# lzzcd001/MeshDiffusion

Hardware: AMD Instinct MI355X
Metric: denoise steps/sec on 64^3x4 DMTet grids (sample-steps/s = n_gpus*batch*steps/wall) (higher is better)
Workload: dtype f16f6 in the Winograd convs behind a GroupNorm (fp16 hi*hi MFMA + MX block-scaled e2m3 cross terms in a K-concatenated scaled MFMA at twice the e4m3 rate; operands and weights equalised per input channel by a power of two: md_wino_equaliser, after the load-time calibration from the measured operand

## Files before the change

### include/meshdiffusion_hip.h

```cpp
#ifndef MESHDIFFUSION_HIP_H
#define MESHDIFFUSION_HIP_H

#include <stdint.h>

#ifdef __cplusplus
extern "C" {
#endif

#define MD_OK 0
#define MD_ERR_BAD_ARG (-1)
#define MD_ERR_UNSUPPORTED (-2)
#define MD_ERR_NO_DEVICE (-3)

#define MD_ABI_VERSION 16

enum {
  MD_CFG_C3_128 = 0,
  MD_CFG_C3_128_K16 = 1,
  MD_CFG_C3_32 = 2,
  MD_CFG_C3_LOW = 3,
  MD_CFG_C3_S2 = 4,
  MD_CFG_G1_128 = 5,
  MD_CFG_G1_128_LOW = 6,
  MD_CFG_G1_64_LOW = 7,
  MD_CFG_C3_128_V2 = 8,
  MD_CFG_C3_128_SW = 9,
  MD_CFG_C3_128_PIPE = 10,
  MD_CFG_C3_128_FAST = 14,
  MD_CFG_C5_128_K16 = 15,
  MD_CFG_C5_32_K16 = 16,
  MD_CFG_C3_128_W4 = 17,
  MD_CFG_C3X_32 = 18,
  MD_CFG_C5X_32_K16 = 19,
  MD_CFG_C3X_128_K16 = 20,
  MD_CFG_C5X_128 = 21,
  MD_CFG_G1_128_N128 = 22,
  MD_CFG_COUNT = 23
};

enum { MD_OUT_F32B = 0, MD_OUT_S16B = 1, MD_OUT_NCDHW = 2 };
enum { MD_A_PACKED = 0, MD_A_S16B = 1 };
enum { MD_B_S16B = 0, MD_B_F32B_GN = 1 };
enum { MD_PREC_BF16X3 = 0, MD_PREC_FP16X2 = 1 };

typedef struct MdGemmConvArgs {
  const void* a;
  const void* b;
  void* out;
  const float* bias;
  const float* residual;
  float alpha;
  int32_t cfg;
  int32_t batch;
  int32_t rows;
  int32_t rows_alloc;
  int32_t kdim;
  int32_t D, H, W;
  int32_t ups;
  int32_t a_src;
  int32_t out_mode;
  int32_t a_rows;
  int64_t a_bstride;
  int64_t bias_bstride;
  int64_t res_bstride;
  int64_t b_bstride;
  float* partial;
  int32_t ksplit;
  int32_t prec;
  double* stats;
  int32_t stagger;
  int32_t b_mode;
  const void* b2;
  const float* b_ac;
  int64_t b2_bstride;
  int32_t b_split;
  int32_t b_silu;
} MdGemmConvArgs;

int md_abi_version(void);
int md_device_count(void);

int md_gemm_conv(const MdGemmConvArgs* args, void* stream);
int64_t md_gemm_conv_partial_bytes(const MdGemmConvArgs* args);
int md_gemm_conv_cfg_info(int32_t cfg, int32_t* nt, int32_t* kc, int32_t* cols,
                          int32_t* taps, int32_t* lds_bytes, int32_t* threads);

int md_pack_weights(const float* w, void* wpk, int32_t rows, int32_t kdim, int32_t taps,
                    int64_t s_row, int64_t s_k, int64_t s_tap, int32_t nt, int32_t kc,
                    int32_t prec, void* stream);
int64_t md_packed_weight_bytes(int32_t rows, int32_t kdim, int32_t taps, int32_t nt, int32_t kc);

int md_gn_stats(const float* x, double* sums, int32_t batch, int32_t C, int64_t P,
                int32_t c_total, int32_t c_off, void* stream);
int md_gn_finalize(const double* sums, const float* gamma, const float* beta,
                   float* params, int32_t batch, int32_t c_total, int32_t groups,
                   int64_t P, float eps, float* ac, void* stream);
int md_gn_apply(const float* x, const float* params, void* out, void* out_raw, int32_t batch,
                int32_t C, int64_t P, int32_t c_total, int32_t c_off, int32_t norm,
                int32_t silu, float drop_p, uint64_t drop_seed, void* stream);
int md_dropout_scale(float* out, int32_t batch, int32_t C, int64_t P, int32_t c_total, int32_t c_off,
                     float drop_p, uint64_t drop_seed, void* stream);
int md_zero(void* p, int64_t bytes, void* stream);

int md_timestep_embedding(const float* t, float* emb, int32_t batch, int32_t dim, void* stream);
int md_linear(const float* x, const float* w, const float* bias, float* y, int32_t batch,
              int32_t in_dim, int32_t out_dim, int32_t silu_in, void* stream);

int md_fold_dx(const float* y, const float* bias, float* out, int32_t batch, int32_t co, int32_t kx, int32_t rows_alloc,
               int32_t D, int32_t H, int32_t W, void* stream);
int md_ncdhw_to_s16b_xfold(const float* x, void* out, int32_t batch, int32_t C, int32_t kx, int32_t c_pad, int32_t D, int32_t H,
                           int32_t W, void* stream);
int md_ncdhw_to_s16b(const float* x, void* out, int32_t batch, int32_t C, int32_t c_pad,
                     int64_t P, void* stream);
int md_f32b_to_ncdhw(const float* x, float* out, int32_t batch, int32_t C, int64_t P, void* stream);
int md_ncdhw_to_f32b(const float* x, float* out, int32_t batch, int32_t C, int64_t P, void* stream);
int md_s16b_to_ncdhw(const void* x, float* out, int32_t batch, int32_t C, int64_t P, void* stream);

int md_softmax_keys(const float* s, void* p, int32_t batch, int32_t n_keys, int32_t n_q,
                    void* stream);

int md_nin_f32(const float* x1, const float* x2, int32_t c1, int32_t c2, const void* wpk, const float* bias,
               float* out, int32_t batch, int32_t cout, int64_t P, int32_t n_cu, void* stream);

int64_t md_wino_operand_bytes(int32_t batch, int32_t cin, int32_t D, int32_t H, int32_t W);
int md_wino_prep(const float* x1, const float* x2, int32_t c1, int32_t c2, const float* ac, int32_t silu, int32_t ups,
                 void* t_out, int32_t batch, int32_t D, int32_t H, int32_t W, float drop_p, uint64_t drop_seed, void* stream);
int64_t md_wino_weight_bytes(int32_t cout, int32_t cin);
int md_wino_pack_weights(const float* w, void* wpk, int32_t cout, int32_t cin, int64_t s_row, int64_t s_k, int32_t flip,
                         void* stream);
int md_conv3_wino(const void* t_in, const void* wpk, float* out, const float* bias, int64_t bias_bstride,
                  const float* residual, int64_t res_bstride, double* stats, int32_t batch, int32_t cin, int32_t cout,
                  int32_t D, int32_t H, int32_t W, int32_t variant, void* stream);

int md_wino_equaliser(const float* gamma, const float* beta, const float* w, int32_t cout, int32_t cin, int64_t s_row, int64_t s_k,
                      float* eq, void* stream);
int md_wino_equaliser_measured(const float* gamma, const float* beta, const float* w, const float* a2m, int32_t cout, int32_t cin,
                               int64_t s_row, int64_t s_k, float* eq, void* stream);
int md_wino_operand_ms(const float* x1, const float* x2, int32_t c1, int32_t c2, const float* ac, int32_t silu, int32_t batch, int64_t P,
                       float* ms, void* stream);
int md_wino_prep_f8(const float* x1, const float* x2, int32_t c1, int32_t c2, const float* ac, int32_t silu, int32_t ups,
                    const float* eq, void* t_out, int32_t batch, int32_t D, int32_t H, int32_t W, void* stream);
int64_t md_wino_weight_bytes_f8(int32_t cout, int32_t cin);
int md_wino_pack_weights_f8(const float* w, const float* eq, void* wpk, int32_t cout, int32_t cin, int64_t s_row, int64_t s_k, void* stream);
int md_conv3_wino_f8(const void* t_in, const void* wpk, float* out, const float* bias, int64_t bias_bstride,
                     const float* residual, int64_t res_bstride, double* stats, int32_t batch, int32_t cin, int32_t cout,
                     int32_t D, int32_t H, int32_t W, void* stream);
int md_absmax(const float* x, int64_t n, uint32_t* amax_bits, void* stream);
int md_wino_prep_dual_f6(const float* x, int32_t c, void* t_out, void* u_out, float* sums, float tscale, const uint32_t* amax_bits,
                         int32_t batch, int32_t D, int32_t H, int32_t W, void* stream);
int md_conv3_wino_f6_scaled(const void* t_in, const void* wpk, float* out, const float* bias, int64_t bias_bstride,
                            const float* residual, int64_t res_bstride, double* stats, int32_t batch, int32_t cin, int32_t cout,
                            int32_t D, int32_t H, int32_t W, float out_scale, const uint32_t* amax_bits, void* stream);

int md_wino_prep_f6(const float* x1, const float* x2, int32_t c1, int32_t c2, const float* ac, int32_t silu, int32_t ups,
                    const float* eq, void* t_out, int32_t batch, int32_t D, int32_t H, int32_t W, void* stream);
int md_wino_pack_weights_f6(const float* w, const float* eq, void* wpk, int32_t cout, int32_t cin, int64_t s_row, int64_t s_k, void* stream);
int md_conv3_wino_f6(const void* t_in, const void* wpk, float* out, const float* bias, int64_t bias_bstride,
                     const float* residual, int64_t res_bstride, double* stats, int32_t batch, int32_t cin, int32_t cout,
                     int32_t D, int32_t H, int32_t W, void* stream);

int md_conv3_stem(const void* x16, const void* wpk, float* out, const float* bias, const float* residual, double* stats,
                  int32_t batch, int32_t cout, int32_t D, int32_t H, int32_t W, void* stream);

int md_conv3_head(const float* x, const float* ac, const void* wpk, float* y, int32_t batch, int32_t cin, int32_t rows_alloc,
                  int32_t D, int32_t H, int32_t W, void* stream);

enum { MD_PACK_WPK = 0, MD_PACK_WINO = 1, MD_PACK_WINO_F6 = 2 };
typedef struct MdPackJob {
  const float* w;
  void* out;
  int64_t s_row, s_k, s_tap, n_items, block0;
  int32_t rows, kdim, taps, nt, kc, prec, flip, kind;
} MdPackJob;
int md_pack_batch(const MdPackJob* jobs_dev, int32_t n_jobs, int64_t total_blocks, int32_t tiled, void* stream);

int md_conv3_s2(const float* x, const void* wpk, float* out, const float* bias, int64_t bias_bstride, double* stats,
                int32_t batch, int32_t cin, int32_t rows, int32_t rows_alloc, int32_t D, int32_t H, int32_t W, void* stream);

int md_wino_prep_v2(const float* x1, const float* x2, int32_t c1, int32_t c2, const float* ac, int32_t silu, int32_t ups,
                    void* t_out, int32_t batch, int32_t D, int32_t H, int32_t W, float drop_p, uint64_t drop_seed, void* stream);

int md_wino_prep_dual(const float* x1, const float* x2, int32_t c1, int32_t c2, const float* ac, int32_t silu, int32_t ups,
                      void* t_out, void* u_out, float* sums, int32_t batch, int32_t D, int32_t H, int32_t W, float drop_p,
                      uint64_t drop_seed, void* stream);

int md_attn_fwd(const void* qk, const void* vT, void* out, const float* bias_v, int32_t batch, int32_t C,
                int32_t N, float scale, void* stream);

int md_ancestral_step(const float* x, const float* eps, const float* z, const float* mask,
                      const float* coef, float* x_out, float* x_mean_out, int32_t batch,
                      int32_t C, int64_t P, void* stream);
int md_ddim_step(const double* x, const float* eps, const float* mask, const double* coef, const float* partial,
                 const float* pmask, int32_t ch, double* x_out, double* x0_out, float* x_f32, int32_t batch,
                 int32_t C, int64_t P, void* stream);
#define MD_LANGEVIN_SLABS 64
#define MD_CORRECTOR_LANGEVIN 0
#define MD_CORRECTOR_ALD 1
#define MD_SDE_REVERSE_DIFFUSION 0
#define MD_SDE_EULER_MARUYAMA 1
int md_langevin_norms(const float* eps, const float* z, int32_t batch, int32_t C, int64_t P, double* slabs, void* stream);
int md_langevin_step(const float* x, const float* eps, const float* z, const float* mask, const float* coef,
                     const double* slabs, float snr, int32_t mode, float* x_out, float* x_mean_out, float* step_out,
                     int32_t batch, int32_t C, int64_t P, void* stream);
int md_sde_step(const float* x, const float* eps, const float* z, const float* mask, const float* coef, int32_t kind,
                float* x_out, float* x_mean_out, int32_t batch, int32_t C, int64_t P, void* stream);
int md_inpaint_blend(float* x, const float* src, const float* pmask, const float* gmask,
                     int32_t batch, int32_t C, int32_t ch, int64_t P, int64_t src_bstride,
                     void* stream);

int md_inpaint_renoise(float* x, float* x_mean, const float* z, const float* pmask,
                       const float* gmask, const float* coef, int32_t batch, int32_t C,
                       int32_t ch, int64_t P, void* stream);

int md_ddpm_perturb(const float* x0, const float* noise, const float* mask, const float* coef, float* out,
                    int32_t batch, int32_t C, int64_t P, void* stream);
int md_masked_sq_err(const float* eps_hat, const float* noise, const float* mask, double* sums, float* grad,
                     float gscale, int32_t batch, int32_t C, int64_t P, void* stream);
int md_grad_sqnorm(const float* g, int64_t n, double* out, void* stream);
int md_adam_ema_step(float* p, const float* g, float* m, float* v, float* ema, int64_t n, float lr, float beta1,
                     float beta2, float eps, float weight_decay, int32_t step, float ema_decay,
                     const double* grad_sqnorm, float max_norm, void* stream);

int64_t md_pb16_bytes(int32_t batch, int32_t C, int32_t D, int32_t H, int32_t W, int32_t guard, int32_t pad);
int md_to_pb16(const void* src, void* out, int32_t batch, int32_t C, int32_t c_src, int32_t D, int32_t H, int32_t W,
               int32_t guard, int32_t pad, int32_t mode, int32_t up, int32_t stuff, int32_t zsplit, int32_t zhalo,
               void* stream);
int md_wgrad_finish(const float* g, float* dw, int32_t rows, int32_t cols, int32_t cols_alloc, int32_t ntap,
                    int32_t tap0, int64_t s_row, int64_t s_k, int64_t s_tap, void* stream);
int64_t md_wgrad_workspace_bytes(int32_t rows, int32_t cols, int32_t taps, int32_t ksplit);
int md_wgrad(const void* dy_pb, const void* act_pb, float* dw, void* workspace, int64_t workspace_bytes, int32_t batch,
             int32_t a_ch, int32_t b_ch, int32_t rows, int32_t cols, int32_t D, int32_t H, int32_t W, int32_t guard,
             int32_t taps, int32_t ksplit, int64_t s_row, int64_t s_k, int64_t s_tap, void* stream);

int64_t md_wgrad_wino_workspace_bytes(int32_t co, int32_t ci, int32_t ksplit);
int md_wgrad_wino(const void* u_dy, const void* t_act, float* dw, void* workspace, int64_t workspace_bytes, int32_t batch,
                  int32_t co, int32_t ci, int32_t D, int32_t H, int32_t W, int32_t ksplit, int64_t s_row, int64_t s_k,
                  int64_t s_tap, void* stream);

int64_t md_wgrad_nin_workspace_bytes(int32_t co, int32_t ci, int32_t ksplit);
int md_wgrad_nin(const void* dy_s16, const void* x_s16, float* dw, void* workspace, int64_t workspace_bytes, int32_t batch,
                 int32_t co, int32_t ci, int64_t P, int32_t ksplit, int64_t s_row, int64_t s_k, void* stream);
int md_gn_bwd_stats(const float* x, const float* dy, const float* params, double* sums, int32_t batch, int32_t C,
                    int64_t P, int32_t c_total, int32_t c_off, int32_t dy_ctotal, int32_t silu, float drop_p,
                    uint64_t drop_seed, void* stream);
int md_gn_bwd_finalize(const double* sums, const float* params, const float* gamma, float* coef, float* dgamma,
                       float* dbeta, int32_t batch, int32_t c_total, int32_t groups, int64_t P, void* stream);
int md_gn_bwd_apply(const float* x, const float* dy, const float* params, const float* coef, float* dx, int32_t batch,
                    int32_t C, int64_t P, int32_t c_total, int32_t c_off, int32_t dy_ctotal, int32_t silu,
                    int32_t accumulate, float drop_p, uint64_t drop_seed, const float* residual, float* ch_sums,
                    uint32_t* amax_bits, void* stream);
int md_channel_sums(const float* x, float* out, int32_t batch, int32_t C, int64_t P, void* stream);
int md_s16b_transpose(const void* in, void* out, int32_t batch, int32_t R, int32_t Cn, void* stream);
int md_softmax_keys_bwd(const void* p, const float* dp, void* ds, int32_t batch, int32_t n_keys, int32_t n_q,
                        float alpha, void* stream);
int md_grad_resample(const float* in, float* out, int32_t batch, int32_t C, int32_t Dc, int32_t Hc, int32_t Wc,
                     int32_t mode, int32_t accumulate, void* stream);

int64_t md_marching_tets_workspace_bytes(int32_t n_meshes, int32_t n_edges, int32_t n_tets);
int md_marching_tets(const float* pos, const float* sdf, const int32_t* tets,
                     const int32_t* edges, const int32_t* tet_edges, int32_t n_meshes,
                     int32_t n_verts, int32_t n_edges, int32_t n_tets, float* verts,
                     int64_t* faces, int64_t* face_tet, int32_t* counts, void* workspace,
                     int64_t workspace_bytes, void* stream);
#define MD_SDF_REG_SLABS 64
#define MD_SDF_REG_WORKSPACE_BYTES (MD_SDF_REG_SLABS * 24)
int md_marching_tets_bwd(const float* pos, const float* sdf, const int32_t* edges, const int32_t* vid,
                         const int32_t* counts, const float* grad_verts, const int32_t* inc_ptr, const int32_t* inc,
                         int32_t n_meshes, int32_t n_verts, int32_t n_edges, float* dpos, float* dsdf, void* stream);
int md_sdf_reg_loss(const float* sdf, const int32_t* edges, int32_t n_verts, int32_t n_edges, void* workspace,
                    float* loss, int32_t* count, void* stream);
int md_sdf_reg_loss_bwd(const float* sdf, const int32_t* edges, const int32_t* inc_ptr, const int32_t* inc,
                        const int32_t* count, const float* grad_out, int32_t n_verts, int32_t n_edges, float* dsdf,
                        void* stream);

int md_vertex_normals(const float* verts, const int64_t* faces, int64_t n_verts, int64_t n_faces, float* v_nrm,
                      float* f_nrm, void* stream);

int64_t md_nn_sided_workspace_bytes(int32_t batch, int32_t n, int32_t m);
int md_nn_sided(const float* p, const float* q, int32_t batch, int32_t n, int32_t m, int32_t skip_same_index,
                float* dist, int64_t* idx, void* workspace, int64_t workspace_bytes, void* stream);
int md_chamfer_bwd(const float* p, const float* q, const int64_t* idx_pq, const int64_t* idx_qp,
                   const int32_t* ptr_p, const int32_t* order_p, const int32_t* ptr_q, const int32_t* order_q,
                   int32_t batch, int32_t n, int32_t m, float w1, float w2, const float* grad_out, float* dp,
                   float* dq, void* stream);
int md_face_areas(const float* verts, const int64_t* faces, int32_t batch, int32_t n_verts, int32_t n_faces,
                  float* areas, void* stream);
int md_sample_points(const float* verts, const int64_t* faces, const float* cdf, const float* r_face,
                     const float* r_u, const float* r_v, const int64_t* face_choices_in, int32_t batch,
                     int32_t n_verts, int32_t n_faces, int32_t n_samples, float* points, int64_t* face_choices,
                     float* weights, void* stream);
int md_sample_points_bwd(const float* grad_points, const float* weights, const int32_t* ptr, const int32_t* order,
                         int32_t batch, int32_t n_verts, int32_t n_samples, float* dverts, void* stream);

#ifdef __cplusplus
}
#endif
#endif
```

### meshdiffusion_amd/_lib.py

```python
import ctypes as C
import os

_HERE = os.path.dirname(os.path.abspath(__file__))
LIB_PATH = os.environ.get("MD_LIB") or os.path.join(_HERE, "libmeshdiffusion_hip.so")

(CFG_C3_128, CFG_C3_128_K16, CFG_C3_32, CFG_C3_LOW, CFG_C3_S2, CFG_G1_128, CFG_G1_128_LOW, CFG_G1_64_LOW,
 CFG_C3_128_V2, CFG_C3_128_SW, CFG_C3_128_PIPE) = range(11)
(CFG_C3_128_FAST, CFG_C5_128_K16, CFG_C5_32_K16, CFG_C3_128_W4, CFG_C3X_32, CFG_C5X_32_K16, CFG_C3X_128_K16, CFG_C5X_128,
 CFG_G1_128_N128) = range(14, 23)
OUT_F32B, OUT_S16B, OUT_NCDHW = 0, 1, 2
PREC_BF16X3, PREC_FP16X2 = 0, 1
A_PACKED, A_S16B = 0, 1
B_S16B, B_F32B_GN = 0, 1
CORRECTOR_LANGEVIN, CORRECTOR_ALD = 0, 1
SDE_REVERSE_DIFFUSION, SDE_EULER_MARUYAMA = 0, 1
LANGEVIN_SLABS = 64

CFG_NT_KC = {
    CFG_C3_128: (128, 32), CFG_C3_128_K16: (128, 16), CFG_C3_32: (32, 32), CFG_C3_LOW: (128, 32),
    CFG_C3_S2: (128, 32), CFG_G1_128: (128, 32), CFG_G1_128_LOW: (128, 32), CFG_G1_64_LOW: (64, 32),
    CFG_C3_128_V2: (128, 32), CFG_C3_128_SW: (128, 32), CFG_C3_128_PIPE: (128, 32),
    CFG_C3_128_FAST: (128, 32), CFG_C5_128_K16: (128, 16), CFG_C5_32_K16: (32, 16), CFG_C3_128_W4: (128, 32), CFG_C3X_32: (32, 32), CFG_C5X_32_K16: (32, 16), CFG_C3X_128_K16: (128, 16), CFG_C5X_128: (128, 32), CFG_G1_128_N128: (128, 32),
}
ABLATION_CFG_NT_KC = {c: (128, 32) for c in (101, 102, 103, 104, 105, 111, 113, 114, 116, 117, 118, 122)}


class MdGemmConvArgs(C.Structure):
    _fields_ = [
        ("a", C.c_void_p), ("b", C.c_void_p), ("out", C.c_void_p), ("bias", C.c_void_p),
        ("residual", C.c_void_p), ("alpha", C.c_float), ("cfg", C.c_int32), ("batch", C.c_int32),
        ("rows", C.c_int32), ("rows_alloc", C.c_int32), ("kdim", C.c_int32), ("D", C.c_int32),
        ("H", C.c_int32), ("W", C.c_int32), ("ups", C.c_int32), ("a_src", C.c_int32),
        ("out_mode", C.c_int32), ("a_rows", C.c_int32), ("a_bstride", C.c_int64),
        ("bias_bstride", C.c_int64), ("res_bstride", C.c_int64), ("b_bstride", C.c_int64), ("partial", C.c_void_p), ("ksplit", C.c_int32), ("prec", C.c_int32),
        ("stats", C.c_void_p), ("stagger", C.c_int32), ("b_mode", C.c_int32), ("b2", C.c_void_p), ("b_ac", C.c_void_p),
        ("b2_bstride", C.c_int64), ("b_split", C.c_int32), ("b_silu", C.c_int32),
    ]


class MdPackJob(C.Structure):
    _fields_ = [
        ("w", C.c_void_p), ("out", C.c_void_p), ("s_row", C.c_int64), ("s_k", C.c_int64), ("s_tap", C.c_int64),
        ("n_items", C.c_int64), ("block0", C.c_int64), ("rows", C.c_int32), ("kdim", C.c_int32), ("taps", C.c_int32),
        ("nt", C.c_int32), ("kc", C.c_int32), ("prec", C.c_int32), ("flip", C.c_int32), ("kind", C.c_int32),
    ]


PACK_WPK, PACK_WINO, PACK_WINO_F6 = 0, 1, 2
ABI_VERSION = 16
_P, _I32, _I64, _F, _U64 = C.c_void_p, C.c_int32, C.c_int64, C.c_float, C.c_uint64

SIGNATURES = {
    "md_abi_version": (C.c_int, []),
    "md_device_count": (C.c_int, []),
    "md_gemm_conv": (C.c_int, [C.POINTER(MdGemmConvArgs), _P]),
    "md_gemm_conv_partial_bytes": (_I64, [C.POINTER(MdGemmConvArgs)]),
    "md_gemm_conv_cfg_info": (C.c_int, [_I32] + [C.POINTER(C.c_int32)] * 6),
    "md_pack_weights": (C.c_int, [_P, _P, _I32, _I32, _I32, _I64, _I64, _I64, _I32, _I32, _I32, _P]),
    "md_packed_weight_bytes": (_I64, [_I32, _I32, _I32, _I32, _I32]),
    "md_gn_stats": (C.c_int, [_P, _P, _I32, _I32, _I64, _I32, _I32, _P]),
    "md_gn_finalize": (C.c_int, [_P, _P, _P, _P, _I32, _I32, _I32, _I64, _F, _P, _P]),
    "md_gn_apply": (C.c_int, [_P, _P, _P, _P, _I32, _I32, _I64, _I32, _I32, _I32, _I32, _F, _U64, _P]),
    "md_dropout_scale": (C.c_int, [_P, _I32, _I32, _I64, _I32, _I32, _F, _U64, _P]),
    "md_zero": (C.c_int, [_P, _I64, _P]),
    "md_timestep_embedding": (C.c_int, [_P, _P, _I32, _I32, _P]),
    "md_linear": (C.c_int, [_P, _P, _P, _P, _I32, _I32, _I32, _I32, _P]),
    "md_ncdhw_to_s16b_xfold": (C.c_int, [_P, _P, _I32, _I32, _I32, _I32, _I32, _I32, _I32, _P]),
    "md_fold_dx": (C.c_int, [_P, _P, _P, _I32, _I32, _I32, _I32, _I32, _I32, _I32, _P]),
    "md_ncdhw_to_s16b": (C.c_int, [_P, _P, _I32, _I32, _I32, _I64, _P]),
    "md_f32b_to_ncdhw": (C.c_int, [_P, _P, _I32, _I32, _I64, _P]),
    "md_ncdhw_to_f32b": (C.c_int, [_P, _P, _I32, _I32, _I64, _P]),
    "md_s16b_to_ncdhw": (C.c_int, [_P, _P, _I32, _I32, _I64, _P]),
    "md_nin_f32": (C.c_int, [_P, _P, _I32, _I32, _P, _P, _P, _I32, _I32, _I64, _I32, _P]),
    "md_wino_operand_bytes": (_I64, [_I32, _I32, _I32, _I32, _I32]),
    "md_wino_prep": (C.c_int, [_P, _P, _I32, _I32, _P, _I32, _I32, _P, _I32, _I32, _I32, _I32, _F, _U64, _P]),
    "md_wino_weight_bytes": (_I64, [_I32, _I32]),
    "md_wino_pack_weights": (C.c_int, [_P, _P, _I32, _I32, _I64, _I64, _I32, _P]),
    "md_conv3_wino": (C.c_int, [_P, _P, _P, _P, _I64, _P, _I64, _P, _I32, _I32, _I32, _I32, _I32, _I32, _I32, _P]),
    "md_wino_equaliser": (C.c_int, [_P, _P, _P, _I32, _I32, _I64, _I64, _P, _P]),
    "md_wino_equaliser_measured": (C.c_int, [_P, _P, _P, _P, _I32, _I32, _I64, _I64, _P, _P]),
    "md_wino_operand_ms": (C.c_int, [_P, _P, _I32, _I32, _P, _I32, _I32, _I64, _P, _P]),
    "md_wino_prep_f8": (C.c_int, [_P, _P, _I32, _I32, _P, _I32, _I32, _P, _P, _I32, _I32, _I32, _I32, _P]),
    "md_wino_weight_bytes_f8": (_I64, [_I32, _I32]),
    "md_wino_pack_weights_f8": (C.c_int, [_P, _P, _P, _I32, _I32, _I64, _I64, _P]),
    "md_conv3_wino_f8": (C.c_int, [_P, _P, _P, _P, _I64, _P, _I64, _P, _I32, _I32, _I32, _I32, _I32, _I32, _P]),
    "md_absmax": (C.c_int, [_P, _I64, _P, _P]),
    "md_wino_prep_dual_f6": (C.c_int, [_P, _I32, _P, _P, _P, _F, _P, _I32, _I32, _I32, _I32, _P]),
    "md_conv3_wino_f6_scaled": (C.c_int, [_P, _P, _P, _P, _I64, _P, _I64, _P, _I32, _I32, _I32, _I32, _I32, _I32, _F, _P, _P]),
    "md_wino_prep_f6": (C.c_int, [_P, _P, _I32, _I32, _P, _I32, _I32, _P, _P, _I32, _I32, _I32, _I32, _P]),
    "md_wino_pack_weights_f6": (C.c_int, [_P, _P, _P, _I32, _I32, _I64, _I64, _P]),
    "md_conv3_wino_f6": (C.c_int, [_P, _P, _P, _P, _I64, _P, _I64, _P, _I32, _I32, _I32, _I32, _I32, _I32, _P]),
    "md_conv3_stem": (C.c_int, [_P, _P, _P, _P, _P, _P, _I32, _I32, _I32, _I32, _I32, _P]),
    "md_conv3_head": (C.c_int, [_P, _P, _P, _P, _I32, _I32, _I32, _I32, _I32, _I32, _P]),
    "md_pack_batch": (C.c_int, [_P, _I32, _I64, _I32, _P]),
    "md_conv3_s2": (C.c_int, [_P, _P, _P, _P, _I64, _P, _I32, _I32, _I32, _I32, _I32, _I32, _I32, _P]),
    "md_wino_prep_v2": (C.c_int, [_P, _P, _I32, _I32, _P, _I32, _I32, _P, _I32, _I32, _I32, _I32, _F, _U64, _P]),
    "md_wino_prep_dual": (C.c_int, [_P, _P, _I32, _I32, _P, _I32, _I32, _P, _P, _P, _I32, _I32, _I32, _I32, _F, _U64, _P]),
    "md_wgrad_wino_workspace_bytes": (_I64, [_I32, _I32, _I32]),
    "md_wgrad_wino": (C.c_int, [_P, _P, _P, _P, _I64, _I32, _I32, _I32, _I32, _I32, _I32, _I32, _I64, _I64, _I64, _P]),
    "md_wgrad_nin_workspace_bytes": (_I64, [_I32, _I32, _I32]),
    "md_wgrad_nin": (C.c_int, [_P, _P, _P, _P, _I64, _I32, _I32, _I32, _I64, _I32, _I64, _I64, _P]),
    "md_attn_fwd": (C.c_int, [_P, _P, _P, _P, _I32, _I32, _I32, _F, _P]),
    "md_softmax_keys": (C.c_int, [_P, _P, _I32, _I32, _I32, _P]),
    "md_ancestral_step": (C.c_int, [_P, _P, _P, _P, _P, _P, _P, _I32, _I32, _I64, _P]),
    "md_ddim_step": (C.c_int, [_P, _P, _P, _P, _P, _P, _I32, _P, _P, _P, _I32, _I32, _I64, _P]),
    "md_langevin_norms": (C.c_int, [_P, _P, _I32, _I32, _I64, _P, _P]),
    "md_langevin_step": (C.c_int, [_P, _P, _P, _P, _P, _P, _F, _I32, _P, _P, _P, _I32, _I32, _I64, _P]),
    "md_sde_step": (C.c_int, [_P, _P, _P, _P, _P, _I32, _P, _P, _I32, _I32, _I64, _P]),
    "md_inpaint_blend": (C.c_int, [_P, _P, _P, _P, _I32, _I32, _I32, _I64, _I64, _P]),
    "md_inpaint_renoise": (C.c_int, [_P, _P, _P, _P, _P, _P, _I32, _I32, _I32, _I64, _P]),
    "md_ddpm_perturb": (C.c_int, [_P, _P, _P, _P, _P, _I32, _I32, _I64, _P]),
    "md_masked_sq_err": (C.c_int, [_P, _P, _P, _P, _P, _F, _I32, _I32, _I64, _P]),
    "md_grad_sqnorm": (C.c_int, [_P, _I64, _P, _P]),
    "md_adam_ema_step": (C.c_int, [_P, _P, _P, _P, _P, _I64, _F, _F, _F, _F, _F, _I32, _F, _P, _F, _P]),
    "md_pb16_bytes": (_I64, [_I32, _I32, _I32, _I32, _I32, _I32, _I32]),
    "md_to_pb16": (C.c_int, [_P, _P, _I32, _I32, _I32, _I32, _I32, _I32, _I32, _I32, _I32, _I32, _I32, _I32, _I32, _P]),
    "md_wgrad_finish": (C.c_int, [_P, _P, _I32, _I32, _I32, _I32, _I32, _I64, _I64, _I64, _P]),
    "md_wgrad_workspace_bytes": (_I64, [_I32, _I32, _I32, _I32]),
    "md_wgrad": (C.c_int, [_P, _P, _P, _P, _I64, _I32, _I32, _I32, _I32, _I32, _I32, _I32, _I32, _I32, _I32, _I32, _I64, _I64,
                           _I64, _P]),
    "md_gn_bwd_stats": (C.c_int, [_P, _P, _P, _P, _I32, _I32, _I64, _I32, _I32, _I32, _I32, _F, _U64, _P]),
    "md_gn_bwd_finalize": (C.c_int, [_P, _P, _P, _P, _P, _P, _I32, _I32, _I32, _I64, _P]),
    "md_gn_bwd_apply": (C.c_int, [_P, _P, _P, _P, _P, _I32, _I32, _I64, _I32, _I32, _I32, _I32, _I32, _F, _U64, _P, _P, _P, _P]),
    "md_channel_sums": (C.c_int, [_P, _P, _I32, _I32, _I64, _P]),
    "md_s16b_transpose": (C.c_int, [_P, _P, _I32, _I32, _I32, _P]),
    "md_softmax_keys_bwd": (C.c_int, [_P, _P, _P, _I32, _I32, _I32, _F, _P]),
    "md_grad_resample": (C.c_int, [_P, _P, _I32, _I32, _I32, _I32, _I32, _I32, _I32, _P]),
    "md_marching_tets_workspace_bytes": (_I64, [_I32, _I32, _I32]),
    "md_vertex_normals": (C.c_int, [_P, _P, _I64, _I64, _P, _P, _P]),
    "md_marching_tets": (C.c_int, [_P, _P, _P, _P, _P, _I32, _I32, _I32, _I32, _P, _P, _P, _P, _P, _I64, _P]),
    "md_marching_tets_bwd": (C.c_int, [_P, _P, _P, _P, _P, _P, _P, _P, _I32, _I32, _I32, _P, _P, _P]),
    "md_sdf_reg_loss": (C.c_int, [_P, _P, _I32, _I32, _P, _P, _P, _P]),
    "md_sdf_reg_loss_bwd": (C.c_int, [_P, _P, _P, _P, _P, _P, _I32, _I32, _P, _P]),
    "md_nn_sided_workspace_bytes": (_I64, [_I32, _I32, _I32]),
    "md_nn_sided": (C.c_int, [_P, _P, _I32, _I32, _I32, _I32, _P, _P, _P, _I64, _P]),
    "md_chamfer_bwd": (C.c_int, [_P, _P, _P, _P, _P, _P, _P, _P, _I32, _I32, _I32, _F, _F, _P, _P, _P, _P]),
    "md_face_areas": (C.c_int, [_P, _P, _I32, _I32, _I32, _P, _P]),
    "md_sample_points": (C.c_int, [_P, _P, _P, _P, _P, _P, _P, _I32, _I32, _I32, _I32, _P, _P, _P, _P]),
    "md_sample_points_bwd": (C.c_int, [_P, _P, _P, _P, _I32, _I32, _I32, _P, _P]),
}
SDF_REG_SLABS = 64
SDF_REG_WORKSPACE_BYTES = SDF_REG_SLABS * 24

ABLATION_SIGNATURES = {"md_wgrad_set_debug": (None, [_I32])}

_lib = None


class MeshDiffusionHipError(RuntimeError):
    pass


def load():
    global _lib
    if _lib is not None:
        return _lib
    if not os.path.exists(LIB_PATH):
        raise MeshDiffusionHipError(
            f"{LIB_PATH} not found: run `python -m meshdiffusion_amd.build` (needs hipcc). "
            "There is no CPU fallback for the HIP path.")
    import torch
    lib = C.CDLL(LIB_PATH)
    for name, (res, args) in SIGNATURES.items():
        fn = getattr(lib, name)
        fn.restype = res
        fn.argtypes = args
    for name, (res, args) in ABLATION_SIGNATURES.items():
        fn = getattr(lib, name, None)
        if fn is not None:
            fn.restype = res
            fn.argtypes = args
    if lib.md_abi_version() != ABI_VERSION:
        raise MeshDiffusionHipError(f"ABI version mismatch: library {lib.md_abi_version()}, host code {ABI_VERSION}")
    if hasattr(lib, "md_wgrad_set_debug"):
        CFG_NT_KC.update(ABLATION_CFG_NT_KC)
    for cfg, (nt, kc) in CFG_NT_KC.items():
        v = [C.c_int32() for _ in range(6)]
        lib.md_gemm_conv_cfg_info(cfg, *[C.byref(x) for x in v])
        if (v[0].value, v[1].value) != (nt, kc):
            raise MeshDiffusionHipError(f"cfg {cfg} NT/KC mismatch between _lib.py and the library")
    if torch.cuda.is_available() and lib.md_device_count() != torch.cuda.device_count():
        raise MeshDiffusionHipError("libmeshdiffusion_hip.so is not sharing PyTorch's HIP runtime "
                                    f"({lib.md_device_count()} vs {torch.cuda.device_count()} devices)")
    _lib = lib
    return lib


def check(rc, what):
    if rc != 0:
        raise MeshDiffusionHipError(f"{what} failed with code {rc}")


def cfg_info(cfg):
    lib = load()
    v = [C.c_int32() for _ in range(6)]
    check(lib.md_gemm_conv_cfg_info(cfg, *[C.byref(x) for x in v]), "md_gemm_conv_cfg_info")
    keys = ("nt", "kc", "cols", "taps", "lds_bytes", "threads")
    return dict(zip(keys, (x.value for x in v)))
```

### meshdiffusion_amd/csrc/conv3_wino.hip

```cpp
#include <type_traits>
#include "md_common.h"
#include "md_pack.h"

namespace {
constexpr int WN_THREADS = 256;
constexpr int WN_TZ = 4, WN_TY = 8, WN_TX = 8;
constexpr int WN_TPOS = 6 * 10 * 4;
constexpr int WN_HBUF = 4 * WN_TPOS * 16;
constexpr int WN_NDMA = WN_HBUF / 1024;
constexpr int WN_RED = 4 * 32 * 2;
constexpr int WN_WAVE_LDS = 2 * WN_HBUF;
constexpr int WN_LDS_BYTES = 4 * WN_WAVE_LDS + 4 * WN_NDMA * 64 * 4;

__device__ const uint4 wn_zero16 = {0u, 0u, 0u, 0u};

typedef uint32_t wn_u32x4 __attribute__((ext_vector_type(4)));
__device__ __forceinline__ uint4 wn_gload16(const void* p) {
  return __builtin_bit_cast(uint4, *(__attribute__((address_space(1))) const wn_u32x4*)(uintptr_t)p);
}
}

__global__ __launch_bounds__(256) void md_wino_prep_kernel(const float* __restrict__ x1, const float* __restrict__ x2,
                                                           int c1, int c2, const float* __restrict__ ac, int silu, int ups,
                                                           uint4* __restrict__ T, int batch, int D, int H, int W,
                                                           uint32_t thr16, float drop_scale, uint64_t seed) {
  const int Wp = W >> 1;
  const int64_t Ph = (int64_t)D * H * Wp;
  const int CG = (c1 + c2) >> 3;
  const int64_t n = (int64_t)batch * CG * Ph;
  const int64_t id = (int64_t)blockIdx.x * 256 + threadIdx.x;
  if (id >= n) return;
  const int64_t pos2 = id % Ph;
  const int cg = (int)((id / Ph) % CG);
  const int b = (int)(id / (Ph * CG));
  const int pr = (int)(pos2 % Wp), y = (int)((pos2 / Wp) % H), z = (int)(pos2 / ((int64_t)Wp * H));
  int Di = D, Hi = H, Wi = W, zs = z, ys = y;
  if (ups) { Di >>= 1; Hi >>= 1; Wi >>= 1; zs >>= 1; ys >>= 1; }
  const int64_t Pin = (int64_t)Di * Hi * Wi;
  const float* src = (cg * 8 < c1) ? x1 + ((int64_t)b * (c1 >> 3) + cg) * Pin * 8
                                   : x2 + ((int64_t)b * (c2 >> 3) + (cg - (c1 >> 3))) * Pin * 8;
  float a[8], c[8];
#pragma unroll
  for (int e = 0; e < 8; ++e) { a[e] = 1.f; c[e] = 0.f; }
  if (ac != nullptr) {
    const f32x4* ap = (const f32x4*)(ac + ((int64_t)b * (c1 + c2) + cg * 8) * 2);
#pragma unroll
    for (int q = 0; q < 4; ++q) {
      const f32x4 v = ap[q];
      a[2 * q] = v[0]; c[2 * q] = v[1]; a[2 * q + 1] = v[2]; c[2 * q + 1] = v[3];
    }
  }
  float d[4][8];
#pragma unroll
  for (int q = 0; q < 4; ++q) {
    const int xw = 2 * pr - 1 + q;
    const bool live = xw >= 0 && xw < W;
    f32x4 v0 = {0.f, 0.f, 0.f, 0.f}, v1 = v0;
    const int xs = ups ? (xw >> 1) : xw;
    const int64_t spos = ((int64_t)zs * Hi + ys) * Wi + xs;
    if (live) {
      const f32x4* p = (const f32x4*)(src + spos * 8);
      v0 = p[0]; v1 = p[1];
    }
    uint64_t bits[2] = {0, 0};
    if (thr16) {
      const uint64_t quad0 = (uint64_t)(((int64_t)b * (c1 + c2) + cg * 8) >> 2) * (uint64_t)Pin;
      bits[0] = md_drop_bits(seed, quad0 + (uint64_t)spos);
      bits[1] = md_drop_bits(seed, quad0 + (uint64_t)Pin + (uint64_t)spos);
    }
#pragma unroll
    for (int e = 0; e < 8; ++e) {
      float yv = e < 4 ? v0[e] : v1[e - 4];
      if (ac != nullptr) {
        yv = yv * a[e] + c[e];
        if (silu) yv = yv * __builtin_amdgcn_rcpf(1.0f + __builtin_amdgcn_exp2f(yv * -1.4426950408889634f));
      }
      if (thr16) yv = md_drop_keep(bits[e >> 2], e & 3, thr16) ? yv * drop_scale : 0.f;
      d[q][e] = live ? yv : 0.f;
    }
  }
  uint4* out = T + ((int64_t)b * CG + cg) * 8 * Ph + pos2;
#pragma unroll
  for (int f = 0; f < 4; ++f) {
    float t[8];
#pragma unroll
    for (int e = 0; e < 8; ++e)
      t[e] = f == 0 ? d[0][e] - d[2][e] : f == 1 ? d[1][e] + d[2][e] : f == 2 ? d[2][e] - d[1][e] : d[1][e] - d[3][e];
    uint32_t hw[4], lw[4];
#pragma unroll
    for (int q = 0; q < 4; ++q) md_split2(t[2 * q], t[2 * q + 1], hw[q], lw[q]);
    out[(int64_t)(f * 2) * Ph] = make_uint4(hw[0], hw[1], hw[2], hw[3]);
    out[(int64_t)(f * 2 + 1) * Ph] = make_uint4(lw[0], lw[1], lw[2], lw[3]);
  }
}

__global__ __launch_bounds__(256) void md_wino_pack_weights_kernel(const float* __restrict__ w, uint4* __restrict__ wpk,
                                                                   int cout, int cin, int64_t s_row, int64_t s_k, int flip) {
  const int64_t n = (int64_t)cout * cin * 36 / 4;
  const int64_t id = (int64_t)blockIdx.x * 256 + threadIdx.x;
  if (id >= n) return;
  wpk[id] = md_pack_wino_item(w, cout, cin, s_row, s_k, flip, id);
}

__global__ __launch_bounds__(256) void md_wino_amax_kernel(const float* __restrict__ w, int cout, int cin, int64_t s_row, int64_t s_k,
                                                           uint32_t* __restrict__ hdr, const float* __restrict__ eq) {
  const int64_t n = (int64_t)cout * cin * 27;
  float m = 0.f;
  for (int64_t i = (int64_t)blockIdx.x * 256 + threadIdx.x; i < n; i += (int64_t)gridDim.x * 256) {
    const int t = (int)(i % 27);
    const int64_t r = i / 27;
    float v = fabsf(w[(r / cin) * s_row + (r % cin) * s_k + t]);
    if (eq) v /= eq[r % cin];
    m = v > m ? v : m;
  }
  m = md_wave_max(m);
  if ((threadIdx.x & 63) == 0) atomicMax(hdr, __float_as_uint(m));
}

__global__ __launch_bounds__(256) void md_wino_pack_weights_f8_kernel(const float* __restrict__ w, uint4* __restrict__ wpk, int cout, int cin,
                                                                      int64_t s_row, int64_t s_k, uint32_t* __restrict__ hdr,
                                                                      const float* __restrict__ eq) {
  const int64_t n = (int64_t)cout * cin * 9;
  const int64_t id = (int64_t)blockIdx.x * 256 + threadIdx.x;
  const float wscale = md_wino_f8_wscale(__uint_as_float(hdr[0]));
  if (id == 0) {
    hdr[1] = (uint32_t)ilogbf(wscale);
    hdr[2] = __float_as_uint(1.0f / wscale);
    hdr[3] = 0u;
  }
  if (id >= n) return;
  wpk[id] = md_pack_wino_f8_item(w, cout, cin, s_row, s_k, wscale, id, eq);
}

__global__ __launch_bounds__(256) void md_wino_pack_weights_f6_kernel(const float* __restrict__ w, uint4* __restrict__ wpk, int cout, int cin,
                                                                      int64_t s_row, int64_t s_k, uint32_t* __restrict__ hdr,
                                                                      const float* __restrict__ eq) {
  const int64_t n = (int64_t)cout * cin * 9;
  const int64_t id = (int64_t)blockIdx.x * 256 + threadIdx.x;
  const float wscale = md_wino_f8_wscale(__uint_as_float(hdr[0]));
  if (id == 0) {
    hdr[1] = (uint32_t)ilogbf(wscale);
    hdr[2] = __float_as_uint(1.0f / wscale);
    hdr[3] = 6u;
  }
  if (id >= n) return;
  wpk[id] = md_pack_wino_f6_item(w, cout, cin, s_row, s_k, wscale, id, eq);
}

struct WnArgs {
  const uint4* T;
  const uint4* wpk;
  float* out;
  const float* bias;
  const float* residual;
  double* stats;
  const float* hdr;
  int64_t bias_bstride, res_bstride;
  int batch, cin, cout, D, H, W;
  float out_scale;
  const uint32_t* amax;
};

typedef int wn_i32x8 __attribute__((ext_vector_type(8)));
typedef int wn_i32x4 __attribute__((ext_vector_type(4)));

template <int ABL, bool F8 = false, bool F6 = false, bool RES = false>
__global__ __launch_bounds__(WN_THREADS) void md_conv3_wino_kernel(const WnArgs A) {
  __shared__ __attribute__((aligned(16))) unsigned char wn_smem[WN_LDS_BYTES];
  const int tid = threadIdx.x, lane = tid & 63;
  const int wid = __builtin_amdgcn_readfirstlane(tid >> 6);
  const int j = lane & 31, h = lane >> 5;
  uint64_t stamp[12];
  auto mark = [&](int k) { if constexpr (ABL & 128) stamp[k] = __builtin_amdgcn_s_memtime(); };
  if constexpr (ABL & 128) stamp[10] = __builtin_amdgcn_s_memrealtime();
  mark(0);

#ifndef W8_STAGGER
#define W8_STAGGER 0
#endif
  if constexpr (W8_STAGGER > 0) {
    const unsigned lin = blockIdx.x + gridDim.x * blockIdx.y;
    if (lin < 256u) {
      const unsigned ph = (lin * 0x9E3779B1u) >> 24;
      const uint64_t t_end = __builtin_amdgcn_s_memtime() + ((uint64_t)ph * (uint64_t)W8_STAGGER >> 8);
      while (__builtin_amdgcn_s_memtime() < t_end) __builtin_amdgcn_s_sleep(16);
    }
  }
  const int D = A.D, H = A.H, W = A.W, Wp = W >> 1;
  const int64_t P = (int64_t)D * H * W, Ph = P >> 1;
  const int ntx = W / WN_TX, nty = H / WN_TY, ntz = D / WN_TZ;
  const int tiles = ntx * nty * ntz;
  int bid = blockIdx.x;
  if ((gridDim.x & 7) == 0) bid = (blockIdx.x & 7) * (gridDim.x >> 3) + (blockIdx.x >> 3);
  const int b = bid / tiles, t = bid % tiles;
  const int x0 = (t % ntx) * WN_TX, y0 = ((t / ntx) % nty) * WN_TY, z0 = (t / (ntx * nty)) * WN_TZ;
  const int rtb = blockIdx.y;
  const int CG = A.cin >> 3, nchunk = A.cin >> 4;
  const int nsteps = nchunk * 9;

  unsigned char* my_smem = wn_smem + wid * WN_WAVE_LDS;

  auto halo_off = [&](int k) -> int {
    const int e = k * 64 + lane;
    const int hp = e / WN_TPOS, tp = e % WN_TPOS;
    const int dz = tp / 40, hy = (tp >> 2) % 10, pr = tp & 3;
    const int z = z0 + dz - 1, y = y0 + hy - 1;
    const bool live = (z >= 0) & (z < D) & (y >= 0) & (y < H);
    if constexpr (F8) {
      const int Phi = (int)Ph;
      const int off = (hp >> 1) * 8 * Phi + (hp & 1) * Phi + (z * H + y) * Wp + (x0 >> 1) + pr;
      return live ? off : -1;
    }
    return live ? (int)((int64_t)(hp >> 1) * 8 * Ph + (int64_t)(hp & 1) * Ph + ((int64_t)z * H + y) * Wp + (x0 >> 1) + pr) : -1;
  };
  const uint4* tbase = A.T + ((int64_t)b * CG * 8 + wid * 2) * Ph;
  const uint4* zsrc = &wn_zero16;
  auto halo_load = [&](int chunk, int k) -> uint4 {
    const int dk = halo_off(k);
    const uint4* src = dk >= 0 ? tbase + (int64_t)chunk * 16 * Ph + dk : zsrc;
    if constexpr (ABL & 32)
      src = A.T + (((blockIdx.x & 255) * 4 + wid) * 2 + (chunk & 1)) * 960 + k * 64 + lane;
    if constexpr (ABL & 64)
      src = A.T + ((((((int64_t)bid * 4 + wid) * nchunk + chunk) * 960) & (((int64_t)1 << 26) - 1)) + k * 64 + lane);
    if constexpr (ABL & 1) return make_uint4(0, 0, 0, 0);
    return wn_gload16(src);
  };
  auto halo_store = [&](int buf, int k, const uint4& v) {
    if constexpr (!(ABL & 1)) *(uint4*)(my_smem + buf * WN_HBUF + k * 1024 + lane * 16) = v;
  };
  const uint4* wbase = A.wpk + (((int64_t)rtb * nsteps) * 4 + wid) * 512 + lane;
  auto load_A = [&](int s, bf16x8 (&dst)[8]) {
    const uint4* wp = wbase + (int64_t)s * 2048;
#pragma unroll
    for (int i = 0; i < 8; ++i) dst[i] = __builtin_bit_cast(bf16x8, wp[i * 64]);
  };
  const unsigned char* vB = my_smem + h * 2 * WN_TPOS * 16 + j * 16;
  auto read_B = [&](int tap, int buf, bf16x8 (&dst)[8], bool force) {
    const int kd = tap / 3, kh = tap % 3;
    const unsigned char* p = vB + buf * WN_HBUF + (kd * 40 + kh * 4) * 16;
#pragma unroll
    for (int ct = 0; ct < 4; ++ct)
      if (force || !(ABL & 8)) {
        dst[ct * 2] = *(const bf16x8*)(p + ct * 40 * 16);
        dst[ct * 2 + 1] = *(const bf16x8*)(p + WN_TPOS * 16 + ct * 40 * 16);
      }
  };

  f32x16 acc[4][4];
  auto zero_acc = [&]() {
#pragma unroll
    for (int rt = 0; rt < 4; ++rt)
#pragma unroll
      for (int ct = 0; ct < 4; ++ct) {
#pragma unroll
        for (int r = 0; r < 16; ++r) acc[rt][ct][r] = 0.f;
        asm volatile("" : "+a"(acc[rt][ct]));
      }
  };
#ifndef W8_PRO_FENCE
#define W8_PRO_FENCE 1
#endif
  if constexpr (!W8_PRO_FENCE) zero_acc();
  float descale = 1.f;
  if constexpr (F8) {
    static_assert(ABL == 0 || ABL == 128, "timing ablations exist for the bf16x3 loop only");
#ifndef W8_HG
#define W8_HG 3
#endif
    auto slot3_of_store = [](int u) constexpr -> int { return (u == 0 || u == 3 || u == 6) ? 0 : ((u == 2 || u == 5 || u == 8) ? 1 : 2); };
    auto slot3_of_request = [](int u) constexpr -> int { return (u == 0 || u == 3 || u == 6) ? 0 : ((u == 2 || u == 5 || u == 8) ? 1 : 2); };
    const int npairs = nsteps >> 1;
    const uint4* wbase8 = A.wpk + (((int64_t)rtb * npairs) * 4 + wid) * 1024 + lane;
    uint4 A8h[2][4][2], B8h[2][2], hs8[W8_HG == 3 ? 3 : 2][4];
    wn_i32x8 A8f[2][4], B8f[2];
    uint32_t* otab = (uint32_t*)(wn_smem + 4 * WN_WAVE_LDS) + wid * (WN_NDMA * 64) + lane;
    static_assert(4 * WN_WAVE_LDS + 4 * WN_NDMA * 64 * 4 <= WN_LDS_BYTES, "offset tables fit behind the halo buffers");
    uint32_t live_mask = 0;
    constexpr int D1 = 64, D2 = (40 - 8) * 16, D3 = WN_HBUF - (2 * 40 + 2 * 4) * 16;
    const unsigned char* vBh = my_smem + h * 2 * WN_TPOS * 16 + j * 16;
    const unsigned char* vB8a = my_smem + WN_TPOS * 16 + j * 16 + h * D1;
    const unsigned char* vB8b = my_smem + WN_TPOS * 16 + j * 16 + h * D2;
    const unsigned char* vB8c = my_smem + WN_TPOS * 16 + j * 16 + h * D3;
    auto step_off = [](int s) constexpr -> int { return (s / 9) * WN_HBUF + (((s % 9) / 3) * 40 + ((s % 9) % 3) * 4) * 16; };
    auto cat8 = [](const uint4& x, const uint4& y) -> wn_i32x8 {
      const wn_i32x4 a = __builtin_bit_cast(wn_i32x4, x), b = __builtin_bit_cast(wn_i32x4, y);
      return __builtin_shufflevector(a, b, 0, 1, 2, 3, 4, 5, 6, 7);
    };
    auto halo_store8 = [&](int buf, int k, uint4 v) {
      const bool lv = (live_mask >> k) & 1u;
      v.x = lv ? v.x : 0u; v.y = lv ? v.y : 0u; v.z = lv ? v.z : 0u; v.w = lv ? v.w : 0u;
      *(uint4*)(my_smem + buf * WN_HBUF + k * 1024 + lane * 16) = v;
    };
    auto read_B8 = [&](auto uc, auto ctc, uint4 (&dh)[2], wn_i32x8& df) {
      constexpr int u = decltype(uc)::value, ct = decltype(ctc)::value;
      constexpr int o0 = step_off(2 * u) + ct * 40 * 16, o1 = step_off(2 * u + 1) + ct * 40 * 16, dk = o1 - o0;
      static_assert(dk == D1 || dk == D2 || dk == D3, "three kinds of step pairs");
      const unsigned char* v8 = dk == D1 ? vB8a : (dk == D2 ? vB8b : vB8c);
      dh[0] = *(const uint4*)(vBh + o0);
      dh[1] = *(const uint4*)(vBh + o1);
      df = cat8(*(const uint4*)(v8 + o0), *(const uint4*)(v8 + o0 + 2 * WN_TPOS * 16));
    };
#ifndef W8_ABL
#define W8_ABL 0
#endif
    auto load_A8 = [&](int p, int set, int rt0, int nrt) {
      const uint4* wp = wbase8 + (int64_t)((W8_ABL & 1) ? 0 : p) * 4096;
#pragma unroll
      for (int rt = 0; rt < 4; ++rt)
        if (rt >= rt0 && rt < rt0 + nrt) {
          A8h[set][rt][0] = wp[(rt * 4 + 0) * 64];
          A8h[set][rt][1] = wp[(rt * 4 + 1) * 64];
          A8f[set][rt] = cat8(wp[(rt * 4 + 2) * 64], wp[(rt * 4 + 3) * 64]);
        }
    };
    {
      uint4 h0[WN_NDMA];
      load_A8(0, 0, 0, 4);
      if constexpr (W8_PRO_FENCE) __builtin_amdgcn_sched_barrier(0);
#pragma unroll
      for (int k = 0; k < WN_NDMA; ++k) {
        const int dk = halo_off(k);
        const uint32_t o = dk >= 0 ? (uint32_t)dk : 0u;
        live_mask |= (dk >= 0 ? 1u : 0u) << k;
        otab[k * 64] = o;
        h0[k] = wn_gload16(tbase + o);
#ifndef W8_PRO_SPLIT
#define W8_PRO_SPLIT 1
#endif
        if constexpr (!W8_PRO_SPLIT)
          if (k < (W8_HG == 3 ? 12 : 8)) hs8[W8_HG == 3 ? slot3_of_store(k >> 2) : (k >> 2)][k & 3] = wn_gload16(tbase + (int64_t)16 * Ph + o);
        if constexpr (W8_PRO_FENCE) __builtin_amdgcn_sched_barrier(0);
      }
      if constexpr (W8_PRO_SPLIT) {
#pragma unroll
        for (int k = 0; k < (W8_HG == 3 ? 12 : 8); ++k)
          hs8[W8_HG == 3 ? slot3_of_store(k >> 2) : (k >> 2)][k & 3] = wn_gload16(tbase + (int64_t)16 * Ph + otab[k * 64]);
        if constexpr (W8_PRO_FENCE) __builtin_amdgcn_sched_barrier(0);
      }
      if constexpr (W8_PRO_FENCE) zero_acc();
      descale = A.hdr[2] * A.out_scale;
      if (A.amax != nullptr) descale *= ldexpf(1.f, -md_dgrad_lift_log2(A.amax[0]));
      if constexpr (W8_PRO_FENCE) __builtin_amdgcn_sched_barrier(0);
#pragma unroll
      for (int k = 0; k < WN_NDMA; ++k) halo_store8(0, k, h0[k]);
    }
    read_B8(std::integral_constant<int, 0>{}, std::integral_constant<int, 0>{}, B8h[0], B8f[0]);
    mark(1);
    const int scale_a = 127 - 11, scale_b = 127;
    auto base_of = [](int u) constexpr -> int {
      if (W8_HG == 3)
        return u == 0 ? 12 : (u >= 2 && u <= 5 ? (u - 2) * 4 : (u >= 6 ? (u - 6) * 4 : 99));
      return u == 0 ? 8 : (u == 1 ? 12 : (u >= 3 && u <= 6 ? (u - 3) * 4 : (u >= 7 ? (u - 7) * 4 : 99)));
    };
    uint32_t off_next[4] = {0u, 0u, 0u, 0u};
    auto body = [&](auto pbc, int c0) {
      constexpr int PB = decltype(pbc)::value;
      const int p0 = (c0 * 9) >> 1;
      const int cn1 = c0 + 1, cn2 = c0 + 2 < nchunk ? c0 + 2 : nchunk - 1, cn3 = c0 + 3 < nchunk ? c0 + 3 : nchunk - 1;
#ifndef W8_TAIL_RES
#define W8_TAIL_RES 1
#endif
      const uint32_t m2 = (!W8_TAIL_RES || c0 + 2 < nchunk) ? ~0u : 0u, m3 = (!W8_TAIL_RES || c0 + 3 < nchunk) ? ~0u : 0u;
      auto group = [&](auto uc, auto ctc) {
        constexpr int u = decltype(uc)::value, ct = decltype(ctc)::value;
        constexpr int aset = (PB + u) & 1, bset = ct & 1;
        constexpr int un = ct < 3 ? u : (u + 1) % 9, ctn = ct < 3 ? ct + 1 : 0;
        constexpr int HG = W8_HG, RG = HG == 1 ? 1 : 2;
        constexpr int sq_lo = HG == 0 ? ct : (HG == 1 ? (ct < 2 ? 2 * ct : 4) : (ct < 2 ? ct : (ct == 2 ? 2 : 4)));
        constexpr int sq_hi = HG == 0 ? ct + 1 : (HG == 1 ? (ct < 2 ? 2 * ct + 2 : 4) : (ct < 2 ? ct + 1 : 4));
        constexpr int st_base = u <= 3 ? u * 4 : (u >= 5 ? (u - 5) * 4 : 99);
        constexpr int st_slot = HG == 3 ? slot3_of_store(u) : (u <= 3 ? (u & 1) : ((u - 5) & 1));
        constexpr int n_st = (sq_lo < sq_hi && st_base + sq_lo < WN_NDMA) + (sq_lo + 1 < sq_hi && st_base + sq_lo + 1 < WN_NDMA);
#pragma unroll
        for (int q = 0; q < 4; ++q)
          if (q >= sq_lo && q < sq_hi && st_base + q < WN_NDMA) {
            if constexpr (W8_ABL & 4) asm volatile("" :: "v"(hs8[st_slot][q].x), "v"(hs8[st_slot][q].w));
            else halo_store8(u <= 3 ? 1 : 0, st_base + q, hs8[st_slot][q]);
          }
        if constexpr (!(W8_ABL & 8)) read_B8(std::integral_constant<int, un>{}, std::integral_constant<int, ctn>{}, B8h[bset ^ 1], B8f[bset ^ 1]);
        else asm volatile("" : "+v"(B8h[bset ^ 1][0]), "+v"(B8h[bset ^ 1][1]), "+v"(B8f[bset ^ 1]));
#pragma unroll
        for (int rt = 0; rt < 4; ++rt)
          acc[rt][ct] = __builtin_amdgcn_mfma_f32_32x32x16_f16(__builtin_bit_cast(f16x8, A8h[aset][rt][0]), __builtin_bit_cast(f16x8, B8h[bset][0]),
                                                               acc[rt][ct], 0, 0, 0);
        __builtin_amdgcn_sched_group_barrier(0x008, 1, 0);
        if constexpr (n_st > 0 && !(W8_ABL & 4)) __builtin_amdgcn_sched_group_barrier(0x200, n_st, 0);
        __builtin_amdgcn_sched_group_barrier(0x100, 1, 0);
        __builtin_amdgcn_sched_group_barrier(0x008, 1, 0);
        __builtin_amdgcn_sched_group_barrier(0x100, 1, 0);
        __builtin_amdgcn_sched_group_barrier(0x008, 1, 0);
        __builtin_amdgcn_sched_group_barrier(0x100, 1, 0);
        __builtin_amdgcn_sched_group_barrier(0x008, 1, 0);
        __builtin_amdgcn_sched_group_barrier(0x100, 1, 0);
        __builtin_amdgcn_sched_barrier(0);
        constexpr int ld_base = base_of(u), ldn_base = base_of(un);
        constexpr int ld_slot = HG == 3 ? slot3_of_request(u) : (u == 0 ? 0 : (u == 1 ? 1 : ((u - 3) & 1)));
        constexpr int rq_lo = HG == 0 ? (ct >= 2 ? 2 * (ct - 2) : 4) : (ct == RG ? 0 : 4), rq_hi = HG == 0 ? (ct >= 2 ? 2 * (ct - 2) + 2 : 4) : 4;
        constexpr int rn_lo = HG == 0 ? (ctn >= 2 ? 2 * (ctn - 2) : 4) : (ctn == RG ? 0 : 4), rn_hi = HG == 0 ? (ctn >= 2 ? 2 * (ctn - 2) + 2 : 4) : 4;
        constexpr int n_ld = (rq_lo < rq_hi ? ((ld_base + rq_lo < WN_NDMA) + (ld_base + rq_lo + 1 < WN_NDMA && rq_lo + 1 < rq_hi) +
                                               (ld_base + rq_lo + 2 < WN_NDMA && rq_lo + 2 < rq_hi) + (ld_base + rq_lo + 3 < WN_NDMA && rq_lo + 3 < rq_hi)) : 0);
        constexpr int n_rd = (rn_lo < rn_hi ? ((ldn_base + rn_lo < WN_NDMA) + (ldn_base + rn_lo + 1 < WN_NDMA && rn_lo + 1 < rn_hi) +
                                               (ldn_base + rn_lo + 2 < WN_NDMA && rn_lo + 2 < rn_hi) + (ldn_base + rn_lo + 3 < WN_NDMA && rn_lo + 3 < rn_hi)) : 0);
        if constexpr (n_ld > 0) {
          constexpr int which = HG == 3 ? (u == 0 ? 1 : (u <= 5 ? 2 : 3)) : (u <= 1 ? 1 : (u <= 6 ? 2 : 3));
          const uint4* cb = tbase + (int64_t)(which == 1 ? cn1 : (which == 2 ? cn2 : cn3)) * 16 * Ph;
          const uint32_t om = which == 1 ? ~0u : (which == 2 ? m2 : m3);
#pragma unroll
          for (int i = 0; i < 4; ++i)
            if (i < n_ld) hs8[ld_slot][rq_lo + i] = wn_gload16((W8_ABL & 2) ? tbase + lane : cb + (off_next[i] & om));
        }
#pragma unroll
        for (int i = 0; i < 4; ++i)
          if (i < n_rd) off_next[i] = otab[(ldn_base + rn_lo + i) * 64];
#pragma unroll
        for (int rt = 0; rt < 4; ++rt)
          acc[rt][ct] = __builtin_amdgcn_mfma_f32_32x32x16_f16(__builtin_bit_cast(f16x8, A8h[aset][rt][1]), __builtin_bit_cast(f16x8, B8h[bset][1]),
                                                               acc[rt][ct], 0, 0, 0);
        __builtin_amdgcn_sched_group_barrier(0x008, 1, 0);
        if constexpr (n_rd > 0) __builtin_amdgcn_sched_group_barrier(0x100, n_rd, 0);
        if constexpr (n_ld > 2) __builtin_amdgcn_sched_group_barrier(0x020, 1, 0);
        __builtin_amdgcn_sched_group_barrier(0x008, 1, 0);
        if constexpr (n_ld > 0) __builtin_amdgcn_sched_group_barrier(0x020, 1, 0);
        __builtin_amdgcn_sched_group_barrier(0x008, 1, 0);
        if constexpr (n_ld > 1) __builtin_amdgcn_sched_group_barrier(0x020, 1, 0);
        __builtin_amdgcn_sched_group_barrier(0x008, 1, 0);
        if constexpr (n_ld > 3) __builtin_amdgcn_sched_group_barrier(0x020, 1, 0);
        __builtin_amdgcn_sched_barrier(0);
#ifndef W8_NA
#define W8_NA 2
#endif
        constexpr int NA = HG == 1 ? 1 : W8_NA;
        if constexpr (ct < NA) {
          const int pn = p0 + u + 1 < npairs ? p0 + u + 1 : npairs - 1;
          load_A8(pn, aset ^ 1, ct * (4 / NA), 4 / NA);
        }
#pragma unroll
        for (int rt = 0; rt < 4; ++rt)
          if constexpr (F6)
            acc[rt][ct] = __builtin_amdgcn_mfma_scale_f32_32x32x64_f8f6f4(A8f[aset][rt], B8f[bset], acc[rt][ct], 2, 2, 0, A8f[aset][rt][6], 0,
                                                                          B8f[bset][6]);
          else
            acc[rt][ct] = __builtin_amdgcn_mfma_scale_f32_32x32x64_f8f6f4(A8f[aset][rt], B8f[bset], acc[rt][ct], 0, 0, 0, scale_a, 0, scale_b);
        if constexpr (ct < NA) {
#pragma unroll
          for (int i_ = 0; i_ < 4; ++i_) {
            __builtin_amdgcn_sched_group_barrier(0x008, 1, 0);
            __builtin_amdgcn_sched_group_barrier(0x020, 8 / NA / 2, 0);
          }
        }
        __builtin_amdgcn_sched_barrier(0);
      };
      auto pair_step = [&](auto uc) {
        group(uc, std::integral_constant<int, 0>{});
        group(uc, std::integral_constant<int, 1>{});
        group(uc, std::integral_constant<int, 2>{});
        group(uc, std::integral_constant<int, 3>{});
      };
      pair_step(std::integral_constant<int, 0>{}); pair_step(std::integral_constant<int, 1>{}); pair_step(std::integral_constant<int, 2>{});
      pair_step(std::integral_constant<int, 3>{}); pair_step(std::integral_constant<int, 4>{}); pair_step(std::integral_constant<int, 5>{});
      pair_step(std::integral_constant<int, 6>{}); pair_step(std::integral_constant<int, 7>{}); pair_step(std::integral_constant<int, 8>{});
      (void)cn1;
    };
    for (int c0 = 0; c0 < nchunk; c0 += 4) {
      body(std::integral_constant<int, 0>{}, c0);
      if (c0 + 2 >= nchunk) break;
      body(std::integral_constant<int, 1>{}, c0 + 2);
    }
  } else {
  bf16x8 Ar[3][8];
    bf16x8 Bf[2][8];
    uint4 hst[2][3];
  
    {
      uint4 h0[WN_NDMA];
      if constexpr (W8_PRO_FENCE) {
        load_A(0, Ar[0]);
        load_A(nsteps > 1 ? 1 : 0, Ar[1]);
        __builtin_amdgcn_sched_barrier(0);
      }
  #pragma unroll
      for (int k = 0; k < WN_NDMA; ++k) {
        h0[k] = halo_load(0, k);
        if constexpr (W8_PRO_FENCE) __builtin_amdgcn_sched_barrier(0);
      }
      if constexpr (W8_PRO_FENCE) {
        zero_acc();
        __builtin_amdgcn_sched_barrier(0);
      } else {
        load_A(0, Ar[0]);
        load_A(nsteps > 1 ? 1 : 0, Ar[1]);
      }
      if constexpr (ABL & 4) load_A(nsteps > 2 ? 2 : 0, Ar[2]);
  #pragma unroll
      for (int k = 0; k < WN_NDMA; ++k) halo_store(0, k, h0[k]);
      if constexpr (ABL & 2) {
  #pragma unroll
        for (int k = 0; k < WN_NDMA; ++k) halo_store(1, k, h0[k]);
      }
    }
    read_B(0, 0, Bf[0], true);
    mark(1);
  
  #define WN_MFMA(PASS, IDX, a, bq)                                                                                       \
    acc[(IDX) >> 2][(IDX) & 3] = __builtin_amdgcn_mfma_f32_32x32x16_bf16(a[((IDX) >> 2) * 2 + ((PASS) == 0 ? 1 : 0)],   \
                                                                         bq[((IDX) & 3) * 2 + ((PASS) == 1 ? 1 : 0)],    \
                                                                         acc[(IDX) >> 2][(IDX) & 3], 0, 0, 0)
    for (int c0 = 0; c0 < nchunk; c0 += 2) {
  #pragma unroll
      for (int u = 0; u < 18; ++u) {
        const int tap = u % 9, cpar = u / 9;
        const int s = c0 * 9 + u;
        const int sw = s + 2 < nsteps ? s + 2 : nsteps - 1;
        const int cn = c0 + cpar + 1 < nchunk ? c0 + cpar + 1 : nchunk - 1;
        bf16x8 (&Aw)[8] = Ar[u % 3], (&Bc)[8] = Bf[u & 1], (&Bn)[8] = Bf[(u + 1) & 1];
        if constexpr (!(ABL & 4)) load_A(sw, Ar[(u + 2) % 3]);
        if (tap < 8) read_B(tap + 1, cpar, Bn, false);
        else read_B(0, cpar ^ 1, Bn, false);
  #pragma unroll
        for (int m = 0; m < 16; ++m) WN_MFMA(0, m, Aw, Bc);
  #pragma unroll
        for (int i_ = 0; i_ < 8; ++i_) {
          __builtin_amdgcn_sched_group_barrier(0x008, 1, 0);
          __builtin_amdgcn_sched_group_barrier(0x100, 1, 0);
          __builtin_amdgcn_sched_group_barrier(0x008, 1, 0);
          __builtin_amdgcn_sched_group_barrier(0x020, 1, 0);
        }
        __builtin_amdgcn_sched_barrier(0);
        if (tap >= 2 && tap <= 6 && !(ABL & 2)) {
  #pragma unroll
          for (int q = 0; q < 3; ++q) halo_store(cpar ^ 1, (tap - 2) * 3 + q, hst[tap & 1][q]);
        }
        if (tap <= 4 && !(ABL & 2)) {
  #pragma unroll
          for (int q = 0; q < 3; ++q) hst[tap & 1][q] = halo_load(cn, tap * 3 + q);
        }
  #pragma unroll
        for (int m = 0; m < 32; ++m) {
          if (m < 16) WN_MFMA(1, m, Aw, Bc); else WN_MFMA(2, m - 16, Aw, Bc);
        }
        __builtin_amdgcn_sched_group_barrier(0x008, 2, 0);
        __builtin_amdgcn_sched_group_barrier(0x020, 1, 0);
        __builtin_amdgcn_sched_group_barrier(0x008, 2, 0);
        __builtin_amdgcn_sched_group_barrier(0x020, 1, 0);
        __builtin_amdgcn_sched_group_barrier(0x008, 2, 0);
        __builtin_amdgcn_sched_group_barrier(0x020, 1, 0);
        __builtin_amdgcn_sched_group_barrier(0x008, 20, 0);
        __builtin_amdgcn_sched_group_barrier(0x200, 1, 0);
        __builtin_amdgcn_sched_group_barrier(0x008, 2, 0);
        __builtin_amdgcn_sched_group_barrier(0x200, 1, 0);
        __builtin_amdgcn_sched_group_barrier(0x008, 2, 0);
        __builtin_amdgcn_sched_group_barrier(0x200, 1, 0);
        __builtin_amdgcn_sched_barrier(0);
      }
    }
  #undef WN_MFMA
  }

  mark(2);
  if constexpr (ABL & 16) {
    float keep = 0.f;
#pragma unroll
    for (int rt = 0; rt < 4; ++rt)
#pragma unroll
      for (int ct = 0; ct < 4; ++ct) keep += acc[rt][ct][0];
    if (keep == 123.456f) A.out[tid] = keep;
    return;
  }
  constexpr int XF_ITEMS = 1024, XREG_FLOATS = (4 * XF_ITEMS + 16) * 4;
  static_assert(2 * XREG_FLOATS * 4 + 2 * WN_RED * 4 <= WN_LDS_BYTES, "two exchange regions + the statistics area fit");
  float* xreg = (float*)wn_smem;
  float* red = xreg + 2 * XREG_FLOATS;
  const int rows_total = A.cout;
  float* outp = A.out + (int64_t)b * rows_total * P;
  const float* resp = A.residual ? A.residual + (int64_t)b * A.res_bstride : nullptr;
  const float* biasp = A.bias ? A.bias + (int64_t)b * A.bias_bstride : nullptr;
  const bool want_stats = (ABL & 128) ? false : A.stats != nullptr;
  const int half = lane & 1, xq = (lane >> 1) & 7, cgp = lane >> 4;
  const int cq = 2 * cgp + half, prr = xq >> 1;
  const bool odd = xq & 1;
  const float sgn = odd ? -1.f : 1.f;
  const int64_t gp0 = ((int64_t)(z0 + wid) * H + y0) * W + x0 + xq;
  auto flush_stats = [&](int r) {
    if (tid < 64) {
      const int ch = tid >> 1, which = tid & 1;
      const float* rb = red + (r & 1) * WN_RED;
      float sum = 0.f;
#pragma unroll
      for (int k = 0; k < 4; ++k) sum += rb[(k * 32 + ch) * 2 + which];
      const int row = rtb * 128 + r * 32 + ch;
      atomicAdd(A.stats + ((int64_t)b * rows_total + row) * 2 + which, (double)sum);
    }
  };
  const bool has_bias = biasp != nullptr;
  f32x4 pbias[4], pres[RES ? 2 : 1][8];
  auto prefetch_res = [&](int r) {
    if constexpr (RES) {
      const float* rp = resp + ((int64_t)(rtb * 16 + r * 4 + cgp) * P + gp0) * 8 + 4 * half;
#pragma unroll
      for (int yr = 0; yr < 8; ++yr) pres[r & 1][yr] = *(const f32x4*)(rp + (int64_t)yr * W * 8);
    }
  };
  {
    const float* bsrc = has_bias ? biasp : (const float*)A.wpk;
#pragma unroll
    for (int r = 0; r < 4; ++r) pbias[r] = *(const f32x4*)(bsrc + rtb * 128 + r * 32 + 4 * cq);
    prefetch_res(0);
    prefetch_res(1);
  }
  auto row_sum8 = [](float v) {
    v += __builtin_bit_cast(float, __builtin_amdgcn_update_dpp(0, __builtin_bit_cast(int, v), 0x128, 0xF, 0xF, true));
    v += __builtin_bit_cast(float, __builtin_amdgcn_update_dpp(0, __builtin_bit_cast(int, v), 0x124, 0xF, 0xF, true));
    v += __builtin_bit_cast(float, __builtin_amdgcn_update_dpp(0, __builtin_bit_cast(int, v), 0x122, 0xF, 0xF, true));
    return v;
  };
  const int sj = ((j & 1) << 2) | ((j >> 1) & 3);
  const int wbase_items = wid * XF_ITEMS + (wid == 2 ? 8 : (wid == 3 ? 16 : 0)) + j * 8;
  auto write_round = [&](int r) {
    float* xw = xreg + (r & 1) * XREG_FLOATS;
#pragma unroll
    for (int q = 0; q < 4; ++q) {
      float* pq = xw + (wbase_items + ((2 * q + h) ^ sj)) * 4;
#pragma unroll
      for (int ct = 0; ct < 4; ++ct) {
        f32x4 v;
#pragma unroll
        for (int e = 0; e < 4; ++e) v[e] = acc[r][ct][q * 4 + e];
        *(f32x4*)(pq + ct * 32 * 8 * 4) = v;
      }
    }
  };
  const int rcol_items = (wid * 32 + prr) * 8;
  const int rx0 = cq ^ (((prr & 1) << 2) | (prr >> 1)), rx1 = rx0 ^ 2;
  const int offA = odd ? 2 * XF_ITEMS + 8 : 0, offC = odd ? 3 * XF_ITEMS + 16 : 2 * XF_ITEMS + 8;
  __syncthreads();
  mark(3);
#ifndef W8_EPI_EARLYW
#define W8_EPI_EARLYW 1
#endif
#pragma unroll
  for (int r = 0; r < 4; ++r) {
    const float* xr = xreg + (r & 1) * XREG_FLOATS;
    if (!W8_EPI_EARLYW || r == 0) write_round(r);
    __syncthreads();
    f32x4 mA[8], mB[8], mC[8];
#pragma unroll
    for (int yr = 0; yr < 8; ++yr) {
      const float* pb = xr + (rcol_items + yr * 32 + ((yr & 1) ? rx1 : rx0)) * 4;
      mA[yr] = *(const f32x4*)(pb + offA * 4);
      mB[yr] = *(const f32x4*)(pb + XF_ITEMS * 4);
      mC[yr] = *(const f32x4*)(pb + offC * 4);
    }
    if (want_stats && r > 0) flush_stats(r - 1);
    if (W8_EPI_EARLYW && r < 3) {
      __builtin_amdgcn_sched_barrier(0);
      write_round(r + 1);
      __builtin_amdgcn_sched_barrier(0);
    }
    float* op = outp + ((int64_t)(rtb * 16 + r * 4 + cgp) * P + gp0) * 8 + 4 * half;
    const f32x4 zero4 = {0.f, 0.f, 0.f, 0.f};
    const f32x4 bv = has_bias ? pbias[r] : zero4;
    f32x4 s1 = zero4, s2 = s1;
#pragma unroll
    for (int yr = 0; yr < 8; ++yr) {
      f32x4 o;
#pragma unroll
      for (int e = 0; e < 4; ++e) {
        const float y = __builtin_fmaf(sgn, mC[yr][e], __builtin_fmaf(sgn, mA[yr][e], mB[yr][e]));
        if constexpr (F8) o[e] = y * descale + bv[e];
        else o[e] = y + bv[e];
      }
      if constexpr (RES) o += pres[r & 1][yr];
      *(f32x4*)(op + (int64_t)yr * W * 8) = o;
      s1 += o;
      s2 += o * o;
    }
    if (r < 2) prefetch_res(r + 2);
    if (want_stats) {
      f32x4 a1, a2;
#pragma unroll
      for (int e = 0; e < 4; ++e) { a1[e] = row_sum8(s1[e]); a2[e] = row_sum8(s2[e]); }
      if ((lane & 14) == 0) {
        float* rb = red + (r & 1) * WN_RED + (wid * 32 + 4 * cq) * 2;
        const f32x4 w0 = {a1[0], a2[0], a1[1], a2[1]}, w1 = {a1[2], a2[2], a1[3], a2[3]};
        *(f32x4*)rb = w0;
        *(f32x4*)(rb + 4) = w1;
      }
    }
    mark(4 + r);
  }
  if (want_stats) {
    __syncthreads();
    flush_stats(3);
  }
  if constexpr (ABL & 128) {
    const unsigned lin = blockIdx.x + gridDim.x * blockIdx.y;
#ifdef W8_STAMPS_LATE
    const unsigned total = gridDim.x * gridDim.y;
    const unsigned lin0 = total > 1024u ? total - 1024u : 0u;
#else
    const unsigned lin0 = 0u;
#endif
    if (lin >= lin0 && lin - lin0 < 1024u && lane == 0) {
      uint64_t* dst = (uint64_t*)A.stats + ((size_t)(lin - lin0) * 4 + wid) * 12;
      stamp[8] = __builtin_amdgcn_s_memtime();
      stamp[11] = __builtin_amdgcn_s_memrealtime();
      stamp[9] = (uint64_t)(uint32_t)__builtin_amdgcn_s_getreg((31 << 11) | 4) |
                 ((uint64_t)(uint32_t)__builtin_amdgcn_s_getreg((31 << 11) | 20) << 32);
#pragma unroll
      for (int k = 0; k < 12; ++k) dst[k] = stamp[k];
    }
  }
}

extern "C" int64_t md_wino_operand_bytes(int32_t batch, int32_t cin, int32_t D, int32_t H, int32_t W) {
  if (batch <= 0 || cin <= 0 || (cin & 7) || D <= 0 || H <= 0 || W <= 0 || (W & 1)) return MD_ERR_BAD_ARG;
  return (int64_t)batch * (cin / 8) * 8 * ((int64_t)D * H * (W / 2)) * 16;
}

extern "C" int md_wino_prep(const float* x1, const float* x2, int32_t c1, int32_t c2, const float* ac, int32_t silu,
                            int32_t ups, void* t_out, int32_t batch, int32_t D, int32_t H, int32_t W, float drop_p,
                            uint64_t drop_seed, void* stream) {
  if (!x1 || !t_out || batch <= 0 || c1 <= 0 || c2 < 0 || (c1 & 7) || (c2 & 7) || (c2 > 0 && !x2)) return MD_ERR_BAD_ARG;
  if (silu && !ac) return MD_ERR_BAD_ARG;
  if (!(drop_p >= 0.f && drop_p < 1.f) || (drop_p > 0.f && (ups || c2 > 0))) return MD_ERR_BAD_ARG;
  if (D <= 0 || H <= 0 || W <= 0 || (W & 1) || (ups && ((D | H | W) & 1))) return MD_ERR_BAD_ARG;
  const int64_t n = (int64_t)batch * ((c1 + c2) / 8) * D * H * (W / 2);
  const int64_t blocks = (n + 255) / 256;
  if (blocks > 0x7fffffff) return MD_ERR_UNSUPPORTED;
  MD_HIP_CLEAR_ERROR();
  hipLaunchKernelGGL(md_wino_prep_kernel, dim3((unsigned)blocks), dim3(256), 0, (hipStream_t)stream, x1, x2, c1, c2, ac, silu,
                     ups, (uint4*)t_out, batch, D, H, W, md_drop_thr16(drop_p), 1.0f / (1.0f - drop_p), drop_seed);
  MD_HIP_CHECK_LAUNCH();
  return MD_OK;
}

extern "C" int64_t md_wino_weight_bytes(int32_t cout, int32_t cin) {
  if (cout <= 0 || cin <= 0 || (cout % 128) || (cin % 32)) return MD_ERR_BAD_ARG;
  return (int64_t)cout * cin * 36 * 4;
}

extern "C" int md_wino_pack_weights(const float* w, void* wpk, int32_t cout, int32_t cin, int64_t s_row, int64_t s_k,
                                    int32_t flip, void* stream) {
  if (!w || !wpk || cout <= 0 || cin <= 0 || (cout % 128) || (cin % 32)) return MD_ERR_BAD_ARG;
  const int64_t n = (int64_t)cout * cin * 9;
  MD_HIP_CLEAR_ERROR();
  hipLaunchKernelGGL(md_wino_pack_weights_kernel, dim3((unsigned)((n + 255) / 256)), dim3(256), 0, (hipStream_t)stream, w,
                     (uint4*)wpk, cout, cin, s_row, s_k, flip);
  MD_HIP_CHECK_LAUNCH();
  return MD_OK;
}

extern "C" int64_t md_wino_weight_bytes_f8(int32_t cout, int32_t cin) {
  if (cout <= 0 || cin <= 0 || (cout % 128) || (cin % 32)) return MD_ERR_BAD_ARG;
  return (int64_t)cout * cin * 36 * 4 + 256;
}

static int md_wino_pack_weights_f8_launch(bool f6, const float* w, const float* eq, void* wpk, int32_t cout, int32_t cin, int64_t s_row, int64_t s_k,
                                          void* stream) {
  if (!w || !wpk || cout <= 0 || cin <= 0 || (cout % 128) || (cin % 32)) return MD_ERR_BAD_ARG;
  const int64_t n = (int64_t)cout * cin * 9;
  uint32_t* hdr = (uint32_t*)((unsigned char*)wpk + n * 16);
  MD_HIP_CLEAR_ERROR();
  hipError_t e = hipMemsetAsync(hdr, 0, 256, (hipStream_t)stream);
  if (e != hipSuccess) return (int)e;
  const int64_t nel = (int64_t)cout * cin * 27;
  int ab = (int)((nel + 255) / 256);
  if (ab > 1024) ab = 1024;
  hipLaunchKernelGGL(md_wino_amax_kernel, dim3((unsigned)ab), dim3(256), 0, (hipStream_t)stream, w, cout, cin, s_row, s_k, hdr, eq);
  MD_HIP_CHECK_LAUNCH();
  if (f6)
    hipLaunchKernelGGL(md_wino_pack_weights_f6_kernel, dim3((unsigned)((n + 255) / 256)), dim3(256), 0, (hipStream_t)stream, w, (uint4*)wpk,
                       cout, cin, s_row, s_k, hdr, eq);
  else
    hipLaunchKernelGGL(md_wino_pack_weights_f8_kernel, dim3((unsigned)((n + 255) / 256)), dim3(256), 0, (hipStream_t)stream, w, (uint4*)wpk,
                       cout, cin, s_row, s_k, hdr, eq);
  MD_HIP_CHECK_LAUNCH();
  return MD_OK;
}

extern "C" int md_wino_pack_weights_f8(const float* w, const float* eq, void* wpk, int32_t cout, int32_t cin, int64_t s_row, int64_t s_k, void* stream) {
  return md_wino_pack_weights_f8_launch(false, w, eq, wpk, cout, cin, s_row, s_k, stream);
}

extern "C" int md_wino_pack_weights_f6(const float* w, const float* eq, void* wpk, int32_t cout, int32_t cin, int64_t s_row, int64_t s_k, void* stream) {
  return md_wino_pack_weights_f8_launch(true, w, eq, wpk, cout, cin, s_row, s_k, stream);
}

static int md_conv3_wino_f8_launch(bool f6, const void* t_in, const void* wpk, float* out, const float* bias, int64_t bias_bstride,
                                   const float* residual, int64_t res_bstride, double* stats, int32_t batch, int32_t cin,
                                   int32_t cout, int32_t D, int32_t H, int32_t W, void* stream, float out_scale = 1.0f,
                                   const uint32_t* amax = nullptr) {
  if (!t_in || !wpk || !out || batch <= 0) return MD_ERR_BAD_ARG;
  if (cin <= 0 || cout <= 0 || (cin % 32) || (cout % 128)) return MD_ERR_UNSUPPORTED;
  if (D <= 0 || H <= 0 || W <= 0 || (D % WN_TZ) || (H % WN_TY) || (W % WN_TX)) return MD_ERR_UNSUPPORTED;
  if ((int64_t)D * H * W * 8 >= (int64_t)1 << 31) return MD_ERR_UNSUPPORTED;
  WnArgs a;
  a.T = (const uint4*)t_in; a.wpk = (const uint4*)wpk; a.out = out; a.bias = bias; a.residual = residual; a.stats = stats;
  a.hdr = (const float*)((const unsigned char*)wpk + (int64_t)cout * cin * 36 * 4);
  a.out_scale = out_scale; a.amax = amax;
  a.bias_bstride = bias_bstride; a.res_bstride = res_bstride;
  a.batch = batch; a.cin = cin; a.cout = cout; a.D = D; a.H = H; a.W = W;
  const int tiles = (D / WN_TZ) * (H / WN_TY) * (W / WN_TX);
  const dim3 grid((unsigned)(tiles * batch), (unsigned)(cout / 128));
  MD_HIP_CLEAR_ERROR();
#ifdef W8_STAMPS
  constexpr int ABL_ = 128;
#else
  constexpr int ABL_ = 0;
#endif
#define WN_LAUNCH8(F6_, RES_) hipLaunchKernelGGL((md_conv3_wino_kernel<ABL_, true, F6_, RES_>), grid, dim3(WN_THREADS), 0, (hipStream_t)stream, a)
  if (f6) { if (residual) WN_LAUNCH8(true, true); else WN_LAUNCH8(true, false); }
  else { if (residual) WN_LAUNCH8(false, true); else WN_LAUNCH8(false, false); }
#undef WN_LAUNCH8
  MD_HIP_CHECK_LAUNCH();
  return MD_OK;
}

extern "C" int md_conv3_wino_f8(const void* t_in, const void* wpk, float* out, const float* bias, int64_t bias_bstride,
                                const float* residual, int64_t res_bstride, double* stats, int32_t batch, int32_t cin,
                                int32_t cout, int32_t D, int32_t H, int32_t W, void* stream) {
  return md_conv3_wino_f8_launch(false, t_in, wpk, out, bias, bias_bstride, residual, res_bstride, stats, batch, cin, cout, D, H, W, stream);
}

extern "C" int md_conv3_wino_f6(const void* t_in, const void* wpk, float* out, const float* bias, int64_t bias_bstride,
                                const float* residual, int64_t res_bstride, double* stats, int32_t batch, int32_t cin,
                                int32_t cout, int32_t D, int32_t H, int32_t W, void* stream) {
  return md_conv3_wino_f8_launch(true, t_in, wpk, out, bias, bias_bstride, residual, res_bstride, stats, batch, cin, cout, D, H, W, stream);
}

extern "C" int md_conv3_wino_f6_scaled(const void* t_in, const void* wpk, float* out, const float* bias, int64_t bias_bstride,
                                       const float* residual, int64_t res_bstride, double* stats, int32_t batch, int32_t cin,
                                       int32_t cout, int32_t D, int32_t H, int32_t W, float out_scale, const uint32_t* amax_bits, void* stream) {
  if (!(out_scale > 0.f)) return MD_ERR_BAD_ARG;
  return md_conv3_wino_f8_launch(true, t_in, wpk, out, bias, bias_bstride, residual, res_bstride, stats, batch, cin, cout, D, H, W, stream, out_scale,
                                 amax_bits);
}

extern "C" int md_conv3_wino(const void* t_in, const void* wpk, float* out, const float* bias, int64_t bias_bstride,
                             const float* residual, int64_t res_bstride, double* stats, int32_t batch, int32_t cin,
                             int32_t cout, int32_t D, int32_t H, int32_t W, int32_t variant, void* stream) {
  if (!t_in || !wpk || !out || batch <= 0) return MD_ERR_BAD_ARG;
  if (cin <= 0 || cout <= 0 || (cin % 32) || (cout % 128)) return MD_ERR_UNSUPPORTED;
  if (D <= 0 || H <= 0 || W <= 0 || (D % WN_TZ) || (H % WN_TY) || (W % WN_TX)) return MD_ERR_UNSUPPORTED;
  if ((int64_t)D * H * W * 8 >= (int64_t)1 << 31) return MD_ERR_UNSUPPORTED;
  WnArgs a;
  a.T = (const uint4*)t_in; a.wpk = (const uint4*)wpk; a.out = out; a.bias = bias; a.residual = residual; a.stats = stats;
  a.hdr = nullptr;
  a.out_scale = 1.0f; a.amax = nullptr;
  a.bias_bstride = bias_bstride; a.res_bstride = res_bstride;
  a.batch = batch; a.cin = cin; a.cout = cout; a.D = D; a.H = H; a.W = W;
  const int tiles = (D / WN_TZ) * (H / WN_TY) * (W / WN_TX);
  MD_HIP_CLEAR_ERROR();
  const dim3 grid((unsigned)(tiles * batch), (unsigned)(cout / 128));
#define WN_LAUNCH(A_) hipLaunchKernelGGL((md_conv3_wino_kernel<A_, false, false, true>), grid, dim3(WN_THREADS), 0, (hipStream_t)stream, a)
  if (variant != 0 && residual == nullptr) return MD_ERR_UNSUPPORTED;
  switch (variant) {
    case 0:
      if (residual) WN_LAUNCH(0);
      else hipLaunchKernelGGL((md_conv3_wino_kernel<0, false, false, false>), grid, dim3(WN_THREADS), 0, (hipStream_t)stream, a);
      break;
#ifdef MD_BUILD_ABLATIONS
    case 1: WN_LAUNCH(1); break;
    case 2: WN_LAUNCH(2); break;
    case 4: WN_LAUNCH(4); break;
    case 6: WN_LAUNCH(6); break;
    case 22: WN_LAUNCH(22); break;
    case 9: WN_LAUNCH(9); break;
    case 16: WN_LAUNCH(16); break;
    case 25: WN_LAUNCH(25); break;
    case 32: WN_LAUNCH(32); break;
    case 64: WN_LAUNCH(64); break;
    case 128: WN_LAUNCH(128); break;
#endif
    default: return MD_ERR_UNSUPPORTED;
  }
#undef WN_LAUNCH
  MD_HIP_CHECK_LAUNCH();
  return MD_OK;
}
```

### meshdiffusion_amd/csrc/wino_prep2.hip

```cpp
#include "md_common.h"

namespace {
constexpr int P2_POS = 256;
constexpr int P2_STRIDE = 12;
constexpr int P2_REGION = (P2_POS / 2) * P2_STRIDE + 16;
constexpr int P2_GROUP = 2 * P2_REGION;
#ifdef P2_OLD_IMAGE
__device__ __forceinline__ int p2_slot(int p) { return p * P2_STRIDE; }
#else
__device__ __forceinline__ int p2_slot(int p) { return (p & 1) * P2_REGION + (p >> 1) * P2_STRIDE; }
#endif
}

template <bool DUAL, bool F8 = false>
__global__ __launch_bounds__(256) void md_wino_prep2_kernel(const float* __restrict__ x1, const float* __restrict__ x2,
                                                            int c1, int c2, const float* __restrict__ ac, int silu, int ups,
                                                            uint4* __restrict__ T, uint4* __restrict__ U, float* __restrict__ sums,
                                                            int batch, int D, int H, int W, uint32_t thr16, float drop_scale,
                                                            uint64_t seed, const float* __restrict__ eq) {
  __shared__ __attribute__((aligned(16))) float act[P2_GROUP];
  __shared__ float wsum[32];
  float psum[8];
  const int tid = threadIdx.x;
  const int Wp = W >> 1;
  const int64_t P = (int64_t)D * H * W, Ph = P >> 1;
  const int CG = (c1 + c2) >> 3;
  const int nblk = (int)(P / P2_POS);
  const int blk = blockIdx.x % nblk;
  const int cg = (blockIdx.x / nblk) % CG;
  const int b = blockIdx.x / (nblk * CG);
  int Di = D, Hi = H, Wi = W;
  if (ups) { Di >>= 1; Hi >>= 1; Wi >>= 1; }
  const int64_t Pin = (int64_t)Di * Hi * Wi;
  const float* src = (cg * 8 < c1) ? x1 + ((int64_t)b * (c1 >> 3) + cg) * Pin * 8
                                   : x2 + ((int64_t)b * (c2 >> 3) + (cg - (c1 >> 3))) * Pin * 8;
  {
    const int64_t p = (int64_t)blk * P2_POS + tid;
    const int x = (int)(p % W), y = (int)((p / W) % H), z = (int)(p / ((int64_t)W * H));
    const int64_t spos = ups ? ((int64_t)(z >> 1) * Hi + (y >> 1)) * Wi + (x >> 1) : p;
    const f32x4* sp = (const f32x4*)(src + spos * 8);
    const f32x4 v0 = sp[0], v1 = sp[1];
    float a[8], c[8];
#pragma unroll
    for (int e = 0; e < 8; ++e) { a[e] = 1.f; c[e] = 0.f; }
    if (ac != nullptr) {
      const f32x4* ap = (const f32x4*)(ac + ((int64_t)b * (c1 + c2) + cg * 8) * 2);
#pragma unroll
      for (int q = 0; q < 4; ++q) {
        const f32x4 v = ap[q];
        a[2 * q] = v[0]; c[2 * q] = v[1]; a[2 * q + 1] = v[2]; c[2 * q + 1] = v[3];
      }
    }
    uint64_t bits[2] = {0, 0};
    if (thr16) {
      const uint64_t quad0 = (uint64_t)(((int64_t)b * (c1 + c2) + cg * 8) >> 2) * (uint64_t)Pin;
      bits[0] = md_drop_bits(seed, quad0 + (uint64_t)spos);
      bits[1] = md_drop_bits(seed, quad0 + (uint64_t)Pin + (uint64_t)spos);
    }
    float yv[8];
#pragma unroll
    for (int e = 0; e < 8; ++e) {
      float t = e < 4 ? v0[e] : v1[e - 4];
      if (ac != nullptr) {
        t = t * a[e] + c[e];
        if (silu) t = t * __builtin_amdgcn_rcpf(1.0f + __builtin_amdgcn_exp2f(t * -1.4426950408889634f));
      }
      if (thr16) t = md_drop_keep(bits[e >> 2], e & 3, thr16) ? t * drop_scale : 0.f;
      yv[e] = t;
    }
    if constexpr (F8) {
      if (eq != nullptr) {
        const f32x4* ep = (const f32x4*)(eq + cg * 8);
        const f32x4 e0 = ep[0], e1 = ep[1];
#pragma unroll
        for (int e = 0; e < 8; ++e) yv[e] *= e < 4 ? e0[e] : e1[e - 4];
      }
    }
#pragma unroll
    for (int e = 0; e < 8; ++e) psum[e] = yv[e];
    float* dst = act + p2_slot(tid);
    *(f32x4*)dst = f32x4{yv[0], yv[1], yv[2], yv[3]};
    *(f32x4*)(dst + 4) = f32x4{yv[4], yv[5], yv[6], yv[7]};
  }
  if constexpr (DUAL) {
    if (sums != nullptr) {
#pragma unroll
      for (int e = 0; e < 8; ++e) {
        float v = psum[e];
        v += __builtin_bit_cast(float, __builtin_amdgcn_update_dpp(0, __builtin_bit_cast(int, v), 0xB1, 0xF, 0xF, true));
        v += __builtin_bit_cast(float, __builtin_amdgcn_update_dpp(0, __builtin_bit_cast(int, v), 0x4E, 0xF, 0xF, true));
        v += __builtin_bit_cast(float, __builtin_amdgcn_update_dpp(0, __builtin_bit_cast(int, v), 0x141, 0xF, 0xF, true));
        v += __builtin_bit_cast(float, __builtin_amdgcn_update_dpp(0, __builtin_bit_cast(int, v), 0x140, 0xF, 0xF, true));
        v += __shfl_xor(v, 16, 64);
        v += __shfl_xor(v, 32, 64);
        if ((tid & 63) == 0) wsum[(tid >> 6) * 8 + e] = v;
      }
    }
  }
  __syncthreads();
  if constexpr (DUAL) {
    if (sums != nullptr && tid < 8)
      atomicAdd(sums + (int64_t)b * (c1 + c2) + cg * 8 + tid, (wsum[tid] + wsum[8 + tid]) + (wsum[16 + tid] + wsum[24 + tid]));
  }
  {
    const int pi = tid & 127, fh = tid >> 7;
    const int lp = 2 * pi;
    const int x = lp % W;
    float d[4][8];
#pragma unroll
    for (int k = 0; k < 4; ++k) {
      const bool need = fh == 0 ? k < 3 : k > 0;
      const int xx = x - 1 + k;
      const bool live = need && xx >= 0 && xx < W;
      f32x4 u0 = {0.f, 0.f, 0.f, 0.f}, u1 = u0;
      if (live) {
        const float* s = act + p2_slot(lp - 1 + k);
        u0 = *(const f32x4*)s; u1 = *(const f32x4*)(s + 4);
      }
#pragma unroll
      for (int e = 0; e < 8; ++e) d[k][e] = e < 4 ? u0[e] : u1[e - 4];
    }
    const int64_t pos2 = ((int64_t)blk * P2_POS >> 1) + pi;
    uint4* out = T + ((int64_t)b * CG + cg) * 8 * Ph + pos2;
#pragma unroll
    for (int g = 0; g < 2; ++g) {
      const int f = 2 * fh + g;
      float t[8];
#pragma unroll
      for (int e = 0; e < 8; ++e)
        t[e] = f == 0 ? d[0][e] - d[2][e] : f == 1 ? d[1][e] + d[2][e] : f == 2 ? d[2][e] - d[1][e] : d[1][e] - d[3][e];
      if constexpr (F8) {
        uint4 hv;
        uint32_t q8[2], ql8[2];
        md_split_f16f8(t, hv, q8, ql8);
        out[(int64_t)(f * 2) * Ph] = hv;
        out[(int64_t)(f * 2 + 1) * Ph] = make_uint4(q8[0], q8[1], ql8[0], ql8[1]);
      } else {
        uint32_t hw[4], lw[4];
#pragma unroll
        for (int q = 0; q < 4; ++q) md_split2(t[2 * q], t[2 * q + 1], hw[q], lw[q]);
        out[(int64_t)(f * 2) * Ph] = make_uint4(hw[0], hw[1], hw[2], hw[3]);
        out[(int64_t)(f * 2 + 1) * Ph] = make_uint4(lw[0], lw[1], lw[2], lw[3]);
      }
    }
    if constexpr (DUAL) {
      uint4* uo = U + ((int64_t)b * CG + cg) * 8 * Ph + pos2;
#pragma unroll
      for (int g = 0; g < 2; ++g) {
        const int f = 2 * fh + g;
        float t[8];
#pragma unroll
        for (int e = 0; e < 8; ++e)
          t[e] = f == 0 ? d[1][e] : f == 1 ? d[1][e] + d[2][e] : f == 2 ? d[1][e] - d[2][e] : d[2][e];
        uint32_t hw[4], lw[4];
#pragma unroll
        for (int q = 0; q < 4; ++q) md_split2(t[2 * q], t[2 * q + 1], hw[q], lw[q]);
        uo[(int64_t)(f * 2) * Ph] = make_uint4(hw[0], hw[1], hw[2], hw[3]);
        uo[(int64_t)(f * 2 + 1) * Ph] = make_uint4(lw[0], lw[1], lw[2], lw[3]);
      }
    }
  }
}

template <bool DUAL>
__global__ __launch_bounds__(256) void md_wino_prep2_f6_kernel(const float* __restrict__ x1, const float* __restrict__ x2, int c1, int c2,
                                                               const float* __restrict__ ac, int silu, int ups, uint4* __restrict__ T, int batch,
                                                               int D, int H, int W, const float* __restrict__ eq, uint4* __restrict__ U,
                                                               float* __restrict__ sums, float tscale, const uint32_t* __restrict__ amax_bits) {
  __shared__ __attribute__((aligned(16))) float act[2 * P2_GROUP];
  __shared__ float wsum[4][16];
  if constexpr (DUAL) {
    if (amax_bits != nullptr) tscale = ldexpf(1.f, md_dgrad_lift_log2(amax_bits[0]));
  }
  const int tid = threadIdx.x;
  const int Wp = W >> 1;
  const int64_t P = (int64_t)D * H * W, Ph = P >> 1;
  const int CG = (c1 + c2) >> 3, CGP = CG >> 1;
  const int nblk = (int)(P / P2_POS);
  const int blk = blockIdx.x % nblk;
  const int cgp = (blockIdx.x / nblk) % CGP;
  const int b = blockIdx.x / (nblk * CGP);
  int Di = D, Hi = H, Wi = W;
  if (ups) { Di >>= 1; Hi >>= 1; Wi >>= 1; }
  const int64_t Pin = (int64_t)Di * Hi * Wi;
  {
    const int64_t p = (int64_t)blk * P2_POS + tid;
    const int x = (int)(p % W), y = (int)((p / W) % H), z = (int)(p / ((int64_t)W * H));
    const int64_t spos = ups ? ((int64_t)(z >> 1) * Hi + (y >> 1)) * Wi + (x >> 1) : p;
#pragma unroll
    for (int g2 = 0; g2 < 2; ++g2) {
      const int cg = 2 * cgp + g2;
      const float* src = (cg * 8 < c1) ? x1 + ((int64_t)b * (c1 >> 3) + cg) * Pin * 8
                                       : x2 + ((int64_t)b * (c2 >> 3) + (cg - (c1 >> 3))) * Pin * 8;
      const f32x4* sp = (const f32x4*)(src + spos * 8);
      const f32x4 v0 = sp[0], v1 = sp[1];
      float a[8], c[8];
#pragma unroll
      for (int e = 0; e < 8; ++e) { a[e] = 1.f; c[e] = 0.f; }
      if (ac != nullptr) {
        const f32x4* ap = (const f32x4*)(ac + ((int64_t)b * (c1 + c2) + cg * 8) * 2);
#pragma unroll
        for (int q = 0; q < 4; ++q) {
          const f32x4 v = ap[q];
          a[2 * q] = v[0]; c[2 * q] = v[1]; a[2 * q + 1] = v[2]; c[2 * q + 1] = v[3];
        }
      }
      float yv[8];
#pragma unroll
      for (int e = 0; e < 8; ++e) {
        float t = e < 4 ? v0[e] : v1[e - 4];
        if (ac != nullptr) {
          t = t * a[e] + c[e];
          if (silu) t = t * __builtin_amdgcn_rcpf(1.0f + __builtin_amdgcn_exp2f(t * -1.4426950408889634f));
        }
        yv[e] = t;
      }
      if (eq != nullptr) {
        const f32x4* ep = (const f32x4*)(eq + cg * 8);
        const f32x4 e0 = ep[0], e1 = ep[1];
#pragma unroll
        for (int e = 0; e < 8; ++e) yv[e] *= e < 4 ? e0[e] : e1[e - 4];
      }
      float* dst = act + g2 * P2_GROUP + p2_slot(tid);
      *(f32x4*)dst = f32x4{yv[0], yv[1], yv[2], yv[3]};
      *(f32x4*)(dst + 4) = f32x4{yv[4], yv[5], yv[6], yv[7]};
      if constexpr (DUAL) {
        if (sums != nullptr) {
#pragma unroll
          for (int e = 0; e < 8; ++e) {
            const float v = md_wave_sum(yv[e]);
            if ((tid & 63) == 0) wsum[tid >> 6][g2 * 8 + e] = v;
          }
        }
      }
    }
  }
  __syncthreads();
  if constexpr (DUAL) {
    if (sums != nullptr && tid < 16)
      atomicAdd(sums + (int64_t)b * (c1 + c2) + cgp * 16 + tid, (wsum[0][tid] + wsum[1][tid]) + (wsum[2][tid] + wsum[3][tid]));
  }
  {
    const int pi = tid & 127, fh = tid >> 7;
    const int lp = 2 * pi;
    const int x = lp % W;
    float d[4][16];
#pragma unroll
    for (int k = 0; k < 4; ++k) {
      const bool need = fh == 0 ? k < 3 : k > 0;
      const int xx = x - 1 + k;
      const bool live = need && xx >= 0 && xx < W;
#pragma unroll
      for (int g2 = 0; g2 < 2; ++g2) {
        f32x4 u0 = {0.f, 0.f, 0.f, 0.f}, u1 = u0;
        if (live) {
          const float* sv = act + g2 * P2_GROUP + p2_slot(lp - 1 + k);
          u0 = *(const f32x4*)sv; u1 = *(const f32x4*)(sv + 4);
        }
#pragma unroll
        for (int e = 0; e < 8; ++e) d[k][g2 * 8 + e] = e < 4 ? u0[e] : u1[e - 4];
      }
    }
    const int64_t pos2 = ((int64_t)blk * P2_POS >> 1) + pi;
    uint4* out0 = T + ((int64_t)b * CG + 2 * cgp) * 8 * Ph + pos2;
    uint4* out1 = out0 + 8 * Ph;
#pragma unroll
    for (int g = 0; g < 2; ++g) {
      const int f = 2 * fh + g;
      float t[16];
#pragma unroll
      for (int e = 0; e < 16; ++e) {
        t[e] = f == 0 ? d[0][e] - d[2][e] : f == 1 ? d[1][e] + d[2][e] : f == 2 ? d[2][e] - d[1][e] : d[1][e] - d[3][e];
        if constexpr (DUAL) t[e] = __builtin_isfinite(t[e]) ? fminf(fmaxf(t[e] * tscale, -60000.f), 60000.f) : t[e];
      }
      uint4 h0, h1, r0, r1;
      md_split_f16f6(t, false, 0, h0, h1, r0, r1);
      out0[(int64_t)(f * 2) * Ph] = h0;
      out1[(int64_t)(f * 2) * Ph] = h1;
      out0[(int64_t)(f * 2 + 1) * Ph] = r0;
      out1[(int64_t)(f * 2 + 1) * Ph] = r1;
    }
    if constexpr (DUAL) {
      uint4* uo0 = U + ((int64_t)b * CG + 2 * cgp) * 8 * Ph + pos2;
      uint4* uo1 = uo0 + 8 * Ph;
#pragma unroll
      for (int g = 0; g < 2; ++g) {
        const int f = 2 * fh + g;
#pragma unroll
        for (int g2 = 0; g2 < 2; ++g2) {
          uint32_t hw[4], lw[4];
#pragma unroll
          for (int q = 0; q < 4; ++q) {
            const int e0 = g2 * 8 + 2 * q;
            const float ta = f == 0 ? d[1][e0] : f == 1 ? d[1][e0] + d[2][e0] : f == 2 ? d[1][e0] - d[2][e0] : d[2][e0];
            const float tb = f == 0 ? d[1][e0 + 1] : f == 1 ? d[1][e0 + 1] + d[2][e0 + 1] : f == 2 ? d[1][e0 + 1] - d[2][e0 + 1] : d[2][e0 + 1];
            md_split2(ta, tb, hw[q], lw[q]);
          }
          uint4* uo = g2 ? uo1 : uo0;
          uo[(int64_t)(f * 2) * Ph] = make_uint4(hw[0], hw[1], hw[2], hw[3]);
          uo[(int64_t)(f * 2 + 1) * Ph] = make_uint4(lw[0], lw[1], lw[2], lw[3]);
        }
      }
    }
  }
}

static int md_wino_prep2_launch(const float* x1, const float* x2, int32_t c1, int32_t c2, const float* ac, int32_t silu,
                                int32_t ups, void* t_out, void* u_out, float* sums, int32_t batch, int32_t D, int32_t H, int32_t W, float drop_p,
                                uint64_t drop_seed, void* stream, bool f8 = false, const float* eq = nullptr) {
  if (!x1 || !t_out || batch <= 0 || c1 <= 0 || c2 < 0 || (c1 & 7) || (c2 & 7) || (c2 > 0 && !x2)) return MD_ERR_BAD_ARG;
  if (silu && !ac) return MD_ERR_BAD_ARG;
  if (D <= 0 || H <= 0 || W <= 0 || (W & 1) || (ups && ((D | H | W) & 1))) return MD_ERR_BAD_ARG;
  if (!(drop_p >= 0.f && drop_p < 1.f) || (drop_p > 0.f && (ups || c2 > 0))) return MD_ERR_BAD_ARG;
  const int64_t P = (int64_t)D * H * W;
  if ((P2_POS % W) || (P % P2_POS)) return MD_ERR_UNSUPPORTED;
  const int64_t blocks = (int64_t)batch * ((c1 + c2) / 8) * (P / P2_POS);
  if (blocks > 0x7fffffff) return MD_ERR_UNSUPPORTED;
  MD_HIP_CLEAR_ERROR();
  if (f8)
    hipLaunchKernelGGL((md_wino_prep2_kernel<false, true>), dim3((unsigned)blocks), dim3(256), 0, (hipStream_t)stream, x1, x2, c1, c2, ac,
                       silu, ups, (uint4*)t_out, (uint4*)nullptr, (float*)nullptr, batch, D, H, W, md_drop_thr16(drop_p),
                       1.0f / (1.0f - drop_p), drop_seed, eq);
  else if (u_out)
    hipLaunchKernelGGL((md_wino_prep2_kernel<true>), dim3((unsigned)blocks), dim3(256), 0, (hipStream_t)stream, x1, x2, c1, c2, ac,
                       silu, ups, (uint4*)t_out, (uint4*)u_out, sums, batch, D, H, W, md_drop_thr16(drop_p), 1.0f / (1.0f - drop_p),
                       drop_seed, (const float*)nullptr);
  else
    hipLaunchKernelGGL((md_wino_prep2_kernel<false>), dim3((unsigned)blocks), dim3(256), 0, (hipStream_t)stream, x1, x2, c1, c2, ac,
                       silu, ups, (uint4*)t_out, (uint4*)nullptr, (float*)nullptr, batch, D, H, W, md_drop_thr16(drop_p),
                       1.0f / (1.0f - drop_p), drop_seed, (const float*)nullptr);
  MD_HIP_CHECK_LAUNCH();
  return MD_OK;
}

extern "C" int md_wino_prep_v2(const float* x1, const float* x2, int32_t c1, int32_t c2, const float* ac, int32_t silu,
                               int32_t ups, void* t_out, int32_t batch, int32_t D, int32_t H, int32_t W, float drop_p,
                               uint64_t drop_seed, void* stream) {
  return md_wino_prep2_launch(x1, x2, c1, c2, ac, silu, ups, t_out, nullptr, nullptr, batch, D, H, W, drop_p, drop_seed, stream);
}

extern "C" int md_wino_prep_dual(const float* x1, const float* x2, int32_t c1, int32_t c2, const float* ac, int32_t silu,
                                 int32_t ups, void* t_out, void* u_out, float* sums, int32_t batch, int32_t D, int32_t H,
                                 int32_t W, float drop_p, uint64_t drop_seed, void* stream) {
  if (!u_out || (sums && ups)) return MD_ERR_BAD_ARG;
  return md_wino_prep2_launch(x1, x2, c1, c2, ac, silu, ups, t_out, u_out, sums, batch, D, H, W, drop_p, drop_seed, stream);
}


extern "C" int md_wino_prep_f8(const float* x1, const float* x2, int32_t c1, int32_t c2, const float* ac, int32_t silu,
                               int32_t ups, const float* eq, void* t_out, int32_t batch, int32_t D, int32_t H, int32_t W, void* stream) {
  return md_wino_prep2_launch(x1, x2, c1, c2, ac, silu, ups, t_out, nullptr, nullptr, batch, D, H, W, 0.f, 0, stream, true, eq);
}

extern "C" int md_wino_prep_f6(const float* x1, const float* x2, int32_t c1, int32_t c2, const float* ac, int32_t silu,
                               int32_t ups, const float* eq, void* t_out, int32_t batch, int32_t D, int32_t H, int32_t W, void* stream) {
  if (!x1 || !t_out || batch <= 0 || c1 <= 0 || c2 < 0 || (c1 & 15) || (c2 & 15) || (c2 > 0 && !x2)) return MD_ERR_BAD_ARG;
  if (silu && !ac) return MD_ERR_BAD_ARG;
  if (D <= 0 || H <= 0 || W <= 0 || (W & 1) || (ups && ((D | H | W) & 1))) return MD_ERR_BAD_ARG;
  const int64_t P = (int64_t)D * H * W;
  if ((P2_POS % W) || (P % P2_POS)) return MD_ERR_UNSUPPORTED;
  const int64_t blocks = (int64_t)batch * ((c1 + c2) / 16) * (P / P2_POS);
  if (blocks > 0x7fffffff) return MD_ERR_UNSUPPORTED;
  MD_HIP_CLEAR_ERROR();
  hipLaunchKernelGGL(md_wino_prep2_f6_kernel<false>, dim3((unsigned)blocks), dim3(256), 0, (hipStream_t)stream, x1, x2, c1, c2, ac, silu, ups,
                     (uint4*)t_out, batch, D, H, W, eq, (uint4*)nullptr, (float*)nullptr, 1.0f, (const uint32_t*)nullptr);
  MD_HIP_CHECK_LAUNCH();
  return MD_OK;
}

extern "C" int md_wino_prep_dual_f6(const float* x, int32_t c, void* t_out, void* u_out, float* sums, float tscale, const uint32_t* amax_bits,
                                    int32_t batch, int32_t D, int32_t H, int32_t W, void* stream) {
  if (!x || !t_out || !u_out || batch <= 0 || c <= 0 || (c & 15)) return MD_ERR_BAD_ARG;
  if (D <= 0 || H <= 0 || W <= 0 || (W & 1) || (!amax_bits && !(tscale > 0.f))) return MD_ERR_BAD_ARG;
  const int64_t P = (int64_t)D * H * W;
  if ((P2_POS % W) || (P % P2_POS)) return MD_ERR_UNSUPPORTED;
  const int64_t blocks = (int64_t)batch * (c / 16) * (P / P2_POS);
  if (blocks > 0x7fffffff) return MD_ERR_UNSUPPORTED;
  MD_HIP_CLEAR_ERROR();
  hipLaunchKernelGGL(md_wino_prep2_f6_kernel<true>, dim3((unsigned)blocks), dim3(256), 0, (hipStream_t)stream, x, (const float*)nullptr, c, 0,
                     (const float*)nullptr, 0, 0, (uint4*)t_out, batch, D, H, W, (const float*)nullptr, (uint4*)u_out, sums, tscale, amax_bits);
  MD_HIP_CHECK_LAUNCH();
  return MD_OK;
}
```

### meshdiffusion_amd/hip_ops.py

```python
import ctypes as C
import math
import os

import torch

from . import _lib
from ._lib import (A_PACKED, A_S16B, PREC_BF16X3, PREC_FP16X2, CFG_C3_128, CFG_C3_128_V2, CFG_C3_128_SW, CFG_C3_128_PIPE, CFG_C3_128_FAST, CFG_C5_128_K16, CFG_C5_32_K16, CFG_C3_128_W4, CFG_C3X_32, CFG_C5X_32_K16, CFG_C3X_128_K16, CFG_C5X_128, CFG_G1_128_N128, CFG_C3_128_K16, CFG_C3_32, CFG_C3_LOW, CFG_C3_S2,
                   CFG_G1_128, CFG_G1_128_LOW, CFG_G1_64_LOW, CFG_NT_KC, OUT_F32B, OUT_NCDHW, OUT_S16B,
                   MdGemmConvArgs, check)


CFG_ABL1, CFG_ABL2, CFG_ABL3, CFG_ABL4, CFG_ABL5 = 101, 102, 103, 104, 105
CFG_F1, CFG_F3, CFG_F4, CFG_F6, CFG_F7, CFG_F8 = 111, 113, 114, 116, 117, 118
CFG_FAST_EC = 122
CONV_STAGGER = int(os.environ.get("MD_CONV_STAGGER", "0"))
DEBUG_ACT_FP16 = 2 if os.environ.get("MD_DEBUG_ACT_FP16") == "1" else 0
_MODES = ("bf16x3", "fp16x2", "f16f8", "f16f6")
DEFAULT_PRECISION = os.environ.get("MD_PRECISION", "bf16x3")
FORCE_PRECISION = os.environ.get("MD_FORCE_PRECISION")
WINO_EQ = os.environ.get("MD_WINO_EQ", "1") == "1"
F8_RAW = os.environ.get("MD_F8_RAW", "0") == "1"


def _decode(mode):
    if mode not in _MODES:
        raise ValueError(f"unknown precision mode {mode!r}")
    return ("bf16x3", mode[3:]) if mode in ("f16f8", "f16f6") else (mode, False)


PRECISION, WINO_F8 = _decode(DEFAULT_PRECISION)
TRAINING_SCOPE = False
_SCOPES = []


def set_precision(mode):
    global DEFAULT_PRECISION, PRECISION, WINO_F8
    _decode(mode)
    DEFAULT_PRECISION = mode
    if not _SCOPES:
        PRECISION, WINO_F8 = _decode(mode)


class precision_scope:

    def __init__(self, mode, training=False):
        if training:
            mode = "bf16x3"
        else:
            mode = FORCE_PRECISION or mode or DEFAULT_PRECISION
        self.state = _decode(mode) + (bool(training),)

    def __enter__(self):
        global PRECISION, WINO_F8, TRAINING_SCOPE
        _SCOPES.append((PRECISION, WINO_F8, TRAINING_SCOPE))
        PRECISION, WINO_F8, TRAINING_SCOPE = self.state
        return self

    def __exit__(self, *exc):
        global PRECISION, WINO_F8, TRAINING_SCOPE
        PRECISION, WINO_F8, TRAINING_SCOPE = _SCOPES.pop()
        return False


def precision_name():
    return ("f16" + WINO_F8) if (WINO_F8 and PRECISION == "bf16x3") else PRECISION


def fast_prec(cfg):
    return PREC_FP16X2 if (PRECISION == "fp16x2" and cfg == CFG_C3_128_FAST) else PREC_BF16X3


PARAM_EPOCH = 0


def bump_param_epoch():
    global PARAM_EPOCH
    PARAM_EPOCH += 1


NIN_SIDE_STREAM = os.environ.get("MD_NIN_SIDE_STREAM", "0") == "1"
_SIDE = {}


def side_stream():
    dev = torch.cuda.current_device()
    if dev not in _SIDE:
        _SIDE[dev] = torch.cuda.Stream(device=dev)
    return _SIDE[dev]


PROFILE = None
AUDIT = None


def _stream():
    return C.c_void_p(torch.cuda.current_stream().cuda_stream)


def _ptr(t):
    return C.c_void_p(t.data_ptr()) if t is not None else C.c_void_p(0)


def _require_cuda(t, name):
    if not t.is_cuda:
        raise _lib.MeshDiffusionHipError(f"{name} must live on the GPU: the HIP path has no CPU fallback")


def f32b_empty(B, Cc, P, device):
    return torch.empty((B, Cc // 8, P, 8), dtype=torch.float32, device=device)


def s16b_empty(B, Cc, P, device):
    return torch.empty((B, Cc // 8, 2, P, 8), dtype=torch.bfloat16, device=device)


class PackedWeight:

    def __init__(self, w, kind, cfg, device, prec=PREC_BF16X3):
        self.prec = prec
        nt, kc = CFG_NT_KC[cfg]
        w = w.detach().to(device=device, dtype=torch.float32).contiguous()
        _require_cuda(w, "weight")
        base_off = 0
        if kind == "conv":
            rows, kdim, taps = w.shape[0], w.shape[1], w.shape[2] * w.shape[3] * w.shape[4]
            s_row, s_k, s_tap = kdim * taps, taps, 1
        elif kind == "conv_dgrad":
            taps = w.shape[2] * w.shape[3] * w.shape[4]
            rows, kdim = w.shape[1], w.shape[0]
            s_row, s_k, s_tap = taps, rows * taps, -1
            base_off = taps - 1
        elif kind == "nin":
            rows, kdim, taps = w.shape[1], w.shape[0], 1
            s_row, s_k, s_tap = 1, rows, 0
        elif kind == "rows":
            rows, kdim, taps = w.shape[0], w.shape[1], 1
            s_row, s_k, s_tap = kdim, 1, 0
        else:
            raise ValueError(kind)
        self.rows, self.taps, self.cfg = rows, taps, cfg
        self.kdim = ((kdim + kc - 1) // kc) * kc
        self._src = (w, rows, kdim, taps, s_row, s_k, s_tap, nt, kc, base_off)
        self._data = None
        self._queued = False

    def request(self):
        if self._data is None and not self._queued:
            lib = _lib.load()
            w, rows, kdim, taps, s_row, s_k, s_tap, nt, kc, base_off = self._src
            nbytes = lib.md_packed_weight_bytes(rows, kdim, taps, nt, kc)
            if nbytes <= 0:
                raise _lib.MeshDiffusionHipError("md_packed_weight_bytes failed")
            self._queued = True
            _PACK_QUEUE.append((self, dict(kind=_lib.PACK_WPK, w=w, w_off=4 * base_off, nbytes=nbytes, rows=rows, kdim=kdim, taps=taps,
                                           s_row=s_row, s_k=s_k, s_tap=s_tap, nt=nt, kc=kc, prec=self.prec, flip=0)))

    @property
    def data(self):
        if self._data is None:
            self.request()
            flush_packs()
            if self._data is None:
                raise _lib.MeshDiffusionHipError("packed weight requested but not produced by flush_packs()")
        return self._data


_PACK_QUEUE = []
PACK_BATCH = os.environ.get("MD_PACK_BATCH", "1") == "1"
PACK_TILED = os.environ.get("MD_PACK_TILED", "1") == "1"


def flush_packs():
    global _PACK_QUEUE
    if not _PACK_QUEUE:
        return
    queue, _PACK_QUEUE = _PACK_QUEUE, []
    try:
        _flush(queue)
    except BaseException:
        for owner, _ in queue:
            if owner._data is None:
                owner._queued = False
        raise


def _flush(queue):
    lib = _lib.load()
    outs = []
    for owner, j in queue:
        outs.append(torch.empty(j["nbytes"] // 2, dtype=torch.bfloat16, device=j["w"].device))
    if PACK_BATCH and len(queue) > 1 and len({j["w"].device for _, j in queue}) == 1:
        def tiled(j):
            return (PACK_TILED and j["kind"] == _lib.PACK_WPK and j["taps"] > 1 and abs(j["s_tap"]) == 1
                    and 16 * j["kc"] * j["taps"] <= 13824 and j["nt"] % 16 == 0)

        def mode(j):
            if j["kind"] == _lib.PACK_WINO_F6:
                return 0
            if PACK_TILED and j["kind"] == _lib.PACK_WINO:
                return 3
            if not tiled(j):
                return 0
            m = j["taps"] * 100 + j["kc"]
            return m if m in (2732, 2716, 932, 916) else 1

        for md in sorted({mode(j) for _, j in queue}, reverse=True):
            sel = [(j, out) for (owner, j), out in zip(queue, outs) if mode(j) == md]
            jobs = (_lib.MdPackJob * len(sel))()
            block0 = 0
            for i, (j, out) in enumerate(sel):
                J = jobs[i]
                J.w, J.out = j["w"].data_ptr() + j["w_off"], out.data_ptr()
                J.s_row, J.s_k, J.s_tap = j["s_row"], j["s_k"], j["s_tap"]
                J.n_items, J.block0 = j["nbytes"] // 16, block0
                J.rows, J.kdim, J.taps, J.nt, J.kc, J.prec, J.flip, J.kind = (j["rows"], j["kdim"], j["taps"], j["nt"], j["kc"],
                                                                             j["prec"], j["flip"], j["kind"])
                if md == 3:
                    block0 += (j["rows"] // 32) * (j["kdim"] // 16)
                elif md:
                    block0 += -(-j["rows"] // j["nt"]) * (j["nt"] // 16) * -(-j["kdim"] // j["kc"])
                else:
                    block0 += (J.n_items + 255) // 256
            table = torch.frombuffer(bytearray(bytes(jobs)), dtype=torch.uint8).to(outs[0].device)
            check(lib.md_pack_batch(_ptr(table), len(sel), block0, md, _stream()), "md_pack_batch")
    else:
        for (owner, j), out in zip(queue, outs):
            wp = C.c_void_p(j["w"].data_ptr() + j["w_off"])
            if j["kind"] == _lib.PACK_WPK:
                check(lib.md_pack_weights(wp, _ptr(out), j["rows"], j["kdim"], j["taps"], j["s_row"], j["s_k"], j["s_tap"], j["nt"],
                                          j["kc"], j["prec"], _stream()), "md_pack_weights")
            elif j["kind"] == _lib.PACK_WINO_F6:
                jobs = (_lib.MdPackJob * 1)()
                J = jobs[0]
                J.w, J.out = j["w"].data_ptr() + j["w_off"], out.data_ptr()
                J.s_row, J.s_k, J.s_tap, J.n_items, J.block0 = j["s_row"], j["s_k"], 0, j["nbytes"] // 16, 0
                J.rows, J.kdim, J.taps, J.nt, J.kc, J.prec, J.flip, J.kind = j["rows"], j["kdim"], 9, 0, 0, j["prec"], j["flip"], j["kind"]
                table = torch.frombuffer(bytearray(bytes(jobs)), dtype=torch.uint8).to(out.device)
                check(lib.md_pack_batch(_ptr(table), 1, (J.n_items + 255) // 256, 0, _stream()), "md_pack_batch")
            else:
                check(lib.md_wino_pack_weights(wp, _ptr(out), j["rows"], j["kdim"], j["s_row"], j["s_k"], j["flip"], _stream()),
                      "md_wino_pack_weights")
    for (owner, j), out in zip(queue, outs):
        owner._data = out
        owner._src = None
        owner._queued = False


import weakref

_PACK_LAYERS = weakref.WeakSet()


def note_pack_use(layer, name, params, builder):
    used = layer.__dict__.get("_md_used")
    if used is None:
        used = layer.__dict__["_md_used"] = {}
        _PACK_LAYERS.add(layer)
    if name not in used:
        used[name] = (list(params), builder)


def prewarm_packs():
    layers = list(_PACK_LAYERS)
    _PACK_LAYERS.clear()
    n = 0
    for layer in layers:
        used = layer.__dict__.pop("_md_used", None) or {}
        if not PACK_BATCH:
            continue
        cache = layer.__dict__.get("_md_cache") or {}
        for name, (params, builder) in used.items():
            old = cache.get(name)
            consumed = old is not None and getattr(old[1], "_data", None) is not None
            obj = layer._cached(name, params, builder, mark=False)
            if consumed and hasattr(obj, "request"):
                obj.request()
                n += 1
    flush_packs()
    return n


def pack_s16b_from_matrix(w_kp, device):
    lib = _lib.load()
    w = w_kp.detach().to(device=device, dtype=torch.float32).contiguous()
    K, P = w.shape
    out = s16b_empty(1, K, P, device)
    check(lib.md_ncdhw_to_s16b(_ptr(w), _ptr(out), 1, K, K, P, _stream()), "md_ncdhw_to_s16b")
    return out


def gemm_conv(*, cfg, a, b, out, batch, rows, rows_alloc, kdim, dims, bias=None, bias_bstride=0,
              residual=None, res_bstride=0, alpha=1.0, ups=0, a_src=A_PACKED, a_rows=0, a_bstride=0,
              b_bstride=None, out_mode=OUT_F32B, ksplit=1, prec=PREC_BF16X3, stats=None, stagger=None,
              b_f32=None):
    lib = _lib.load()
    D, H, W = dims
    args = MdGemmConvArgs()
    args.a, args.out = a.data_ptr(), out.data_ptr()
    if b_f32 is not None:
        parts = b_f32["parts"]
        assert 1 <= len(parts) <= 2 and sum(c for _, c in parts) == kdim and all(c % 8 == 0 for _, c in parts)
        pin = D * H * W // (8 if ups else 1)
        args.b, args.b_split = parts[0][0].data_ptr(), parts[0][1]
        b_bstride = parts[0][1] * pin
        if len(parts) == 2:
            args.b2, args.b2_bstride = parts[1][0].data_ptr(), parts[1][1] * pin
        ac = b_f32.get("ac")
        args.b_ac = ac.data_ptr() if ac is not None else None
        args.b_silu = 1 if b_f32.get("silu") else 0
        args.b_mode = _lib.B_F32B_GN
    else:
        args.b = b.data_ptr()
    args.bias = bias.data_ptr() if bias is not None else None
    args.residual = residual.data_ptr() if residual is not None else None
    args.alpha = alpha
    args.cfg, args.batch, args.rows, args.rows_alloc, args.kdim = cfg, batch, rows, rows_alloc, kdim
    args.D, args.H, args.W, args.ups = D, H, W, ups
    args.a_src, args.out_mode, args.a_rows = a_src, out_mode, a_rows
    args.a_bstride, args.bias_bstride, args.res_bstride = a_bstride, bias_bstride, res_bstride
    if b_bstride is None:
        pin = D * H * W
        if ups:
            pin //= 8
        elif cfg == CFG_C3_S2:
            pin *= 8
        b_bstride = (kdim // 8) * 2 * pin * 8
    args.b_bstride = b_bstride
    args.prec = prec
    args.stats = stats.data_ptr() if stats is not None else None
    args.stagger = CONV_STAGGER if stagger is None else int(stagger)
    part = None
    if ksplit > 1:
        if out_mode != OUT_F32B:
            raise ValueError("split-K supports F32B output only")
        args.ksplit = ksplit
        part = torch.empty((ksplit * batch * rows_alloc * D * H * W,), dtype=torch.float32, device=out.device)
        args.partial = part.data_ptr()
    if PROFILE is None:
        check(lib.md_gemm_conv(C.byref(args), _stream()), f"md_gemm_conv(cfg={cfg})")
    else:
        taps = _lib.cfg_info(cfg)["taps"]
        flops = 2.0 * batch * rows * kdim * taps * D * H * W
        pin = D * H * W // (8 if ups else 1) * (8 if cfg == CFG_C3_S2 else 1)
        abytes = 4.0 * (batch * kdim * pin + rows * kdim * taps + batch * rows * D * H * W * (2 if residual is not None else 1))
        e0, e1 = torch.cuda.Event(enable_timing=True), torch.cuda.Event(enable_timing=True)
        e0.record()
        check(lib.md_gemm_conv(C.byref(args), _stream()), f"md_gemm_conv(cfg={cfg})")
        e1.record()
        PROFILE.append((cfg, flops, e0, e1, abytes,
                        f"{kdim}->{rows}@{D}x{H}x{W}" + ("/ups" if ups else "") + (f"/ks{ksplit}" if ksplit > 1 else "") +
                        ("/res" if residual is not None else "") + ("/stats" if stats is not None else "")))
    return out


WINO = os.environ.get("MD_WINO", "1") == "1"
WINO_PREP_V2 = os.environ.get("MD_WINO_PREP_V2", "1") == "1"
WINO_TRAIN_FWD = os.environ.get("MD_WINO_TRAIN_FWD", "1") == "1"


class WinoWeight:

    def __init__(self, w, device, kind="conv"):
        lib = _lib.load()
        w = w.detach().to(device=device, dtype=torch.float32).contiguous()
        _require_cuda(w, "weight")
        assert w.dim() == 5 and tuple(w.shape[2:]) == (3, 3, 3)
        if kind == "conv":
            self.rows, self.kdim = w.shape[0], w.shape[1]
            s_row, s_k, flip = self.kdim * 27, 27, 0
        elif kind == "conv_dgrad":
            self.rows, self.kdim = w.shape[1], w.shape[0]
            s_row, s_k, flip = 27, self.rows * 27, 1
        else:
            raise ValueError(kind)
        nbytes = lib.md_wino_weight_bytes(self.rows, self.kdim)
        if nbytes <= 0:
            raise _lib.MeshDiffusionHipError("md_wino_weight_bytes: unsupported weight shape")
        self._data, self._queued = None, False
        self._src = dict(kind=_lib.PACK_WINO, w=w, w_off=0, nbytes=nbytes, rows=self.rows, kdim=self.kdim, taps=9, s_row=s_row,
                         s_k=s_k, s_tap=0, nt=0, kc=0, prec=PREC_BF16X3, flip=flip)

    def request(self):
        if self._data is None and not self._queued:
            self._queued = True
            _PACK_QUEUE.append((self, self._src))

    @property
    def data(self):
        if self._data is None:
            self.request()
            flush_packs()
            if self._data is None:
                raise _lib.MeshDiffusionHipError("packed weight requested but not produced by flush_packs()")
        return self._data


class WinoWeightF8:

    def __init__(self, w, device, fmt="f8", eq=None):
        lib = _lib.load()
        w = w.detach().to(device=device, dtype=torch.float32).contiguous()
        _require_cuda(w, "weight")
        assert w.dim() == 5 and tuple(w.shape[2:]) == (3, 3, 3) and fmt in ("f8", "f6")
        self.rows, self.kdim, self.fmt = w.shape[0], w.shape[1], fmt
        assert eq is None or (eq.is_cuda and eq.dtype == torch.float32 and eq.numel() == self.kdim and eq.is_contiguous())
        self.eq = eq
        nbytes = lib.md_wino_weight_bytes_f8(self.rows, self.kdim)
        if nbytes <= 0:
            raise _lib.MeshDiffusionHipError("md_wino_weight_bytes_f8: unsupported weight shape")
        self.data = torch.empty(nbytes // 2, dtype=torch.bfloat16, device=device)
        pack = lib.md_wino_pack_weights_f6 if fmt == "f6" else lib.md_wino_pack_weights_f8
        check(pack(_ptr(w), _ptr(eq), _ptr(self.data), self.rows, self.kdim, self.kdim * 27, 27, _stream()), "md_wino_pack_weights_" + fmt)


DGRAD_F6 = os.environ.get("MD_DGRAD_F6", "1") == "1"
DGRAD_LIFT = os.environ.get("MD_DGRAD_LIFT", "dyn")
DGRAD_TSCALE = 2.0 ** int(DGRAD_LIFT) if DGRAD_LIFT != "dyn" else 64.0
DGRAD_WSCALE_LOG2 = 8
_AMAX_SLOTS = {}


def amax_slot(device):
    device = torch.device(device)
    key = (device.index, torch.cuda.current_stream(device).cuda_stream)
    arena = _AMAX_SLOTS.get(key)
    if arena is None or arena[1] >= arena[0].numel():
        arena = _AMAX_SLOTS[key] = [torch.zeros(1024, dtype=torch.int32, device=device), 0]
    word = arena[0][arena[1]:arena[1] + 1]
    arena[1] += 1
    return word


def absmax_word(x):
    lib = _lib.load()
    word = amax_slot(x.device)
    check(lib.md_absmax(_ptr(x), x.numel(), _ptr(word), _stream()), "md_absmax")
    return word


class WinoWeightF6Dgrad:
    fmt, eq = "f6", None

    def __init__(self, w, device):
        lib = _lib.load()
        w = w.detach().to(device=device, dtype=torch.float32).contiguous()
        _require_cuda(w, "weight")
        assert w.dim() == 5 and tuple(w.shape[2:]) == (3, 3, 3)
        self.rows, self.kdim = w.shape[1], w.shape[0]
        nbytes = lib.md_wino_weight_bytes_f8(self.rows, self.kdim)
        if nbytes <= 0:
            raise _lib.MeshDiffusionHipError("md_wino_weight_bytes_f8: unsupported weight shape")
        self._data, self._queued = None, False
        self._src = dict(kind=_lib.PACK_WINO_F6, w=w, w_off=0, nbytes=nbytes, rows=self.rows, kdim=self.kdim, taps=9, s_row=27,
                         s_k=self.rows * 27, s_tap=0, nt=0, kc=0, prec=DGRAD_WSCALE_LOG2, flip=1)

    request = WinoWeight.request
    data = WinoWeight.data


def wino_equaliser(gamma, beta, w, a2m=None):
    lib = _lib.load()
    w = w.detach().to(dtype=torch.float32).contiguous()
    _require_cuda(w, "weight")
    cout, cin = w.shape[0], w.shape[1]
    assert w.dim() == 5 and tuple(w.shape[2:]) == (3, 3, 3)
    assert (gamma is None) == (beta is None) and (gamma is not None or a2m is not None)
    if gamma is not None:
        gamma = gamma.detach().to(device=w.device, dtype=torch.float32).contiguous()
        beta = beta.detach().to(device=w.device, dtype=torch.float32).contiguous()
        assert gamma.numel() == cin and beta.numel() == cin
    eq = torch.empty(cin, dtype=torch.float32, device=w.device)
    if a2m is not None:
        assert a2m.is_cuda and a2m.dtype == torch.float32 and a2m.numel() == cin and a2m.is_contiguous()
        check(lib.md_wino_equaliser_measured(_ptr(gamma), _ptr(beta), _ptr(w), _ptr(a2m), cout, cin, cin * 27, 27, _ptr(eq), _stream()),
              "md_wino_equaliser_measured")
    else:
        check(lib.md_wino_equaliser(_ptr(gamma), _ptr(beta), _ptr(w), cout, cin, cin * 27, 27, _ptr(eq), _stream()), "md_wino_equaliser")
    return eq


CALIBRATE = None


def wino_operand_ms(parts, ac, silu, B, P):
    lib = _lib.load()
    assert 1 <= len(parts) <= 2
    cin = sum(c for _, c in parts)
    x2, c2 = (parts[1][0], parts[1][1]) if len(parts) == 2 else (None, 0)
    ms = torch.zeros(cin, dtype=torch.float32, device=parts[0][0].device)
    check(lib.md_wino_operand_ms(_ptr(parts[0][0]), _ptr(x2), parts[0][1], c2, _ptr(ac), 1 if silu else 0, B, P, _ptr(ms), _stream()),
          "md_wino_operand_ms")
    return ms


WINO_MIN_WGS = int(os.environ.get("MD_WINO_MIN_WGS", "128"))
WINO_MIN_WGS_TRAIN = int(os.environ.get("MD_WINO_MIN_WGS_TRAIN", "256"))


def wino_ok(rows, kdim, S, B):
    return (WINO and PRECISION == "bf16x3" and rows % 128 == 0 and kdim % 32 == 0 and S % 8 == 0
            and B * (S ** 3 // 256) * (rows // 128) >= (max(WINO_MIN_WGS, WINO_MIN_WGS_TRAIN) if TRAINING_SCOPE else WINO_MIN_WGS))


WGRAD_NIN = os.environ.get("MD_WGRAD_NIN", "1") == "1"


def wgrad_nin_ok(co, ci, P):
    return WGRAD_NIN and co % 128 == 0 and ci % 128 == 0 and P % 16 == 0


def wgrad_nin(dy_s16, x_s16, B, co, ci, P, dw):
    lib = _lib.load()
    units = (co // 128) * (ci // 128)
    ksplit = max(1, min(256 // units, B * P // 16 // 8))
    nbytes = lib.md_wgrad_nin_workspace_bytes(co, ci, ksplit)
    if nbytes <= 0:
        raise _lib.MeshDiffusionHipError("md_wgrad_nin_workspace_bytes: unsupported shape")
    ws = torch.empty(nbytes // 4, dtype=torch.float32, device=dy_s16.device)
    ev = _prof_begin()
    check(lib.md_wgrad_nin(_ptr(dy_s16), _ptr(x_s16), _ptr(dw), _ptr(ws), nbytes, B, co, ci, P, ksplit, 1, co, _stream()),
          "md_wgrad_nin")
    _prof_end(ev, "wgrad_nin", 2.0 * B * co * ci * P, 4.0 * B * (co + ci) * P, f"{ci}->{co}@{P}")


_WINO_SCRATCH = {}


def _wino_scratch(n_bf16, device, slot="t"):
    key = (device.type, device.index, torch.cuda.current_stream(device).cuda_stream, slot)
    buf = _WINO_SCRATCH.get(key)
    if buf is None or buf.numel() < n_bf16:
        _WINO_SCRATCH.pop(key, None)
        buf = None
        buf = _WINO_SCRATCH[key] = torch.empty(n_bf16, dtype=torch.bfloat16, device=device)
    return buf[:n_bf16]


def release_scratch():
    _WINO_SCRATCH.clear()


def wino_f8_ok(S, drop=None, keep=False, parts=None, normalised=True):
    if not (WINO_F8 and PRECISION == "bf16x3" and not drop and not keep and 256 % S == 0 and (normalised or F8_RAW)):
        return False
    if WINO_F8 == "f6" and parts is not None and any(c % 16 for _, c in parts):
        return "f8"
    return WINO_F8


def wino_prep(parts, ac, silu, ups, B, S, drop=None, keep=False, dual=False, sums=None, f8=False, eq=None, tscale=1.0, amax=None, dims=None):
    lib = _lib.load()
    D, H, W = dims if dims is not None else (S, S, S)
    cin = sum(c for _, c in parts)
    assert 1 <= len(parts) <= 2
    assert eq is None or (f8 and eq.numel() == cin and eq.dtype == torch.float32 and eq.is_cuda), "eq belongs to the f16f8 / f16f6 operand"
    assert ac is not None or not silu, "SiLU is applied together with the folded GroupNorm affine (pass `ac`)"
    nbytes = lib.md_wino_operand_bytes(B, cin, D, H, W)
    if nbytes <= 0:
        raise _lib.MeshDiffusionHipError("md_wino_operand_bytes: unsupported operand shape")
    dev = parts[0][0].device
    t = torch.empty(nbytes // 2, dtype=torch.bfloat16, device=dev) if keep else _wino_scratch(nbytes // 2, dev)
    x2, c2 = (parts[1][0], parts[1][1]) if len(parts) == 2 else (None, 0)
    ev = _prof_begin()
    args = (_ptr(parts[0][0]), _ptr(x2), parts[0][1], c2, _ptr(ac), 1 if silu else 0, 1 if ups else 0)
    tail = (B, D, H, W, drop[0] if drop else 0.0, drop[1] if drop else 0, _stream())
    if f8 and dual:
        assert f8 == "f6" and len(parts) == 1 and ac is None and not (ups or keep or drop or eq is not None) and 256 % W == 0
        u = _wino_scratch(nbytes // 2, dev, slot="u")
        check(lib.md_wino_prep_dual_f6(_ptr(parts[0][0]), cin, _ptr(t), _ptr(u), _ptr(sums), float(tscale), _ptr(amax), B, D, H, W, _stream()),
              "md_wino_prep_dual_f6")
    elif f8:
        assert not (dual or keep or drop), "the f16f8 / f16f6 operand is an inference format"
        if f8 == "f6":
            check(lib.md_wino_prep_f6(*args, _ptr(eq), _ptr(t), B, D, H, W, _stream()), "md_wino_prep_f6")
        else:
            check(lib.md_wino_prep_f8(*args, _ptr(eq), _ptr(t), B, D, H, W, _stream()), "md_wino_prep_f8")
    elif dual:
        if 256 % W:
            raise _lib.MeshDiffusionHipError("md_wino_prep_dual needs W | 256")
        u = _wino_scratch(nbytes // 2, dev, slot="u")
        check(lib.md_wino_prep_dual(*args, _ptr(t), _ptr(u), _ptr(sums), *tail), "md_wino_prep_dual")
    else:
        fn = lib.md_wino_prep_v2 if (WINO_PREP_V2 and 256 % W == 0 and (D * H * W) % 256 == 0) else lib.md_wino_prep
        check(fn(*args, _ptr(t), *tail), "md_wino_prep")
    _prof_end(ev, "wino_prep", 0.0, 4.0 * B * cin * (D * H * W // (8 if ups else 1)) + (16.0 if dual else 8.0) * B * cin * D * H * W,
              f"{cin}@{D}x{H}x{W}" + ("/ups" if ups else "") + ("/dual" if dual else "") + (("/f6" if f8 == "f6" else "/f8") if f8 else ""))
    t._md_fmt = ("f6" if f8 == "f6" else "f8") if f8 else False
    t._md_eq = eq.data_ptr() if eq is not None else 0
    return (t, u) if dual else t


WGRAD_WINO = os.environ.get("MD_WGRAD_WINO", "1") == "1"


def wgrad_wino_ok(co, ci, S, B):
    return WGRAD_WINO and WINO_TRAIN_FWD and S in (32, 64) and co % 128 == 0 and ci % 128 == 0 and wino_ok(co, ci, S, B)


def wgrad_wino(u_dy, t_act, B, co, ci, S, dw):
    lib = _lib.load()
    units = (co // 128) * (ci // 128) * 12
    ksplit = max(1, min(256 // units, B * (S - 1)))
    nbytes = lib.md_wgrad_wino_workspace_bytes(co, ci, ksplit)
    if nbytes <= 0:
        raise _lib.MeshDiffusionHipError("md_wgrad_wino_workspace_bytes: unsupported shape")
    ws = torch.empty(nbytes // 4, dtype=torch.float32, device=u_dy.device)
    ev = _prof_begin()
    check(lib.md_wgrad_wino(_ptr(u_dy), _ptr(t_act), _ptr(dw), _ptr(ws), nbytes, B, co, ci, S, S, S, ksplit, ci * 27, 27, 1,
                            _stream()), "md_wgrad_wino")
    _prof_end(ev, "wgrad_wino", 2.0 * B * co * ci * 27 * S ** 3, 16.0 * B * (co + ci) * S ** 3 / 2, f"{ci}->{co}@{S}x{S}x{S}")


WINO_VARIANT = int(os.environ.get("MD_WINO_VARIANT", "0"))


def conv3_wino(ww, t, B, S, *, bias=None, bias_bstride=0, residual=None, res_bstride=0, stats=None, out=None, variant=None, out_scale=1.0,
               amax=None, dims=None):
    lib = _lib.load()
    D, H, W = dims if dims is not None else (S, S, S)
    P = D * H * W
    if out is None:
        out = f32b_empty(B, ww.rows, P, t.device)
    ev = _prof_begin()
    f8 = isinstance(ww, (WinoWeightF8, WinoWeightF6Dgrad))
    t_fmt = getattr(t, "_md_fmt", None)
    if t_fmt is not None:
        want = ww.fmt if f8 else False
        if t_fmt != want or getattr(t, "_md_eq", 0) != ((ww.eq.data_ptr() if ww.eq is not None else 0) if f8 else 0):
            raise _lib.MeshDiffusionHipError(f"conv3_wino: operand format {t_fmt!r} / equaliser does not belong to these weights ({want!r})")
    if f8 and (out_scale != 1.0 or amax is not None):
        assert ww.fmt == "f6"
        check(lib.md_conv3_wino_f6_scaled(_ptr(t), _ptr(ww.data), _ptr(out), _ptr(bias), bias_bstride, _ptr(residual), res_bstride,
                                          _ptr(stats), B, ww.kdim, ww.rows, D, H, W, float(out_scale), _ptr(amax), _stream()),
              "md_conv3_wino_f6_scaled")
    elif f8:
        fn = lib.md_conv3_wino_f6 if ww.fmt == "f6" else lib.md_conv3_wino_f8
        check(fn(_ptr(t), _ptr(ww.data), _ptr(out), _ptr(bias), bias_bstride, _ptr(residual), res_bstride,
                 _ptr(stats), B, ww.kdim, ww.rows, D, H, W, _stream()), "md_conv3_wino_" + ww.fmt)
    else:
        check(lib.md_conv3_wino(_ptr(t), _ptr(ww.data), _ptr(out), _ptr(bias), bias_bstride, _ptr(residual), res_bstride,
                                _ptr(stats), B, ww.kdim, ww.rows, D, H, W, WINO_VARIANT if variant is None else variant, _stream()),
              "md_conv3_wino")
    _prof_end(ev, "wino", 2.0 * B * ww.rows * ww.kdim * 27 * P,
              4.0 * (2 * B * ww.kdim * P + ww.rows * ww.kdim * 36 + B * ww.rows * P * (2 if residual is not None else 1)),
              f"{ww.kdim}->{ww.rows}@{D}x{H}x{W}" + ("/res" if residual is not None else "") + ("/stats" if stats is not None else "")
              + (("/" + ww.fmt) if f8 else ""))
    return out


CONV3_S2 = os.environ.get("MD_CONV3_S2", "1") == "1"
CFG_S2_PACK = CFG_C3_128_K16


S2_MIN_WGS = int(os.environ.get("MD_S2_MIN_WGS", "100"))


def conv3_s2_ok(rows, kdim, S_out, B=None):
    ok = CONV3_S2 and PRECISION == "bf16x3" and kdim % 32 == 0 and rows % 8 == 0 and S_out % 8 == 0
    return ok and (B is None or B * (S_out ** 3 // 256) * ((rows + 127) // 128) >= S2_MIN_WGS)


def conv3_s2(pw, x, B, S_out, *, bias=None, bias_bstride=0, stats=None, out=None, dims=None):
    lib = _lib.load()
    D, H, W = dims if dims is not None else (S_out, S_out, S_out)
    P = D * H * W
    rows_alloc = ((pw.rows + 7) // 8) * 8
    if out is None:
        out = f32b_empty(B, rows_alloc, P, x.device)
    ev = _prof_begin()
    check(lib.md_conv3_s2(_ptr(x), _ptr(pw.data), _ptr(out), _ptr(bias), bias_bstride, _ptr(stats), B, pw.kdim, pw.rows,
                          rows_alloc, D, H, W, _stream()), "md_conv3_s2")
    _prof_end(ev, "s2", 2.0 * B * pw.rows * pw.kdim * 27 * P, 4.0 * (B * pw.kdim * 8 * P + pw.rows * pw.kdim * 27 + B * pw.rows * P),
              f"{pw.kdim}->{pw.rows}@{D}x{H}x{W}" + ("/stats" if stats is not None else ""))
    return out


CONV3_STEM = os.environ.get("MD_CONV3_STEM", "1") == "1"


def conv3_stem_ok(rows, kdim, S):
    return CONV3_STEM and PRECISION == "bf16x3" and kdim == 16 and rows % 8 == 0 and S % 8 == 0


def conv3_stem(pw, x16, B, S, *, bias=None, residual=None, stats=None, dims=None):
    lib = _lib.load()
    D, H, W = dims if dims is not None else (S, S, S)
    P = D * H * W
    out = f32b_empty(B, pw.rows, P, x16.device)
    ev = _prof_begin()
    check(lib.md_conv3_stem(_ptr(x16), _ptr(pw.data), _ptr(out), _ptr(bias), _ptr(residual), _ptr(stats), B, pw.rows, D, H, W,
                            _stream()), "md_conv3_stem")
    _prof_end(ev, "stem", 2.0 * B * pw.rows * pw.kdim * 9 * P, 4.0 * (B * pw.kdim * P + pw.rows * pw.kdim * 9 + B * pw.rows * P),
              f"{pw.kdim}->{pw.rows}@{D}x{H}x{W}" + ("/res" if residual is not None else "") + ("/stats" if stats is not None else ""))
    return out


CONV3_HEAD = os.environ.get("MD_CONV3_HEAD", "1") == "1"
CFG_HEAD_PACK = CFG_C5X_32_K16


def conv3_head_ok(rows, cin, S):
    return CONV3_HEAD and FUSE_GN_APPLY and PRECISION == "bf16x3" and rows <= 32 and cin % 32 == 0 and S % 8 == 0


def conv3_head(pw, x, ac, B, S, rows_alloc, dims=None):
    lib = _lib.load()
    D, H, W = dims if dims is not None else (S, S, S)
    P = D * H * W
    y = f32b_empty(B, rows_alloc, P, x.device)
    ev = _prof_begin()
    check(lib.md_conv3_head(_ptr(x), _ptr(ac), _ptr(pw.data), _ptr(y), B, pw.kdim, rows_alloc, D, H, W, _stream()), "md_conv3_head")
    _prof_end(ev, "head", 2.0 * B * pw.rows * pw.kdim * 9 * P, 4.0 * (B * pw.kdim * P + pw.rows * pw.kdim * 9 + B * rows_alloc * P),
              f"{pw.kdim}->{pw.rows}@{D}x{H}x{W}")
    return y


def _prof_begin():
    if PROFILE is None:
        return None
    e0 = torch.cuda.Event(enable_timing=True)
    e0.record()
    return e0


def _prof_end(e0, cfg, flops, abytes, tag):
    if e0 is None:
        return
    e1 = torch.cuda.Event(enable_timing=True)
    e1.record()
    PROFILE.append((cfg, flops, e0, e1, abytes, tag))


FUSE_GN_APPLY = os.environ.get("MD_FUSE_GN_APPLY", "1") == "1"
FUSE_GN_STATS = True
SPLITK_STATS = os.environ.get("MD_SPLITK_STATS", "1") == "1"


STATS_ARENA = os.environ.get("MD_STATS_ARENA", "1") == "1"
_STATS_ARENAS = {}
_STATS_ARENA_DOUBLES = 1 << 20


def stats_arena_reset(device):
    if not STATS_ARENA:
        return
    a = _STATS_ARENAS.get(device)
    if a is None:
        return
    if a["off"] > 0:
        a["buf"][:a["off"]].zero_()
    a["off"] = 0


def stats_zeros(B, rows, device):
    n = B * rows * 2
    if not STATS_ARENA or n > _STATS_ARENA_DOUBLES // 4:
        return torch.zeros((B, rows, 2), dtype=torch.float64, device=device)
    device = torch.device(device)
    if device.index is None:
        device = torch.device("cuda", torch.cuda.current_device())
    a = _STATS_ARENAS.get(device)
    if a is None or a["off"] + n > _STATS_ARENA_DOUBLES:
        a = _STATS_ARENAS[device] = dict(buf=torch.zeros(_STATS_ARENA_DOUBLES, dtype=torch.float64, device=device), off=0)
    out = a["buf"][a["off"]:a["off"] + n].view(B, rows, 2)
    a["off"] += (n + 15) & ~15
    return out


def gn_params(parts, gamma, beta, B, P, eps=1e-6, groups=32, want_ac=False):
    lib = _lib.load()
    dev = parts[0][0].device
    ctot = sum(c for _, c in parts)
    cached = [getattr(t, "_md_sums", None) if FUSE_GN_STATS else None for t, _ in parts]
    if len(parts) == 1 and cached[0] is not None:
        sums = cached[0]
    else:
        sums = stats_zeros(B, ctot, dev) if any(c is None for c in cached) else torch.empty((B, ctot, 2), dtype=torch.float64, device=dev)
        off = 0
        for (t, c), cs in zip(parts, cached):
            if cs is not None:
                sums[:, off:off + c] = cs
            else:
                check(lib.md_gn_stats(_ptr(t), _ptr(sums), B, c, P, ctot, off, _stream()), "md_gn_stats")
            off += c
    params = torch.empty((B, ctot, 4), dtype=torch.float32, device=dev)
    ac = torch.empty((B, ctot, 2), dtype=torch.float32, device=dev) if want_ac else None
    check(lib.md_gn_finalize(_ptr(sums), _ptr(gamma), _ptr(beta), _ptr(params), B, ctot, groups, P,
                             eps, _ptr(ac), _stream()), "md_gn_finalize")
    return (params, ac) if want_ac else params


def next_dropout_seed():
    return int(torch.randint(0, 2 ** 62, (1,), dtype=torch.int64).item())


def dropout_scale(B, C, P, p, seed, device):
    lib = _lib.load()
    out = f32b_empty(B, C, P, device)
    check(lib.md_dropout_scale(_ptr(out), B, C, P, C, 0, float(p), int(seed), _stream()), "md_dropout_scale")
    return out


def gn_apply(parts, params, B, P, norm=True, silu=True, out=None, fp16=False, want_raw=False, drop=None):
    dp, dseed = (float(drop[0]), int(drop[1])) if drop else (0.0, 0)
    lib = _lib.load()
    dev = parts[0][0].device
    ctot = sum(c for _, c in parts)
    if out is None:
        out = s16b_empty(B, ctot, P, dev)
    raw = s16b_empty(B, ctot, P, dev) if want_raw else None
    off = 0
    for t, c in parts:
        check(lib.md_gn_apply(_ptr(t), _ptr(params) if norm else None, _ptr(out), _ptr(raw), B, c, P, ctot, off,
                              1 if norm else 0, (1 if silu else 0) | DEBUG_ACT_FP16 | (4 if fp16 else 0), dp, dseed,
                              _stream()),
              "md_gn_apply")
        off += c
    return (out, raw) if want_raw else out


def fold_dx(y, bias, B, co, kx, rows_alloc, S, out=None, dims=None):
    lib = _lib.load()
    D, H, W = dims if dims is not None else (S, S, S)
    if out is None:
        out = torch.empty((B, co, D, H, W), dtype=torch.float32, device=y.device)
    check(lib.md_fold_dx(_ptr(y), _ptr(bias), _ptr(out), B, co, kx, rows_alloc, D, H, W, _stream()), "md_fold_dx")
    return out


def timestep_embedding(t, dim):
    lib = _lib.load()
    _require_cuda(t, "timesteps")
    t = t.to(torch.float32).contiguous()
    emb = torch.empty((t.shape[0], dim), dtype=torch.float32, device=t.device)
    check(lib.md_timestep_embedding(_ptr(t), _ptr(emb), t.shape[0], dim, _stream()), "md_timestep_embedding")
    return emb


def linear(x, w, bias, silu_in=False):
    lib = _lib.load()
    B, in_dim = x.shape
    out_dim = w.shape[0]
    y = torch.empty((B, out_dim), dtype=torch.float32, device=x.device)
    check(lib.md_linear(_ptr(x), _ptr(w), _ptr(bias), _ptr(y), B, in_dim, out_dim, 1 if silu_in else 0,
                        _stream()), "md_linear")
    return y


def ncdhw_to_s16b(x, c_pad):
    lib = _lib.load()
    _require_cuda(x, "x")
    x = x.to(torch.float32).contiguous()
    B, Cc = x.shape[0], x.shape[1]
    P = x[0, 0].numel()
    out = s16b_empty(B, c_pad, P, x.device)
    check(lib.md_ncdhw_to_s16b(_ptr(x), _ptr(out), B, Cc, c_pad, P, _stream()), "md_ncdhw_to_s16b")
    return out


def ncdhw_to_s16b_xfold(x, kx, c_pad):
    lib = _lib.load()
    _require_cuda(x, "x")
    x = x.to(torch.float32).contiguous()
    B, Cc, D, H, W = x.shape
    out = s16b_empty(B, c_pad, D * H * W, x.device)
    check(lib.md_ncdhw_to_s16b_xfold(_ptr(x), _ptr(out), B, Cc, kx, c_pad, D, H, W, _stream()), "md_ncdhw_to_s16b_xfold")
    return out


def ncdhw_to_f32b(x):
    lib = _lib.load()
    _require_cuda(x, "x")
    x = x.to(torch.float32).contiguous()
    B, Cc = x.shape[0], x.shape[1]
    P = x[0, 0].numel()
    out = f32b_empty(B, Cc, P, x.device)
    check(lib.md_ncdhw_to_f32b(_ptr(x), _ptr(out), B, Cc, P, _stream()), "md_ncdhw_to_f32b")
    return out


def f32b_to_ncdhw(x, spatial):
    lib = _lib.load()
    B, CG, P, _ = x.shape
    out = torch.empty((B, CG * 8) + tuple(spatial), dtype=torch.float32, device=x.device)
    check(lib.md_f32b_to_ncdhw(_ptr(x), _ptr(out), B, CG * 8, P, _stream()), "md_f32b_to_ncdhw")
    return out


def s16b_to_ncdhw(x, spatial):
    lib = _lib.load()
    B, CG, _, P, _ = x.shape
    out = torch.empty((B, CG * 8) + tuple(spatial), dtype=torch.float32, device=x.device)
    check(lib.md_s16b_to_ncdhw(_ptr(x), _ptr(out), B, CG * 8, P, _stream()), "md_s16b_to_ncdhw")
    return out


NIN_STREAM = os.environ.get("MD_NIN_STREAM", "1") == "1"


def nin_stream_ok(parts, rows, P):
    k = sum(c for _, c in parts)
    return (NIN_STREAM and rows == 128 and k in (128, 256) and len(parts) <= 2 and all(c % 16 == 0 for _, c in parts)
            and P % 256 == 0 and P >= 32768)


def nin_f32(parts, pw, bias, B, P, out=None):
    lib = _lib.load()
    if out is None:
        out = f32b_empty(B, 128, P, parts[0][0].device)
    x2, c2 = (parts[1][0], parts[1][1]) if len(parts) == 2 else (None, 0)
    check(lib.md_nin_f32(_ptr(parts[0][0]), _ptr(x2), parts[0][1], c2, _ptr(pw.data), _ptr(bias), _ptr(out), B, 128, P, 0,
                         _stream()), "md_nin_f32")
    return out


FUSE_ATTN = os.environ.get("MD_FUSE_ATTN", "1") == "1"


def attn_fused_ok(Cc, n_tokens):
    return FUSE_ATTN and Cc == 256 and n_tokens % 128 == 0


def attn_fwd(qk, vT, bias_v, B, Cc, n_tokens, scale):
    lib = _lib.load()
    o = s16b_empty(B, Cc, n_tokens, qk.device)
    check(lib.md_attn_fwd(_ptr(qk), _ptr(vT), _ptr(o), _ptr(bias_v), B, Cc, n_tokens, float(scale), _stream()), "md_attn_fwd")
    return o


def softmax_keys(s, B, nk, nq):
    lib = _lib.load()
    p = torch.empty((B, nk // 8, 2, nq, 8), dtype=torch.bfloat16, device=s.device)
    check(lib.md_softmax_keys(_ptr(s), _ptr(p), B, nk, nq, _stream()), "md_softmax_keys")
    return p


def ancestral_step(x, eps, z, mask, coef):
    lib = _lib.load()
    for name, t in (("x", x), ("eps", eps), ("z", z)):
        _require_cuda(t, name)
    x, eps, z = x.contiguous(), eps.contiguous(), z.contiguous()
    B, Cc = x.shape[0], x.shape[1]
    P = x[0, 0].numel()
    x_out, xm_out = torch.empty_like(x), torch.empty_like(x)
    check(lib.md_ancestral_step(_ptr(x), _ptr(eps), _ptr(z), _ptr(mask), _ptr(coef), _ptr(x_out),
                                _ptr(xm_out), B, Cc, P, _stream()), "md_ancestral_step")
    return x_out, xm_out


def langevin_step(x, eps, z, mask, coef, snr, mode="langevin"):
    lib = _lib.load()
    for name, t in (("x", x), ("eps", eps), ("z", z), ("coef", coef)):
        _require_cuda(t, name)
    x, eps, z, coef = x.contiguous(), eps.contiguous(), z.contiguous(), coef.contiguous()
    B, Cc = x.shape[0], x.shape[1]
    P = x[0, 0].numel()
    assert coef.dtype == torch.float32 and coef.shape == (B, 3), coef.shape
    kind = {"langevin": _lib.CORRECTOR_LANGEVIN, "ald": _lib.CORRECTOR_ALD}[mode]
    x_out, xm_out = torch.empty_like(x), torch.empty_like(x)
    step = torch.empty(B, dtype=torch.float32, device=x.device)
    slabs = None
    if kind == _lib.CORRECTOR_LANGEVIN:
        slabs = torch.empty((B, _lib.LANGEVIN_SLABS, 2), dtype=torch.float64, device=x.device)
        check(lib.md_langevin_norms(_ptr(eps), _ptr(z), B, Cc, P, _ptr(slabs), _stream()), "md_langevin_norms")
    check(lib.md_langevin_step(_ptr(x), _ptr(eps), _ptr(z), _ptr(mask), _ptr(coef), _ptr(slabs), float(snr), kind,
                               _ptr(x_out), _ptr(xm_out), _ptr(step), B, Cc, P, _stream()), "md_langevin_step")
    return x_out, xm_out, step


def sde_step(x, eps, z, mask, coef, kind):
    lib = _lib.load()
    for name, t in (("x", x), ("eps", eps), ("z", z), ("coef", coef)):
        _require_cuda(t, name)
    x, eps, z, coef = x.contiguous(), eps.contiguous(), z.contiguous(), coef.contiguous()
    B, Cc = x.shape[0], x.shape[1]
    P = x[0, 0].numel()
    assert coef.dtype == torch.float32 and coef.shape == (B, 5), coef.shape
    k = {"reverse_diffusion": _lib.SDE_REVERSE_DIFFUSION, "euler_maruyama": _lib.SDE_EULER_MARUYAMA}[kind]
    x_out, xm_out = torch.empty_like(x), torch.empty_like(x)
    check(lib.md_sde_step(_ptr(x), _ptr(eps), _ptr(z), _ptr(mask), _ptr(coef), k, _ptr(x_out), _ptr(xm_out), B, Cc, P,
                          _stream()), "md_sde_step")
    return x_out, xm_out


def ddim_step(x64, eps, mask, coef, partial=None, pmask=None, ch=0):
    lib = _lib.load()
    for name, t in (("x", x64), ("eps", eps)):
        _require_cuda(t, name)
    assert x64.dtype == torch.float64 and eps.dtype == torch.float32 and coef.dtype == torch.float64
    x64, eps, coef = x64.contiguous(), eps.contiguous(), coef.contiguous()
    B, Cc = x64.shape[0], x64.shape[1]
    P = x64[0, 0].numel()
    x_out, x0_out = torch.empty_like(x64), torch.empty_like(x64)
    x_f32 = torch.empty_like(eps)
    check(lib.md_ddim_step(_ptr(x64), _ptr(eps), _ptr(mask), _ptr(coef), _ptr(partial), _ptr(pmask), int(ch), _ptr(x_out),
                           _ptr(x0_out), _ptr(x_f32), B, Cc, P, _stream()), "md_ddim_step")
    return x_out, x0_out, x_f32


def inpaint_blend_(x, src, pmask, gmask, ch, src_bstride=0):
    lib = _lib.load()
    B, Cc = x.shape[0], x.shape[1]
    P = x[0, 0].numel()
    check(lib.md_inpaint_blend(_ptr(x), _ptr(src), _ptr(pmask), _ptr(gmask), B, Cc, ch, P, src_bstride,
                               _stream()), "md_inpaint_blend")
    return x


def inpaint_renoise_(x, x_mean, z, pmask, gmask, coef, ch):
    lib = _lib.load()
    B, Cc = x.shape[0], x.shape[1]
    P = x[0, 0].numel()
    check(lib.md_inpaint_renoise(_ptr(x), _ptr(x_mean), _ptr(z), _ptr(pmask), _ptr(gmask), _ptr(coef), B, Cc,
                                 ch, P, _stream()), "md_inpaint_renoise")
    return x


def ksplit_for(cfg, batch, rows, kdim, spatial_out):
    info = _lib.cfg_info(cfg)
    tiles = max(1, spatial_out ** 3 // info["cols"]) * batch * ((rows + info["nt"] - 1) // info["nt"])
    ncc = kdim // info["kc"]
    ks = 1
    while tiles * ks < 256 and ks * 2 <= ncc and ks < 32:
        ks *= 2
    return ks


def conv_cfg_for(spatial, stride=1):
    if stride == 2:
        return CFG_C3_S2
    return CFG_C3_128_FAST if spatial % 8 == 0 else CFG_C3_LOW


NIN_N128 = os.environ.get("MD_NIN_N128", "1") == "1"


def gemm_cfg_for(ncols, nrows, hbm_bound=False):
    if hbm_bound and NIN_N128 and ncols % 128 == 0 and ncols >= 32768:
        return CFG_G1_128_N128
    if ncols % 256 == 0:
        return CFG_G1_128
    return CFG_G1_128_LOW if nrows % 128 == 0 else CFG_G1_64_LOW


def attn_scale(channels):
    return float(int(channels) ** (-0.5))


__all__ = [n for n in dir() if not n.startswith("_")]
_ = math
```

### meshdiffusion_amd/lib/diffusion/models/layers.py

```python
import math

import numpy as np
import torch
import torch.nn as nn

from .... import hip_ops as ops


def variance_scaling(scale, mode, distribution, in_axis=1, out_axis=0, dtype=torch.float32, device="cpu"):
    def init(shape, dtype=dtype, device=device):
        receptive = np.prod(shape) / shape[in_axis] / shape[out_axis]
        fan_in, fan_out = shape[in_axis] * receptive, shape[out_axis] * receptive
        denom = {"fan_in": fan_in, "fan_out": fan_out, "fan_avg": (fan_in + fan_out) / 2}[mode]
        var = scale / denom
        if distribution == "normal":
            return torch.randn(*shape, dtype=dtype, device=device) * np.sqrt(var)
        if distribution == "uniform":
            return (torch.rand(*shape, dtype=dtype, device=device) * 2.0 - 1.0) * np.sqrt(3 * var)
        raise ValueError("invalid distribution for variance scaling initializer")

    return init


def default_init(scale=1.0):
    return variance_scaling(1e-10 if scale == 0 else scale, "fan_avg", "uniform")


def get_act(config):
    name = config.model.nonlinearity.lower()
    if name == "swish":
        return nn.SiLU()
    raise NotImplementedError("only the 'swish' nonlinearity is implemented on the HIP path "
                              "(both registered reference models use it)")


def _conv(in_planes, out_planes, k, stride=1, padding=1, init_scale=1.0):
    conv = nn.Conv3d(in_planes, out_planes, kernel_size=k, stride=stride, padding=padding, bias=True)
    conv.weight.data = default_init(init_scale)(conv.weight.data.shape)
    nn.init.zeros_(conv.bias)
    return conv


def ddpm_conv3x3(in_planes, out_planes, stride=1, bias=True, dilation=1, init_scale=1.0, padding=1):
    assert bias and dilation == 1
    return _conv(in_planes, out_planes, 3, stride, padding, init_scale)


def ddpm_conv5x5(in_planes, out_planes, stride=2, bias=True, dilation=1, init_scale=1.0, padding=2):
    assert bias and dilation == 1
    return _conv(in_planes, out_planes, 5, stride, padding, init_scale)


def get_timestep_embedding(timesteps, embedding_dim, max_positions=10000):
    assert len(timesteps.shape) == 1 and max_positions == 10000
    return ops.timestep_embedding(timesteps, embedding_dim)


class HipLayer(nn.Module):

    def _cached(self, name, params, builder, mark=True):
        cache = self.__dict__.setdefault("_md_cache", {})
        key = (ops.PARAM_EPOCH,) + tuple((p.data_ptr(), p._version, str(p.device)) for p in params)
        hit = cache.get(name)
        if hit is None or hit[0] != key:
            hit = (key, builder())
            cache[name] = hit
        if mark:
            ops.note_pack_use(self, name, params, builder)
        return hit[1]


def _spatial_edge(P):
    s = round(P ** (1.0 / 3.0))
    assert s * s * s == P, "cubic grids only"
    return s


def _parts_of(x):
    B, Cc = x.shape[0], x.shape[1]
    spatial = tuple(x.shape[2:])
    return [(ops.ncdhw_to_f32b(x), Cc)], B, int(np.prod(spatial)), spatial


def conv3_packed(layer, name, conv, cfg):
    prec = ops.fast_prec(cfg)
    return layer._cached(f"{name}/p{prec}", [conv.weight],
                         lambda: ops.PackedWeight(conv.weight, "conv", cfg, conv.weight.device, prec))


def conv3_wino_packed(layer, name, conv, gn=None):
    def measured():
        return layer.__dict__.get("_md_act_ms", {}).get(name)

    def eq():
        ms = measured() if ops.WINO_EQ else None
        if ms is None and not (gn is not None and ops.WINO_EQ):
            return None
        gp = [gn.weight, gn.bias] if gn is not None else []
        if ms is None:
            return layer._cached(f"{name}/wino_eq", [conv.weight] + gp, lambda: ops.wino_equaliser(gn.weight, gn.bias, conv.weight), mark=False)
        return layer._cached(f"{name}/wino_eqm", [conv.weight] + gp + [ms],
                             lambda: ops.wino_equaliser(gn.weight if gn is not None else None, gn.bias if gn is not None else None,
                                                        conv.weight, a2m=ms), mark=False)

    def build(f8=False):
        if f8:
            fmt = "f6" if f8 == "f6" else "f8"
            ms = measured() if ops.WINO_EQ else None
            use_eq = ms is not None or (gn is not None and ops.WINO_EQ)
            deps = [conv.weight] + ([gn.weight, gn.bias] if (use_eq and gn is not None) else []) + ([ms] if ms is not None else [])
            return layer._cached(f"{name}/wino_{fmt}{('m' if ms is not None else 'e') if use_eq else ''}", deps,
                                 lambda: ops.WinoWeightF8(conv.weight, conv.weight.device, fmt, eq=eq()), mark=False)
        return layer._cached(f"{name}/wino", [conv.weight], lambda: ops.WinoWeight(conv.weight, conv.weight.device))
    build.eq, build.measured = eq, measured
    build.owner, build.site = layer, name
    return build


def fused_operand_ok(pw, ups=0):
    cfgs = (ops.CFG_C3_128_FAST,) if ups else (ops.CFG_C3_128_FAST, ops.CFG_C3_LOW)
    return ops.FUSE_GN_APPLY and pw.cfg in cfgs and pw.prec == ops.PREC_BF16X3


def run_conv3(pw, act_s16, B, S_out, *, bias=None, bias_bstride=0, residual=None, res_bstride=None, ups=0,
              out=None, out_mode=ops.OUT_F32B, rows_alloc=None, want_stats=False, b_f32=None, wino=None):
    P = S_out ** 3
    dev = act_s16.device if act_s16 is not None else b_f32["parts"][0][0].device
    rows_alloc = rows_alloc if rows_alloc is not None else ((pw.rows + 7) // 8) * 8
    if out is None:
        out = ops.f32b_empty(B, rows_alloc, P, dev)
    if residual is not None and res_bstride is None:
        res_bstride = rows_alloc * P
    if (b_f32 is not None and wino is not None and out_mode == ops.OUT_F32B and rows_alloc == pw.rows
            and pw.prec == ops.PREC_BF16X3 and ops.wino_ok(pw.rows, pw.kdim, S_out, B)):
        stats = ops.stats_zeros(B, rows_alloc, dev) if want_stats and ops.FUSE_GN_STATS else None
        owner = getattr(wino, "owner", None)
        if ops.CALIBRATE is not None and owner is not None and not b_f32.get("wino_only"):
            ms = ops.wino_operand_ms(b_f32["parts"], b_f32.get("ac"), b_f32.get("silu"), B, b_f32["parts"][0][0].shape[2])
            rec = ops.CALIBRATE.setdefault((id(owner), wino.site), [owner, wino.site, torch.zeros_like(ms), 0])
            rec[2] += ms
            rec[3] += 1
        f8 = (not b_f32.get("wino_only")) and ops.wino_f8_ok(
            S_out, drop=b_f32.get("drop"), keep=bool(b_f32.get("keep")), parts=b_f32["parts"],
            normalised=b_f32.get("ac") is not None
            or (ops.WINO_EQ and hasattr(wino, "measured") and wino.measured() is not None))
        if f8 and owner is not None and wino.site in getattr(owner, "md_bf16x3_sites", ()):
            f8 = False
        t = ops.wino_prep(b_f32["parts"], b_f32.get("ac"), b_f32.get("silu"), ups, B, S_out, drop=b_f32.get("drop"),
                          keep=bool(b_f32.get("keep")), f8=f8, eq=wino.eq() if f8 and hasattr(wino, "eq") else None)
        if b_f32.get("keep"):
            b_f32["t_out"] = t
        ops.conv3_wino(wino(f8) if f8 else wino(), t, B, S_out, bias=bias, bias_bstride=bias_bstride, residual=residual,
                       res_bstride=res_bstride or 0, stats=stats, out=out)
        if f8 and ops.AUDIT is not None:
            t3 = ops.wino_prep(b_f32["parts"], b_f32.get("ac"), b_f32.get("silu"), ups, B, S_out)
            ref = ops.conv3_wino(wino(), t3, B, S_out, bias=bias, bias_bstride=bias_bstride, residual=residual, res_bstride=res_bstride or 0)
            ops.AUDIT.append(dict(owner=getattr(wino, "owner", None), site=getattr(wino, "site", None), fmt=f8, cin=pw.kdim, cout=pw.rows,
                                  S=S_out, rel_l2=float((torch.linalg.vector_norm(out - ref, dtype=torch.float64)
                                                         / torch.linalg.vector_norm(ref, dtype=torch.float64).clamp_min(1e-300)).item())))
            del t3, ref
        if stats is not None:
            out._md_sums = stats
        elif hasattr(out, "_md_sums"):
            del out._md_sums
        return out
    if b_f32 is not None and b_f32.get("wino_only"):
        b_f32 = None
    ksplit = ops.ksplit_for(pw.cfg, B, pw.rows, pw.kdim, S_out) if out_mode == ops.OUT_F32B else 1
    stats = None
    if (want_stats and ops.FUSE_GN_STATS and ((pw.cfg == ops.CFG_C3_128_FAST and ksplit == 1)
                                              or (ksplit > 1 and ops.SPLITK_STATS and P <= 512 and B * rows_alloc >= 2048))
            and out_mode == ops.OUT_F32B and rows_alloc == pw.rows):
        stats = ops.stats_zeros(B, rows_alloc, dev)
    ops.gemm_conv(cfg=pw.cfg, a=pw.data, b=act_s16, out=out, batch=B, rows=pw.rows,
                  rows_alloc=rows_alloc, kdim=pw.kdim, dims=(S_out, S_out, S_out), bias=bias,
                  bias_bstride=bias_bstride, residual=residual, res_bstride=res_bstride or 0, ups=ups,
                  out_mode=out_mode, ksplit=ksplit, prec=pw.prec, stats=stats, b_f32=b_f32)
    if stats is not None:
        out._md_sums = stats
    elif hasattr(out, "_md_sums"):
        del out._md_sums
    return out


def run_gemm(pw, act_s16, B, P, *, bias=None, bias_bstride=0, residual=None, out=None, out_mode=ops.OUT_F32B,
             alpha=1.0, b_bstride=None, b_f32=None):
    rows_alloc = ((pw.rows + 7) // 8) * 8
    dev = act_s16.device if act_s16 is not None else b_f32["parts"][0][0].device
    if out is None:
        out = (ops.f32b_empty if out_mode == ops.OUT_F32B else ops.s16b_empty)(B, rows_alloc, P, dev)
    return ops.gemm_conv(cfg=pw.cfg, a=pw.data, b=act_s16, out=out, batch=B, rows=pw.rows,
                         rows_alloc=rows_alloc, kdim=pw.kdim, dims=(1, 1, P), bias=bias,
                         bias_bstride=bias_bstride, residual=residual,
                         res_bstride=rows_alloc * P if residual is not None else 0, alpha=alpha,
                         out_mode=out_mode, b_bstride=b_bstride, b_f32=b_f32)


class NIN(HipLayer):

    def __init__(self, in_dim, num_units, init_scale=0.1):
        super().__init__()
        self.W = nn.Parameter(default_init(scale=init_scale)((in_dim, num_units)), requires_grad=True)
        self.b = nn.Parameter(torch.zeros(num_units), requires_grad=True)

    def packed(self, P, hbm_bound=False):
        rows = self.W.shape[1]
        cfg = ops.gemm_cfg_for(P, rows, hbm_bound)
        return self._cached(f"w{cfg}", [self.W], lambda: ops.PackedWeight(self.W, "nin", cfg, self.W.device))

    def forward_s16(self, act_s16, B, P, residual=None, out_mode=ops.OUT_F32B):
        return run_gemm(self.packed(P), act_s16, B, P, bias=self.b, residual=residual, out_mode=out_mode)

    def forward(self, x):
        parts, B, P, spatial = _parts_of(x)
        act = ops.gn_apply(parts, None, B, P, norm=False, silu=False)
        return ops.f32b_to_ncdhw(self.forward_s16(act, B, P), spatial)


class AttnBlock(HipLayer):

    def __init__(self, channels):
        super().__init__()
        self.GroupNorm_0 = nn.GroupNorm(num_groups=32, num_channels=channels, eps=1e-6)
        self.NIN_0 = NIN(channels, channels)
        self.NIN_1 = NIN(channels, channels)
        self.NIN_2 = NIN(channels, channels)
        self.NIN_3 = NIN(channels, channels, init_scale=0.0)
        self.channels = channels

    def _qk_packed(self, P):
        cfg = ops.gemm_cfg_for(P, 2 * self.channels)

        def build():
            w = torch.cat([self.NIN_0.W.detach(), self.NIN_1.W.detach()], dim=1)
            return ops.PackedWeight(w, "nin", cfg, w.device)

        return self._cached(f"qk{cfg}", [self.NIN_0.W, self.NIN_1.W], build)

    def _qk_bias(self):
        return self._cached("qkb", [self.NIN_0.b, self.NIN_1.b],
                            lambda: torch.cat([self.NIN_0.b.detach(), self.NIN_1.b.detach()]).contiguous())

    def _wv_s16(self):
        return self._cached("wv", [self.NIN_2.W], lambda: ops.pack_s16b_from_matrix(self.NIN_2.W, self.NIN_2.W.device))

    def forward_blocked(self, x, B, P, tape=None):
        Cc = self.channels
        dev = x.device
        gn = self.GroupNorm_0
        params = ops.gn_params([(x, Cc)], gn.weight, gn.bias, B, P, eps=gn.eps, groups=gn.num_groups)
        h = ops.gn_apply([(x, Cc)], params, B, P, norm=True, silu=False)
        qk = run_gemm(self._qk_packed(P), h, B, P, bias=self._qk_bias(), out_mode=ops.OUT_S16B)
        qk_bstride = (2 * Cc // 8) * 2 * P * 8
        k_view = qk.view(-1)[(Cc // 8) * 2 * P * 8:]
        cfg_v = ops.gemm_cfg_for(Cc, P)
        vT = ops.s16b_empty(B, P, Cc, dev)
        ops.gemm_conv(cfg=cfg_v, a=h, b=self._wv_s16(), out=vT, batch=B, rows=P, rows_alloc=P, kdim=Cc,
                      dims=(1, 1, Cc), a_src=ops.A_S16B, a_rows=P, a_bstride=(Cc // 8) * 2 * P * 8,
                      b_bstride=0, out_mode=ops.OUT_S16B)
        if tape is None and ops.attn_fused_ok(Cc, P):
            o = ops.attn_fwd(qk, vT, self.NIN_2.b, B, Cc, P, ops.attn_scale(Cc))
            return self.NIN_3.forward_s16(o, B, P, residual=x)
        cfg_s = ops.gemm_cfg_for(P, P)
        sT = ops.f32b_empty(B, P, P, dev)
        ops.gemm_conv(cfg=cfg_s, a=k_view, b=qk, out=sT, batch=B, rows=P, rows_alloc=P, kdim=Cc,
                      dims=(1, 1, P), a_src=ops.A_S16B, a_rows=P, a_bstride=qk_bstride, b_bstride=qk_bstride,
                      alpha=ops.attn_scale(Cc))
        pr = ops.softmax_keys(sT, B, P, P)
        cfg_o = ops.gemm_cfg_for(P, Cc)
        o = ops.s16b_empty(B, Cc, P, dev)
        ops.gemm_conv(cfg=cfg_o, a=vT, b=pr, out=o, batch=B, rows=Cc, rows_alloc=Cc, kdim=P, dims=(1, 1, P),
                      a_src=ops.A_S16B, a_rows=Cc, a_bstride=(P // 8) * 2 * Cc * 8, bias=self.NIN_2.b,
                      out_mode=ops.OUT_S16B)
        if tape is not None:
            tape.append(dict(layer=self, x=x, prm=params, hN=h, qk=qk, vT=vT, pr=pr, o=o, B=B, P=P, S=_spatial_edge(P)))
        return self.NIN_3.forward_s16(o, B, P, residual=x)

    def backward_blocked(self, sv, dy):
        from . import backward as bw
        return bw.attn_backward(self, sv, dy)

    def forward(self, x):
        parts, B, P, spatial = _parts_of(x)
        return ops.f32b_to_ncdhw(self.forward_blocked(parts[0][0], B, P), spatial)


class Upsample(HipLayer):
    def __init__(self, channels, with_conv=False):
        super().__init__()
        if not with_conv:
            raise NotImplementedError("Upsample without conv is not used by the registered models")
        self.Conv_0 = ddpm_conv3x3(channels, channels)
        self.with_conv = with_conv

    def forward_blocked(self, x, Cc, B, P, tape=None):
        s_out = 2 * _spatial_edge(P)
        pw = conv3_packed(self, "w", self.Conv_0, ops.conv_cfg_for(s_out))
        if tape is None and fused_operand_ok(pw, ups=1) and pw.kdim == Cc:
            return run_conv3(pw, None, B, s_out, bias=self.Conv_0.bias, ups=1, want_stats=True,
                             b_f32=dict(parts=[(x, Cc)], ac=None, silu=False), wino=conv3_wino_packed(self, "w", self.Conv_0))
        fw = None
        ww = (tape is not None and pw.prec == ops.PREC_BF16X3 and pw.kdim == Cc
              and ops.wgrad_wino_ok(pw.rows, pw.kdim, s_out, B))
        act = None if ww else ops.gn_apply([(x, Cc)], None, B, P, norm=False, silu=False, fp16=pw.prec == ops.PREC_FP16X2)
        if tape is not None:
            assert pw.prec == ops.PREC_BF16X3
            if ops.WINO_TRAIN_FWD:
                fw = dict(parts=[(x, Cc)], ac=None, silu=False, wino_only=True, keep=ww)
        out = run_conv3(pw, act, B, s_out, bias=self.Conv_0.bias, ups=1, want_stats=True, b_f32=fw,
                        wino=conv3_wino_packed(self, "w", self.Conv_0) if fw is not None else None)
        if tape is not None:
            tape.append(dict(layer=self, act=act, t=fw.get("t_out") if fw else None, B=B, S_out=s_out))
        return out

    def backward_blocked(self, sv, dy):
        from . import backward as bw
        return bw.conv3_backward(self, "w", self.Conv_0, dy, sv["act"], sv["B"], sv["S_out"], ups=1, t_act=sv.get("t"))

    def forward(self, x):
        parts, B, P, spatial = _parts_of(x)
        return ops.f32b_to_ncdhw(self.forward_blocked(parts[0][0], parts[0][1], B, P), tuple(2 * s for s in spatial))


class Downsample(HipLayer):
    def __init__(self, channels, with_conv=False):
        super().__init__()
        if not with_conv:
            raise NotImplementedError("Downsample without conv is not used by the registered models")
        self.Conv_0 = ddpm_conv3x3(channels, channels, stride=2, padding=0)
        self.with_conv = with_conv

    def forward_blocked(self, x, Cc, B, P, tape=None):
        s_out = _spatial_edge(P) // 2
        if ops.conv3_s2_ok(self.Conv_0.weight.shape[0], Cc, s_out, B):
            pw = self._cached("w/s2", [self.Conv_0.weight],
                              lambda: ops.PackedWeight(self.Conv_0.weight, "conv", ops.CFG_S2_PACK, self.Conv_0.weight.device))
            stats = ops.stats_zeros(B, pw.rows, x.device) if ops.FUSE_GN_STATS and pw.rows % 8 == 0 else None
            out = ops.conv3_s2(pw, x, B, s_out, bias=self.Conv_0.bias, stats=stats)
            if stats is not None:
                out._md_sums = stats
            if tape is not None:
                tape.append(dict(layer=self, act=ops.gn_apply([(x, Cc)], None, B, P, norm=False, silu=False), B=B, S_out=s_out))
            return out
        act = ops.gn_apply([(x, Cc)], None, B, P, norm=False, silu=False)
        pw = conv3_packed(self, "w", self.Conv_0, ops.conv_cfg_for(s_out, stride=2))
        if tape is not None:
            tape.append(dict(layer=self, act=act, B=B, S_out=s_out))
        return run_conv3(pw, act, B, s_out, bias=self.Conv_0.bias)

    def backward_blocked(self, sv, dy):
        from . import backward as bw
        return bw.conv3_backward(self, "w", self.Conv_0, dy, sv["act"], sv["B"], sv["S_out"], stride=2)

    def forward(self, x):
        parts, B, P, spatial = _parts_of(x)
        return ops.f32b_to_ncdhw(self.forward_blocked(parts[0][0], parts[0][1], B, P), tuple(s // 2 for s in spatial))


class ResnetBlockDDPM(HipLayer):

    def __init__(self, act, in_ch, out_ch=None, temb_dim=None, conv_shortcut=False, dropout=0.1):
        super().__init__()
        out_ch = in_ch if out_ch is None else out_ch
        if conv_shortcut:
            raise NotImplementedError("conv_shortcut is never enabled by the registered models")
        self.GroupNorm_0 = nn.GroupNorm(num_groups=32, num_channels=in_ch, eps=1e-6)
        self.act = act
        self.Conv_0 = ddpm_conv3x3(in_ch, out_ch)
        if temb_dim is not None:
            self.Dense_0 = nn.Linear(temb_dim, out_ch)
            self.Dense_0.weight.data = default_init()(self.Dense_0.weight.data.shape)
            nn.init.zeros_(self.Dense_0.bias)
        self.GroupNorm_1 = nn.GroupNorm(num_groups=32, num_channels=out_ch, eps=1e-6)
        self.Dropout_0 = nn.Dropout(dropout)
        self.Conv_1 = ddpm_conv3x3(out_ch, out_ch, init_scale=0.0)
        if in_ch != out_ch:
            self.NIN_0 = NIN(in_ch, out_ch)
        self.out_ch, self.in_ch, self.conv_shortcut = out_ch, in_ch, conv_shortcut

    def _bias0(self):
        if hasattr(self, "Dense_0"):
            return self._cached("b0", [self.Conv_0.bias, self.Dense_0.bias],
                                lambda: (self.Conv_0.bias.detach() + self.Dense_0.bias.detach()).contiguous())
        return self.Conv_0.bias

    def forward_blocked(self, parts, B, P, temb=None, bias0=None, bias0_stride=None, tape=None):
        drop = (self.Dropout_0.p, ops.next_dropout_seed()) if self.training and self.Dropout_0.p > 0 else None
        S = _spatial_edge(P)
        cin = sum(c for _, c in parts)
        assert cin == self.in_ch
        cfg = ops.conv_cfg_for(S)
        g0, g1 = self.GroupNorm_0, self.GroupNorm_1
        pw0, pw1 = conv3_packed(self, "w0", self.Conv_0, cfg), conv3_packed(self, "w1", self.Conv_1, cfg)
        f16 = pw0.prec == ops.PREC_FP16X2
        need_nin = self.in_ch != self.out_ch
        if (tape is None and drop is None and fused_operand_ok(pw0) and fused_operand_ok(pw1) and pw0.kdim == cin
                and pw1.kdim == self.out_ch and not ops.NIN_SIDE_STREAM):
            _, ac0 = ops.gn_params(parts, g0.weight, g0.bias, B, P, eps=g0.eps, groups=g0.num_groups, want_ac=True)
            if bias0 is None:
                if temb is not None:
                    bias0, bias0_stride = ops.linear(temb, self.Dense_0.weight, self._bias0(), silu_in=True), self.out_ch
                else:
                    bias0, bias0_stride = self.Conv_0.bias, 0
            h = run_conv3(pw0, None, B, S, bias=bias0, bias_bstride=bias0_stride, want_stats=True,
                          b_f32=dict(parts=parts, ac=ac0, silu=True), wino=conv3_wino_packed(self, "w0", self.Conv_0, gn=g0))
            if need_nin:
                pwn = self.NIN_0.packed(P, hbm_bound=True)
                if pwn.kdim == cin and ops.nin_stream_ok(parts, self.out_ch, P):
                    res = ops.nin_f32(parts, pwn, self.NIN_0.b, B, P)
                elif pwn.cfg in (ops.CFG_G1_128, ops.CFG_G1_128_N128) and pwn.kdim == cin:
                    res = run_gemm(pwn, None, B, P, bias=self.NIN_0.b, b_f32=dict(parts=parts, ac=None, silu=False))
                else:
                    xs = ops.gn_apply(parts, None, B, P, norm=False, silu=False)
                    res = self.NIN_0.forward_s16(xs, B, P)
            else:
                res = parts[0][0]
            _, ac1 = ops.gn_params([(h, self.out_ch)], g1.weight, g1.bias, B, P, eps=g1.eps, groups=g1.num_groups, want_ac=True)
            return run_conv3(pw1, None, B, S, bias=self.Conv_1.bias, residual=res, want_stats=True,
                             b_f32=dict(parts=[(h, self.out_ch)], ac=ac1, silu=True), wino=conv3_wino_packed(self, "w1", self.Conv_1, gn=g1))
        wino_fwd = tape is not None and not f16 and ops.WINO_TRAIN_FWD
        ww0 = wino_fwd and pw0.kdim == cin and ops.wgrad_wino_ok(self.out_ch, cin, S, B)
        ww1 = wino_fwd and pw1.kdim == self.out_ch and ops.wgrad_wino_ok(self.out_ch, self.out_ch, S, B)
        prm, ac0 = ops.gn_params(parts, g0.weight, g0.bias, B, P, eps=g0.eps, groups=g0.num_groups, want_ac=True)
        f0 = dict(parts=parts, ac=ac0, silu=True, wino_only=True, keep=ww0) if wino_fwd else None
        w0 = conv3_wino_packed(self, "w0", self.Conv_0) if f0 is not None else None
        xs = None
        res = None
        if ww0:
            a0 = None
            if need_nin:
                xs = ops.gn_apply(parts, None, B, P, norm=False, silu=False)
        else:
            a0 = ops.gn_apply(parts, prm, B, P, norm=True, silu=True, fp16=f16, want_raw=need_nin)
            if need_nin:
                a0, xs = a0
        if need_nin and ops.NIN_SIDE_STREAM:
            main, side = torch.cuda.current_stream(), ops.side_stream()
            side.wait_stream(main)
            with torch.cuda.stream(side):
                res = self.NIN_0.forward_s16(xs, B, P)
            res.record_stream(main)
            xs.record_stream(side)
        if bias0 is not None:
            h = run_conv3(pw0, a0, B, S, bias=bias0, bias_bstride=bias0_stride, want_stats=True, b_f32=f0, wino=w0)
        elif temb is not None:
            bias0 = ops.linear(temb, self.Dense_0.weight, self._bias0(), silu_in=True)
            h = run_conv3(pw0, a0, B, S, bias=bias0, bias_bstride=self.out_ch, want_stats=True, b_f32=f0, wino=w0)
        else:
            h = run_conv3(pw0, a0, B, S, bias=self.Conv_0.bias, want_stats=True, b_f32=f0, wino=w0)
        prm1, ac1 = ops.gn_params([(h, self.out_ch)], g1.weight, g1.bias, B, P, eps=g1.eps, groups=g1.num_groups, want_ac=True)
        a1 = None if ww1 else ops.gn_apply([(h, self.out_ch)], prm1, B, P, norm=True, silu=True, fp16=f16, drop=drop)
        f1 = dict(parts=[(h, self.out_ch)], ac=ac1, silu=True, drop=drop, wino_only=True, keep=ww1) if wino_fwd else None
        w1 = conv3_wino_packed(self, "w1", self.Conv_1) if f1 is not None else None
        if need_nin:
            if res is None:
                res = self.NIN_0.forward_s16(xs, B, P)
            else:
                torch.cuda.current_stream().wait_stream(ops.side_stream())
        else:
            assert len(parts) == 1
            res = parts[0][0]
        out = run_conv3(pw1, a1, B, S, bias=self.Conv_1.bias, residual=res, want_stats=True, b_f32=f1, wino=w1)
        if tape is not None:
            assert not f16, "the backward pass uses the bf16x3 operand format"
            tape.append(dict(layer=self, parts=parts, prm0=prm, a0=a0, h=h, prm1=prm1, a1=a1, xs=xs, B=B, P=P, S=S,
                             temb=temb, drop=drop, t0=f0.get("t_out") if f0 else None, t1=f1.get("t_out") if f1 else None))
        return out

    def backward_blocked(self, sv, dy):
        from . import backward as bw
        B, P, S, parts = sv["B"], sv["P"], sv["S"], sv["parts"]
        shared = {} if self.in_ch != self.out_ch else None
        if sv.get("t1") is not None:
            bsum = torch.zeros((B, self.out_ch), dtype=torch.float32, device=dy.device)
        else:
            bsum = bw.channel_sums(dy, B, self.out_ch, P)
        d_a1 = bw.conv3_backward(self, "w1", self.Conv_1, dy, sv["a1"], B, S, bias_sums=bsum, shared=shared, t_act=sv.get("t1"),
                                 bias_sums_out=sv.get("t1") is not None)
        dbias0 = torch.zeros((B, self.out_ch), dtype=torch.float32, device=dy.device)
        d_h = bw.gn_backward([(sv["h"], self.out_ch)], d_a1, sv["prm1"], self.GroupNorm_1, B, P, silu=True,
                             drop=sv.get("drop"), sums_out=dbias0,
                             want_amax=ops.DGRAD_F6 and ops.DGRAD_LIFT == "dyn" and sv.get("t0") is not None)[0]
        del d_a1
        d_a0 = bw.conv3_backward(self, "w0", self.Conv_0, d_h, sv["a0"], B, S, bias_sums=False, t_act=sv.get("t0"))
        del d_h
        if self.in_ch != self.out_ch:
            dparts = bw.gn_backward(parts, d_a0, sv["prm0"], self.GroupNorm_0, B, P, silu=True)
            bw.nin_backward(self.NIN_0, dy, sv["xs"], B, P, S, bias_sums=bsum, shared=shared,
                            accumulate_into=[(g, c) for g, (_, c) in zip(dparts, parts)])
            shared.clear()
            return dparts, dbias0
        d_x = bw.gn_backward(parts, d_a0, sv["prm0"], self.GroupNorm_0, B, P, silu=True, residual=dy)[0]
        return [d_x], dbias0

    def forward(self, x, temb=None):
        parts, B, P, spatial = _parts_of(x)
        return ops.f32b_to_ncdhw(self.forward_blocked(parts, B, P, temb), spatial)


_ = math
```

Baseline: 109.7.

## Store upsampled Winograd operand compactly in D and H, expand in conv gather

For nearest-upsampled Winograd conv inputs, the prep kernel now writes the transformed operand only at half resolution in D and H (W transform still full), and the conv kernel indexes rows with z>>1, y>>1 to read duplicated rows. This cuts operand write traffic and scratch size by four on upsampling layers while the conv reads the same data more times from a smaller footprint. It is enabled by default via an env flag and restricted to inference paths without dropout or kept operands.

```diff
diff --git a/include/meshdiffusion_hip.h b/include/meshdiffusion_hip.h
--- a/include/meshdiffusion_hip.h
+++ b/include/meshdiffusion_hip.h
@@ -159,6 +159,15 @@
                      const float* residual, int64_t res_bstride, double* stats, int32_t batch, int32_t cin, int32_t cout,
                      int32_t D, int32_t H, int32_t W, void* stream);
 
+#define MD_WINO_FMT_BF16X3 0
+#define MD_WINO_FMT_F16F8 1
+#define MD_WINO_FMT_F16F6 2
+int md_wino_prep_upsdh(int32_t fmt, const float* x1, const float* x2, int32_t c1, int32_t c2, const float* ac, int32_t silu,
+                       const float* eq, void* t_out, int32_t batch, int32_t D, int32_t H, int32_t W, void* stream);
+int md_conv3_wino_upsdh(int32_t fmt, const void* t_in, const void* wpk, float* out, const float* bias, int64_t bias_bstride,
+                        const float* residual, int64_t res_bstride, double* stats, int32_t batch, int32_t cin, int32_t cout,
+                        int32_t D, int32_t H, int32_t W, void* stream);
+
 int md_conv3_stem(const void* x16, const void* wpk, float* out, const float* bias, const float* residual, double* stats,
                   int32_t batch, int32_t cout, int32_t D, int32_t H, int32_t W, void* stream);
 
diff --git a/meshdiffusion_amd/_lib.py b/meshdiffusion_amd/_lib.py
--- a/meshdiffusion_amd/_lib.py
+++ b/meshdiffusion_amd/_lib.py
@@ -47,6 +47,7 @@
 
 
 PACK_WPK, PACK_WINO, PACK_WINO_F6 = 0, 1, 2
+WINO_FMT = {False: 0, "f8": 1, "f6": 2}
 ABI_VERSION = 16
 _P, _I32, _I64, _F, _U64 = C.c_void_p, C.c_int32, C.c_int64, C.c_float, C.c_uint64
 
@@ -90,6 +91,8 @@
     "md_wino_prep_f6": (C.c_int, [_P, _P, _I32, _I32, _P, _I32, _I32, _P, _P, _I32, _I32, _I32, _I32, _P]),
     "md_wino_pack_weights_f6": (C.c_int, [_P, _P, _P, _I32, _I32, _I64, _I64, _P]),
     "md_conv3_wino_f6": (C.c_int, [_P, _P, _P, _P, _I64, _P, _I64, _P, _I32, _I32, _I32, _I32, _I32, _I32, _P]),
+    "md_wino_prep_upsdh": (C.c_int, [_I32, _P, _P, _I32, _I32, _P, _I32, _P, _P, _I32, _I32, _I32, _I32, _P]),
+    "md_conv3_wino_upsdh": (C.c_int, [_I32, _P, _P, _P, _P, _I64, _P, _I64, _P, _I32, _I32, _I32, _I32, _I32, _I32, _P]),
     "md_conv3_stem": (C.c_int, [_P, _P, _P, _P, _P, _P, _I32, _I32, _I32, _I32, _I32, _P]),
     "md_conv3_head": (C.c_int, [_P, _P, _P, _P, _I32, _I32, _I32, _I32, _I32, _I32, _P]),
     "md_pack_batch": (C.c_int, [_P, _I32, _I64, _I32, _P]),
diff --git a/meshdiffusion_amd/csrc/conv3_wino.hip b/meshdiffusion_amd/csrc/conv3_wino.hip
--- a/meshdiffusion_amd/csrc/conv3_wino.hip
+++ b/meshdiffusion_amd/csrc/conv3_wino.hip
@@ -159,6 +159,7 @@
   int batch, cin, cout, D, H, W;
   float out_scale;
   const uint32_t* amax;
+  int ups_dh;
 };
 
 typedef int wn_i32x8 __attribute__((ext_vector_type(8)));
@@ -187,7 +188,8 @@
     }
   }
   const int D = A.D, H = A.H, W = A.W, Wp = W >> 1;
-  const int64_t P = (int64_t)D * H * W, Ph = P >> 1;
+  const int64_t P = (int64_t)D * H * W, Ph = P >> (1 + 2 * A.ups_dh);
+  const int ush = A.ups_dh, Hrows = H >> ush;
   const int ntx = W / WN_TX, nty = H / WN_TY, ntz = D / WN_TZ;
   const int tiles = ntx * nty * ntz;
   int bid = blockIdx.x;
@@ -206,12 +208,13 @@
     const int dz = tp / 40, hy = (tp >> 2) % 10, pr = tp & 3;
     const int z = z0 + dz - 1, y = y0 + hy - 1;
     const bool live = (z >= 0) & (z < D) & (y >= 0) & (y < H);
+    const int row = (z >> ush) * Hrows + (y >> ush);
     if constexpr (F8) {
       const int Phi = (int)Ph;
-      const int off = (hp >> 1) * 8 * Phi + (hp & 1) * Phi + (z * H + y) * Wp + (x0 >> 1) + pr;
+      const int off = (hp >> 1) * 8 * Phi + (hp & 1) * Phi + row * Wp + (x0 >> 1) + pr;
       return live ? off : -1;
     }
-    return live ? (int)((int64_t)(hp >> 1) * 8 * Ph + (int64_t)(hp & 1) * Ph + ((int64_t)z * H + y) * Wp + (x0 >> 1) + pr) : -1;
+    return live ? (int)((int64_t)(hp >> 1) * 8 * Ph + (int64_t)(hp & 1) * Ph + (int64_t)row * Wp + (x0 >> 1) + pr) : -1;
   };
   const uint4* tbase = A.T + ((int64_t)b * CG * 8 + wid * 2) * Ph;
   const uint4* zsrc = &wn_zero16;
@@ -789,7 +792,7 @@
 static int md_conv3_wino_f8_launch(bool f6, const void* t_in, const void* wpk, float* out, const float* bias, int64_t bias_bstride,
                                    const float* residual, int64_t res_bstride, double* stats, int32_t batch, int32_t cin,
                                    int32_t cout, int32_t D, int32_t H, int32_t W, void* stream, float out_scale = 1.0f,
-                                   const uint32_t* amax = nullptr) {
+                                   const uint32_t* amax = nullptr, bool upsdh = false) {
   if (!t_in || !wpk || !out || batch <= 0) return MD_ERR_BAD_ARG;
   if (cin <= 0 || cout <= 0 || (cin % 32) || (cout % 128)) return MD_ERR_UNSUPPORTED;
   if (D <= 0 || H <= 0 || W <= 0 || (D % WN_TZ) || (H % WN_TY) || (W % WN_TX)) return MD_ERR_UNSUPPORTED;
@@ -800,6 +803,7 @@
   a.out_scale = out_scale; a.amax = amax;
   a.bias_bstride = bias_bstride; a.res_bstride = res_bstride;
   a.batch = batch; a.cin = cin; a.cout = cout; a.D = D; a.H = H; a.W = W;
+  a.ups_dh = upsdh ? 1 : 0;
   const int tiles = (D / WN_TZ) * (H / WN_TY) * (W / WN_TX);
   const dim3 grid((unsigned)(tiles * batch), (unsigned)(cout / 128));
   MD_HIP_CLEAR_ERROR();
@@ -836,9 +840,9 @@
                                  amax_bits);
 }
 
-extern "C" int md_conv3_wino(const void* t_in, const void* wpk, float* out, const float* bias, int64_t bias_bstride,
-                             const float* residual, int64_t res_bstride, double* stats, int32_t batch, int32_t cin,
-                             int32_t cout, int32_t D, int32_t H, int32_t W, int32_t variant, void* stream) {
+static int md_conv3_wino_launch(const void* t_in, const void* wpk, float* out, const float* bias, int64_t bias_bstride,
+                                const float* residual, int64_t res_bstride, double* stats, int32_t batch, int32_t cin,
+                                int32_t cout, int32_t D, int32_t H, int32_t W, int32_t variant, void* stream, bool upsdh) {
   if (!t_in || !wpk || !out || batch <= 0) return MD_ERR_BAD_ARG;
   if (cin <= 0 || cout <= 0 || (cin % 32) || (cout % 128)) return MD_ERR_UNSUPPORTED;
   if (D <= 0 || H <= 0 || W <= 0 || (D % WN_TZ) || (H % WN_TY) || (W % WN_TX)) return MD_ERR_UNSUPPORTED;
@@ -849,11 +853,13 @@
   a.out_scale = 1.0f; a.amax = nullptr;
   a.bias_bstride = bias_bstride; a.res_bstride = res_bstride;
   a.batch = batch; a.cin = cin; a.cout = cout; a.D = D; a.H = H; a.W = W;
+  a.ups_dh = upsdh ? 1 : 0;
   const int tiles = (D / WN_TZ) * (H / WN_TY) * (W / WN_TX);
   MD_HIP_CLEAR_ERROR();
   const dim3 grid((unsigned)(tiles * batch), (unsigned)(cout / 128));
 #define WN_LAUNCH(A_) hipLaunchKernelGGL((md_conv3_wino_kernel<A_, false, false, true>), grid, dim3(WN_THREADS), 0, (hipStream_t)stream, a)
   if (variant != 0 && residual == nullptr) return MD_ERR_UNSUPPORTED;
+  if (upsdh && variant != 0) return MD_ERR_BAD_ARG;
   switch (variant) {
     case 0:
       if (residual) WN_LAUNCH(0);
@@ -878,3 +884,19 @@
   MD_HIP_CHECK_LAUNCH();
   return MD_OK;
 }
+
+extern "C" int md_conv3_wino(const void* t_in, const void* wpk, float* out, const float* bias, int64_t bias_bstride,
+                             const float* residual, int64_t res_bstride, double* stats, int32_t batch, int32_t cin,
+                             int32_t cout, int32_t D, int32_t H, int32_t W, int32_t variant, void* stream) {
+  return md_conv3_wino_launch(t_in, wpk, out, bias, bias_bstride, residual, res_bstride, stats, batch, cin, cout, D, H, W, variant, stream, false);
+}
+
+extern "C" int md_conv3_wino_upsdh(int32_t fmt, const void* t_in, const void* wpk, float* out, const float* bias, int64_t bias_bstride,
+                                   const float* residual, int64_t res_bstride, double* stats, int32_t batch, int32_t cin,
+                                   int32_t cout, int32_t D, int32_t H, int32_t W, void* stream) {
+  if (fmt == MD_WINO_FMT_BF16X3)
+    return md_conv3_wino_launch(t_in, wpk, out, bias, bias_bstride, residual, res_bstride, stats, batch, cin, cout, D, H, W, 0, stream, true);
+  if (fmt != MD_WINO_FMT_F16F8 && fmt != MD_WINO_FMT_F16F6) return MD_ERR_BAD_ARG;
+  return md_conv3_wino_f8_launch(fmt == MD_WINO_FMT_F16F6, t_in, wpk, out, bias, bias_bstride, residual, res_bstride, stats, batch, cin, cout, D, H,
+                                 W, stream, 1.0f, nullptr, true);
+}
diff --git a/meshdiffusion_amd/csrc/wino_prep2.hip b/meshdiffusion_amd/csrc/wino_prep2.hip
--- a/meshdiffusion_amd/csrc/wino_prep2.hip
+++ b/meshdiffusion_amd/csrc/wino_prep2.hip
@@ -30,14 +30,15 @@
   const int cg = (blockIdx.x / nblk) % CG;
   const int b = blockIdx.x / (nblk * CG);
   int Di = D, Hi = H, Wi = W;
-  if (ups) { Di >>= 1; Hi >>= 1; Wi >>= 1; }
+  const int ush = ups == 1;
+  if (ups) { Di >>= ush; Hi >>= ush; Wi >>= 1; }
   const int64_t Pin = (int64_t)Di * Hi * Wi;
   const float* src = (cg * 8 < c1) ? x1 + ((int64_t)b * (c1 >> 3) + cg) * Pin * 8
                                    : x2 + ((int64_t)b * (c2 >> 3) + (cg - (c1 >> 3))) * Pin * 8;
   {
     const int64_t p = (int64_t)blk * P2_POS + tid;
     const int x = (int)(p % W), y = (int)((p / W) % H), z = (int)(p / ((int64_t)W * H));
-    const int64_t spos = ups ? ((int64_t)(z >> 1) * Hi + (y >> 1)) * Wi + (x >> 1) : p;
+    const int64_t spos = ups ? ((int64_t)(z >> ush) * Hi + (y >> ush)) * Wi + (x >> 1) : p;
     const f32x4* sp = (const f32x4*)(src + spos * 8);
     const f32x4 v0 = sp[0], v1 = sp[1];
     float a[8], c[8];
@@ -181,12 +182,13 @@
   const int cgp = (blockIdx.x / nblk) % CGP;
   const int b = blockIdx.x / (nblk * CGP);
   int Di = D, Hi = H, Wi = W;
-  if (ups) { Di >>= 1; Hi >>= 1; Wi >>= 1; }
+  const int ush = ups == 1;
+  if (ups) { Di >>= ush; Hi >>= ush; Wi >>= 1; }
   const int64_t Pin = (int64_t)Di * Hi * Wi;
   {
     const int64_t p = (int64_t)blk * P2_POS + tid;
     const int x = (int)(p % W), y = (int)((p / W) % H), z = (int)(p / ((int64_t)W * H));
-    const int64_t spos = ups ? ((int64_t)(z >> 1) * Hi + (y >> 1)) * Wi + (x >> 1) : p;
+    const int64_t spos = ups ? ((int64_t)(z >> ush) * Hi + (y >> ush)) * Wi + (x >> 1) : p;
 #pragma unroll
     for (int g2 = 0; g2 < 2; ++g2) {
       const int cg = 2 * cgp + g2;
@@ -308,6 +310,7 @@
 static int md_wino_prep2_launch(const float* x1, const float* x2, int32_t c1, int32_t c2, const float* ac, int32_t silu,
                                 int32_t ups, void* t_out, void* u_out, float* sums, int32_t batch, int32_t D, int32_t H, int32_t W, float drop_p,
                                 uint64_t drop_seed, void* stream, bool f8 = false, const float* eq = nullptr) {
+  ups = ups ? 1 : 0;
   if (!x1 || !t_out || batch <= 0 || c1 <= 0 || c2 < 0 || (c1 & 7) || (c2 & 7) || (c2 > 0 && !x2)) return MD_ERR_BAD_ARG;
   if (silu && !ac) return MD_ERR_BAD_ARG;
   if (D <= 0 || H <= 0 || W <= 0 || (W & 1) || (ups && ((D | H | W) & 1))) return MD_ERR_BAD_ARG;
@@ -354,6 +357,7 @@
 
 extern "C" int md_wino_prep_f6(const float* x1, const float* x2, int32_t c1, int32_t c2, const float* ac, int32_t silu,
                                int32_t ups, const float* eq, void* t_out, int32_t batch, int32_t D, int32_t H, int32_t W, void* stream) {
+  ups = ups ? 1 : 0;
   if (!x1 || !t_out || batch <= 0 || c1 <= 0 || c2 < 0 || (c1 & 15) || (c2 & 15) || (c2 > 0 && !x2)) return MD_ERR_BAD_ARG;
   if (silu && !ac) return MD_ERR_BAD_ARG;
   if (D <= 0 || H <= 0 || W <= 0 || (W & 1) || (ups && ((D | H | W) & 1))) return MD_ERR_BAD_ARG;
@@ -382,3 +386,31 @@
   MD_HIP_CHECK_LAUNCH();
   return MD_OK;
 }
+
+extern "C" int md_wino_prep_upsdh(int32_t fmt, const float* x1, const float* x2, int32_t c1, int32_t c2, const float* ac, int32_t silu,
+                                  const float* eq, void* t_out, int32_t batch, int32_t D, int32_t H, int32_t W, void* stream) {
+  if (fmt < MD_WINO_FMT_BF16X3 || fmt > MD_WINO_FMT_F16F6) return MD_ERR_BAD_ARG;
+  const int cmask = fmt == MD_WINO_FMT_F16F6 ? 15 : 7;
+  if (!x1 || !t_out || batch <= 0 || c1 <= 0 || c2 < 0 || (c1 & cmask) || (c2 & cmask) || (c2 > 0 && !x2)) return MD_ERR_BAD_ARG;
+  if ((eq && fmt == MD_WINO_FMT_BF16X3) || (silu && !ac)) return MD_ERR_BAD_ARG;
+  if (D <= 0 || H <= 0 || W <= 0 || ((D | H | W) & 1)) return MD_ERR_BAD_ARG;
+  D >>= 1; H >>= 1;
+  const int64_t P = (int64_t)D * H * W;
+  if ((P2_POS % W) || (P % P2_POS)) return MD_ERR_UNSUPPORTED;
+  const int64_t blocks = (int64_t)batch * ((c1 + c2) / (cmask + 1)) * (P / P2_POS);
+  if (blocks > 0x7fffffff) return MD_ERR_UNSUPPORTED;
+  const dim3 grid((unsigned)blocks);
+  hipStream_t st = (hipStream_t)stream;
+  MD_HIP_CLEAR_ERROR();
+  if (fmt == MD_WINO_FMT_F16F6)
+    hipLaunchKernelGGL(md_wino_prep2_f6_kernel<false>, grid, dim3(256), 0, st, x1, x2, c1, c2, ac, silu, 2, (uint4*)t_out, batch, D, H, W, eq,
+                       (uint4*)nullptr, (float*)nullptr, 1.0f, (const uint32_t*)nullptr);
+  else if (fmt == MD_WINO_FMT_F16F8)
+    hipLaunchKernelGGL((md_wino_prep2_kernel<false, true>), grid, dim3(256), 0, st, x1, x2, c1, c2, ac, silu, 2, (uint4*)t_out, (uint4*)nullptr,
+                       (float*)nullptr, batch, D, H, W, 0u, 1.0f, (uint64_t)0, eq);
+  else
+    hipLaunchKernelGGL((md_wino_prep2_kernel<false>), grid, dim3(256), 0, st, x1, x2, c1, c2, ac, silu, 2, (uint4*)t_out, (uint4*)nullptr,
+                       (float*)nullptr, batch, D, H, W, 0u, 1.0f, (uint64_t)0, (const float*)nullptr);
+  MD_HIP_CHECK_LAUNCH();
+  return MD_OK;
+}
diff --git a/meshdiffusion_amd/hip_ops.py b/meshdiffusion_amd/hip_ops.py
--- a/meshdiffusion_amd/hip_ops.py
+++ b/meshdiffusion_amd/hip_ops.py
@@ -548,23 +548,39 @@
     return WINO_F8
 
 
-def wino_prep(parts, ac, silu, ups, B, S, drop=None, keep=False, dual=False, sums=None, f8=False, eq=None, tscale=1.0, amax=None, dims=None):
+PREP_COMPACT_UPS = os.environ.get("MD_PREP_COMPACT_UPS", "1") == "1"
+
+
+def prep_compact_ok(ups, D, H, W, drop=None, keep=False):
+    return bool(PREP_COMPACT_UPS and WINO_PREP_V2 and ups and not drop and not keep and not ((D | H | W) & 1) and 256 % W == 0
+                and ((D // 2) * (H // 2) * W) % 256 == 0)
+
+
+def wino_prep(parts, ac, silu, ups, B, S, drop=None, keep=False, dual=False, sums=None, f8=False, eq=None, tscale=1.0, amax=None, dims=None,
+              compact=False):
     lib = _lib.load()
     D, H, W = dims if dims is not None else (S, S, S)
     cin = sum(c for _, c in parts)
     assert 1 <= len(parts) <= 2
+    assert not (compact and (dual or keep or drop)), "the compact operand is an inference layout"
     assert eq is None or (f8 and eq.numel() == cin and eq.dtype == torch.float32 and eq.is_cuda), "eq belongs to the f16f8 / f16f6 operand"
     assert ac is not None or not silu, "SiLU is applied together with the folded GroupNorm affine (pass `ac`)"
     nbytes = lib.md_wino_operand_bytes(B, cin, D, H, W)
     if nbytes <= 0:
         raise _lib.MeshDiffusionHipError("md_wino_operand_bytes: unsupported operand shape")
     dev = parts[0][0].device
+    if compact:
+        assert ups and prep_compact_ok(ups, D, H, W)
+        nbytes //= 4
     t = torch.empty(nbytes // 2, dtype=torch.bfloat16, device=dev) if keep else _wino_scratch(nbytes // 2, dev)
     x2, c2 = (parts[1][0], parts[1][1]) if len(parts) == 2 else (None, 0)
     ev = _prof_begin()
     args = (_ptr(parts[0][0]), _ptr(x2), parts[0][1], c2, _ptr(ac), 1 if silu else 0, 1 if ups else 0)
     tail = (B, D, H, W, drop[0] if drop else 0.0, drop[1] if drop else 0, _stream())
-    if f8 and dual:
+    if compact:
+        check(lib.md_wino_prep_upsdh(_lib.WINO_FMT["f6" if f8 == "f6" else ("f8" if f8 else False)], *args[:6], _ptr(eq), _ptr(t), B, D, H, W,
+                                     _stream()), "md_wino_prep_upsdh")
+    elif f8 and dual:
         assert f8 == "f6" and len(parts) == 1 and ac is None and not (ups or keep or drop or eq is not None) and 256 % W == 0
         u = _wino_scratch(nbytes // 2, dev, slot="u")
         check(lib.md_wino_prep_dual_f6(_ptr(parts[0][0]), cin, _ptr(t), _ptr(u), _ptr(sums), float(tscale), _ptr(amax), B, D, H, W, _stream()),
@@ -583,10 +599,11 @@
     else:
         fn = lib.md_wino_prep_v2 if (WINO_PREP_V2 and 256 % W == 0 and (D * H * W) % 256 == 0) else lib.md_wino_prep
         check(fn(*args, _ptr(t), *tail), "md_wino_prep")
-    _prof_end(ev, "wino_prep", 0.0, 4.0 * B * cin * (D * H * W // (8 if ups else 1)) + (16.0 if dual else 8.0) * B * cin * D * H * W,
+    _prof_end(ev, "wino_prep", 0.0, 4.0 * B * cin * (D * H * W // (8 if ups else 1)) + (16.0 if dual else 8.0) * B * cin * (D * H * W // (4 if compact else 1)),
               f"{cin}@{D}x{H}x{W}" + ("/ups" if ups else "") + ("/dual" if dual else "") + (("/f6" if f8 == "f6" else "/f8") if f8 else ""))
     t._md_fmt = ("f6" if f8 == "f6" else "f8") if f8 else False
     t._md_eq = eq.data_ptr() if eq is not None else 0
+    t._md_compact = bool(compact)
     return (t, u) if dual else t
 
 
@@ -628,7 +645,11 @@
         want = ww.fmt if f8 else False
         if t_fmt != want or getattr(t, "_md_eq", 0) != ((ww.eq.data_ptr() if ww.eq is not None else 0) if f8 else 0):
             raise _lib.MeshDiffusionHipError(f"conv3_wino: operand format {t_fmt!r} / equaliser does not belong to these weights ({want!r})")
-    if f8 and (out_scale != 1.0 or amax is not None):
+    if getattr(t, "_md_compact", False):
+        assert out_scale == 1.0 and amax is None and variant is None
+        check(lib.md_conv3_wino_upsdh(_lib.WINO_FMT[ww.fmt if f8 else False], _ptr(t), _ptr(ww.data), _ptr(out), _ptr(bias), bias_bstride,
+                                      _ptr(residual), res_bstride, _ptr(stats), B, ww.kdim, ww.rows, D, H, W, _stream()), "md_conv3_wino_upsdh")
+    elif f8 and (out_scale != 1.0 or amax is not None):
         assert ww.fmt == "f6"
         check(lib.md_conv3_wino_f6_scaled(_ptr(t), _ptr(ww.data), _ptr(out), _ptr(bias), bias_bstride, _ptr(residual), res_bstride,
                                           _ptr(stats), B, ww.kdim, ww.rows, D, H, W, float(out_scale), _ptr(amax), _stream()),
diff --git a/meshdiffusion_amd/lib/diffusion/models/layers.py b/meshdiffusion_amd/lib/diffusion/models/layers.py
--- a/meshdiffusion_amd/lib/diffusion/models/layers.py
+++ b/meshdiffusion_amd/lib/diffusion/models/layers.py
@@ -146,14 +146,15 @@
             or (ops.WINO_EQ and hasattr(wino, "measured") and wino.measured() is not None))
         if f8 and owner is not None and wino.site in getattr(owner, "md_bf16x3_sites", ()):
             f8 = False
+        compact = (not b_f32.get("wino_only")) and ops.prep_compact_ok(ups, S_out, S_out, S_out, drop=b_f32.get("drop"), keep=bool(b_f32.get("keep")))
         t = ops.wino_prep(b_f32["parts"], b_f32.get("ac"), b_f32.get("silu"), ups, B, S_out, drop=b_f32.get("drop"),
-                          keep=bool(b_f32.get("keep")), f8=f8, eq=wino.eq() if f8 and hasattr(wino, "eq") else None)
+                          keep=bool(b_f32.get("keep")), f8=f8, eq=wino.eq() if f8 and hasattr(wino, "eq") else None, compact=compact)
         if b_f32.get("keep"):
             b_f32["t_out"] = t
         ops.conv3_wino(wino(f8) if f8 else wino(), t, B, S_out, bias=bias, bias_bstride=bias_bstride, residual=residual,
                        res_bstride=res_bstride or 0, stats=stats, out=out)
         if f8 and ops.AUDIT is not None:
-            t3 = ops.wino_prep(b_f32["parts"], b_f32.get("ac"), b_f32.get("silu"), ups, B, S_out)
+            t3 = ops.wino_prep(b_f32["parts"], b_f32.get("ac"), b_f32.get("silu"), ups, B, S_out, compact=compact)
             ref = ops.conv3_wino(wino(), t3, B, S_out, bias=bias, bias_bstride=bias_bstride, residual=residual, res_bstride=res_bstride or 0)
             ops.AUDIT.append(dict(owner=getattr(wino, "owner", None), site=getattr(wino, "site", None), fmt=f8, cin=pw.kdim, cout=pw.rows,
                                   S=S_out, rel_l2=float((torch.linalg.vector_norm(out - ref, dtype=torch.float64)
```

After: 111.0 (median of 6 runs). 1.01x the previous value.
